# tomer196/GaUDI

Measured on AMD Instinct MI355X. Metric: guided molecules/sec (1000-step), higher is better.
Workload: dtype f32

## Files before the change

gaudi_amd/_lib.py:

```python
from __future__ import annotations

import ctypes as C
import os

import numpy as np

_PKG = os.path.dirname(os.path.abspath(__file__))
LIB_PATH = os.environ.get("GAUDI_LIB", os.path.join(_PKG, "libgaudi_hip.so"))


class GaudiError(RuntimeError):
    pass


class EdmConfig(C.Structure):
    _fields_ = [("in_node_nf", C.c_int32), ("hidden_nf", C.c_int32), ("n_layers", C.c_int32),
                ("inv_sublayers", C.c_int32), ("attention", C.c_int32), ("tanh", C.c_int32),
                ("coords_range", C.c_float), ("norm_constant", C.c_float), ("normalization_factor", C.c_float),
                ("diffusion_steps", C.c_int32), ("noise_power", C.c_float), ("noise_precision", C.c_float),
                ("norm_values", C.c_float * 3), ("sin_embedding", C.c_int32)]


class PredConfig(C.Structure):
    _fields_ = [("in_nf", C.c_int32), ("out_nf", C.c_int32), ("hidden_nf", C.c_int32), ("n_layers", C.c_int32),
# ... 4 lines not shown
    _fields_ = [("max_masked_leak", C.c_float), ("max_cog_rel", C.c_float), ("max_cog_abs", C.c_float),
                ("nan_count", C.c_int32), ("reprojected", C.c_int32)]


class RingTables(C.Structure):
    _fields_ = [("n_types", C.c_int32), ("orientation", C.c_int32), ("check_dihedrals", C.c_int32), ("tol", C.c_double),
                ("min_dist", C.c_double), ("dist_lo", (C.c_double * 16) * 16), ("dist_hi", (C.c_double * 16) * 16),
                ("a3_count", C.c_int32 * 16), ("a3_lo", (C.c_double * 4) * 16), ("a3_hi", (C.c_double * 4) * 16),
                ("a4_0", C.c_double), ("a4_180", C.c_double)]


class StabilityAux(C.Structure):
    _fields_ = [("n_rings", C.c_int32), ("n_edges", C.c_int32), ("n_triplets", C.c_int32), ("n_nan_angles", C.c_int32),
                ("a3_min", C.c_float), ("a3_max", C.c_float), ("a4_min", C.c_float), ("a4_max", C.c_float)]


class AtomTables(C.Structure):
    _fields_ = [("n_types", C.c_int32), ("ring_size", C.c_int32 * 16), ("ring_elem", (C.c_int32 * 6) * 16),
                ("templ", ((C.c_double * 2) * 6) * 16), ("no_orientation", C.c_int32 * 16), ("extra_angle", C.c_double * 16),
                ("n_template_h", C.c_int32 * 16), ("template_h_parent", (C.c_int32 * 2) * 16), ("h_elem", C.c_int32),
                ("c_elem", C.c_int32), ("h_bond", C.c_double)]


class PerceptionTables(C.Structure):
    _fields_ = [("n_elems", C.c_int32), ("cov_radius", C.c_double * 8), ("h_elem", C.c_int32), ("c_elem", C.c_int32),
                ("b_elem", C.c_int32), ("n_types", C.c_int32), ("ring_size", C.c_int32 * 16), ("ring_elem", (C.c_int32 * 6) * 16),
                ("no_orientation", C.c_int32 * 16), ("db_type", C.c_int32), ("dhdb_type", C.c_int32)]


class ValenceTables(C.Structure):
    _fields_ = [("n_elems", C.c_int32), ("n_options", (C.c_int32 * 5) * 8), ("option", (((C.c_int32 * 2) * 2) * 5) * 8),
                ("h_elem", C.c_int32), ("c_elem", C.c_int32)]


RINGS_MAX_ATOMS, RINGS_MAX_HEAVY, RINGS_MAX_RINGS = 384, 192, 32
RINGS_USE_H = 1
RINGS_OK, RINGS_NO_RINGS, RINGS_BAD_TYPE, RINGS_NOT_A_BASIS, RINGS_OVERFLOW = 0, 1, 2, 3, 4

ATOMS_MAX_ATOMS = 384
ATOMS_MAX_BONDS = 384
ATOMS_PLACE_H, ATOMS_FINGERPRINT = 1, 2

BONDS_MAX_ATOMS, BONDS_MAX_HEAVY, BONDS_MAX_BONDS, BONDS_MAX_CHARGED = 384, 192, 384, 4
(BONDS_OK, BONDS_NO_STRUCTURE, BONDS_CAPPED, BONDS_NOT_CONNECTED, BONDS_BAD_VALENCE, BONDS_BAD_INPUT, BONDS_OVERFLOW,
 BONDS_EMPTY, BONDS_GAVE_UP) = range(9)

FP_BINS = (256, 512, 1024)
CANON_MAX_ATOMS, CANON_MAX_HEAVY, CANON_MAX_BONDS, CANON_MAX_DEGREE, CANON_MAX_NODES, CANON_MAX_DEPTH = 384, 192, 384, 8, 4096, 16
CANON_OK, CANON_GAVE_UP, CANON_BAD_INPUT, CANON_OVERFLOW, CANON_EMPTY = range(5)
SUB_MAX_QUERY, SUB_MAX_PATTERNS, SUB_MAX_STEPS, SUB_H_EXACT, SUB_CLOSED = 32, 64, 8192, 1, 2
SUB_OK, SUB_GAVE_UP, SUB_BAD_INPUT, SUB_OVERFLOW, SUB_EMPTY, SUB_BAD_PATTERN = range(6)

FP = C.POINTER(C.c_float)
IP = C.POINTER(C.c_int32)
DP = C.POINTER(C.c_double)
U8P = C.POINTER(C.c_uint8)


class TargetSpec(C.Structure):
    _fields_ = [("K", C.c_int32), ("w", FP), ("q", FP), ("c", FP), ("side", IP), ("scale", FP),
                ("w_per_mol", C.c_int32), ("q_per_mol", C.c_int32), ("c_per_mol", C.c_int32), ("side_per_mol", C.c_int32),
                ("scale_per_mol", C.c_int32), ("t_lo", C.c_int32), ("t_hi", C.c_int32)]


TARGET_CB = C.CFUNCTYPE(None, C.c_void_p, C.c_int, C.c_int, FP, C.c_float, FP)
TARGET_CBZ = C.CFUNCTYPE(None, C.c_void_p, C.c_int, C.c_int, C.c_int, C.c_int, FP, FP, C.c_float, FP, FP)

EXPORTS = {
    "gaudi_create": (C.c_int, [C.c_int, C.POINTER(C.c_void_p)]),
    "gaudi_destroy": (None, [C.c_void_p]),
    "gaudi_last_error": (C.c_char_p, [C.c_void_p]),
    "gaudi_load_edm": (C.c_int, [C.c_void_p, C.POINTER(EdmConfig), C.c_int, C.POINTER(C.c_char_p), C.POINTER(FP),
                                 C.POINTER(C.c_int64)]),
    "gaudi_load_predictor": (C.c_int, [C.c_void_p, C.POINTER(PredConfig), C.c_int, C.POINTER(C.c_char_p),
                                       C.POINTER(FP), C.POINTER(C.c_int64)]),
    "gaudi_get_gamma": (C.c_int, [C.c_void_p, FP]),
    "gaudi_get_step_coefficients": (C.c_int, [C.c_void_p, FP]),
    "gaudi_phi": (C.c_int, [C.c_void_p, C.c_int, C.c_int, FP, FP, FP, FP, FP]),
    "gaudi_predictor_fwd": (C.c_int, [C.c_void_p, C.c_int, C.c_int, FP, FP, FP, FP, FP]),
    "gaudi_predictor_grad": (C.c_int, [C.c_void_p, C.c_int, C.c_int, FP, FP, FP, FP, FP, FP, FP]),
    "gaudi_step": (C.c_int, [C.c_void_p, C.c_int, C.c_int, C.c_int, FP, FP, FP, FP, FP, C.c_float, FP]),
    "gaudi_decode": (C.c_int, [C.c_void_p, C.c_int, C.c_int, FP, FP, FP, FP, FP, FP]),
    "gaudi_sample": (C.c_int, [C.c_void_p, C.c_int, C.c_int, FP, FP, C.c_uint64, C.c_int64, FP, C.c_float, FP,
                               C.c_float, FP, FP, FP, C.POINTER(Diag)]),
    "gaudi_sample_cb": (C.c_int, [C.c_void_p, C.c_int, C.c_int, FP, FP, C.c_uint64, C.c_int64, FP, C.c_float, TARGET_CB,
                                  C.c_void_p, C.c_float, FP, FP, FP, C.POINTER(Diag)]),
    "gaudi_sample_cbz": (C.c_int, [C.c_void_p, C.c_int, C.c_int, FP, FP, C.c_uint64, C.c_int64, FP, C.c_float, TARGET_CBZ,
                                   C.c_void_p, C.c_float, FP, FP, FP, C.POINTER(Diag)]),
    "gaudi_sample_chain": (C.c_int, [C.c_void_p, C.c_int, C.c_int, FP, FP, C.c_uint64, C.c_int64, FP, C.c_float, C.c_int, FP]),
    "gaudi_predict_noised": (C.c_int, [C.c_void_p, C.c_int, C.c_int, FP, FP, IP, FP, FP, C.c_uint64, C.c_int64, FP, FP, FP]),
    "gaudi_check_stability": (C.c_int, [C.c_void_p, C.POINTER(RingTables), C.c_int, C.c_int, FP, IP, IP,
                                        C.POINTER(C.c_uint8), FP, FP, C.POINTER(StabilityAux)]),
    "gaudi_stability_profile_get": (C.c_int, [C.c_void_p, C.POINTER(C.c_int32), C.POINTER(C.c_double)]),
    "gaudi_rings_to_atoms": (C.c_int, [C.c_void_p, C.POINTER(RingTables), C.POINTER(AtomTables), C.c_int, C.c_int, FP, IP, IP,
                                       C.c_int, C.c_int, C.c_int, IP, IP, DP, DP, IP, IP, IP, C.POINTER(C.c_uint64)]),
    "gaudi_atoms_profile_get": (C.c_int, [C.c_void_p, C.POINTER(C.c_int32), C.POINTER(C.c_double)]),
    "gaudi_atoms_to_rings": (C.c_int, [C.c_void_p, C.POINTER(PerceptionTables), C.c_int, C.c_int, DP, IP, IP, C.c_int, C.c_double,
                                       C.c_int, IP, IP, IP, IP, IP, DP, IP, DP, C.POINTER(C.c_uint8)]),
    "gaudi_rings_profile_get": (C.c_int, [C.c_void_p, C.POINTER(C.c_int32), C.POINTER(C.c_double)]),
    "gaudi_host_atoms_to_rings": (C.c_int, [C.POINTER(PerceptionTables), C.c_int, C.c_int, DP, IP, IP, C.c_int, C.c_double,
                                            C.c_int, IP, IP, IP, IP, IP, DP, IP, DP, C.POINTER(C.c_uint8)]),
    "gaudi_bond_orders": (C.c_int, [C.c_void_p, C.POINTER(ValenceTables), C.c_int, C.c_int, C.c_int, IP, IP, IP, IP,
                                    C.POINTER(C.c_uint8), C.POINTER(C.c_int8), IP, IP]),
    "gaudi_bonds_profile_get": (C.c_int, [C.c_void_p, C.POINTER(C.c_int32), C.POINTER(C.c_double)]),
    "gaudi_host_bond_orders": (C.c_int, [C.POINTER(ValenceTables), C.c_int, C.c_int, C.c_int, IP, IP, IP, IP,
                                         C.POINTER(C.c_uint8), C.POINTER(C.c_int8), IP, IP]),
    "gaudi_canonical_order": (C.c_int, [C.c_void_p, C.c_int, C.c_int, C.c_int, C.c_int, C.c_int, C.c_int, IP, IP, IP, IP, IP, IP,
                                        C.POINTER(C.c_uint8), IP, C.POINTER(C.c_uint16), IP, IP]),
    "gaudi_canon_profile_get": (C.c_int, [C.c_void_p, C.POINTER(C.c_int32), C.POINTER(C.c_double)]),
    "gaudi_host_canonical_order": (C.c_int, [C.c_int, C.c_int, C.c_int, C.c_int, C.c_int, C.c_int, IP, IP, IP, IP, IP, IP,
                                             C.POINTER(C.c_uint8), IP, C.POINTER(C.c_uint16), IP, IP]),
    "gaudi_circular_fingerprint": (C.c_int, [C.c_void_p, C.c_int, C.c_int, C.c_int, C.c_int, C.c_int, C.c_int, IP, IP, IP, IP, C.c_int,
                                             C.c_int, U8P, IP, IP]),
    "gaudi_host_circular_fingerprint": (C.c_int, [C.c_int, C.c_int, C.c_int, C.c_int, C.c_int, C.c_int, IP, IP, IP, IP, C.c_int,
                                                  C.c_int, U8P, IP, IP]),
    "gaudi_fp_library_set": (C.c_int, [C.c_void_p, C.c_int, C.c_int, U8P]),
    "gaudi_fp_nearest": (C.c_int, [C.c_void_p, C.c_int, C.c_int, U8P, C.c_int, U8P, C.c_int, IP, IP, IP]),
    "gaudi_fp_common": (C.c_int, [C.c_void_p, C.c_int, C.c_int, U8P, C.c_int, U8P, IP]),
    "gaudi_host_fp_nearest": (C.c_int, [C.c_int, C.c_int, U8P, C.c_int, U8P, C.c_int, IP, IP, IP]),
    "gaudi_fp_profile_get": (C.c_int, [C.c_void_p, C.POINTER(C.c_int32), C.POINTER(C.c_double)]),
    "gaudi_substructure_search": (C.c_int, [C.c_void_p] + [C.c_int] * 6 + [IP] * 4 + [C.c_int] * 3 + [IP] * 5 + [IP, IP, U8P, IP, IP]),
    "gaudi_host_substructure_search": (C.c_int, [C.c_int] * 6 + [IP] * 4 + [C.c_int] * 3 + [IP] * 5 + [IP, IP, U8P, IP, IP]),
    "gaudi_host_substructure_root_steps": (C.c_int, [C.c_int]),
    "gaudi_substructure_profile_get": (C.c_int, [C.c_void_p, C.POINTER(C.c_int32), C.POINTER(C.c_double)]),
    "gaudi_philox_normal": (C.c_int, [C.c_void_p, C.c_uint64, C.c_int64, C.c_int, C.c_int, C.c_int, C.c_int, FP]),
    "gaudi_host_schedule": (C.c_int, [C.c_int, C.c_float, C.c_float, FP, FP]),
    "gaudi_host_eigh3": (C.c_int, [C.c_int, DP, DP]),
    "gaudi_host_graph_meta": (C.c_int, [C.c_int, C.c_int, FP, FP, C.POINTER(C.c_int32), C.POINTER(C.c_int32),
                                        C.POINTER(C.c_int32), C.POINTER(C.c_uint32), C.POINTER(C.c_uint32), FP, C.c_int32,
                                        C.POINTER(C.c_int32)]),
    "gaudi_host_pack_matrix": (C.c_int, [C.c_int, C.c_int, C.c_int, C.c_int, C.c_int, FP, FP]),
    "gaudi_host_pack_matrix_split": (C.c_int, [C.c_int, C.c_int, C.c_int, C.c_int, C.c_int, C.c_int, C.c_float, FP, FP]),
    "gaudi_host_pack_matrix_f16": (C.c_int, [C.c_int, C.c_int, C.c_int, C.c_int, C.c_int, C.c_float, FP, FP]),
    "gaudi_host_weight_scale": (C.c_int, [C.c_int, C.POINTER(FP), IP, IP, IP, FP]),
    "gaudi_host_node_operand_offset": (C.c_int, [C.c_int, C.c_int, C.c_int, C.c_int, C.c_int, IP]),
    "gaudi_profile_reset": (C.c_int, [C.c_void_p, C.c_int]),
    "gaudi_profile_get": (C.c_int, [C.c_void_p, C.POINTER(C.c_int32), C.POINTER(C.c_double), C.POINTER(C.c_int64)]),
    "gaudi_set_steps_per_launch": (C.c_int, [C.c_void_p, C.c_int]),
    "gaudi_set_readout_nodes": (C.c_int, [C.c_void_p, C.c_int]),
    "gaudi_set_fix_noise": (C.c_int, [C.c_void_p, C.c_int, C.c_int64]),
    "gaudi_host_graph_meta8": (C.c_int, [C.c_int, C.c_int, FP, FP, C.POINTER(C.c_int32), C.POINTER(C.c_int32),
                                         C.POINTER(C.c_int32), C.POINTER(C.c_uint32), C.POINTER(C.c_uint32), FP,
                                         C.POINTER(C.c_uint16), C.POINTER(C.c_uint16), C.c_int32, C.POINTER(C.c_int32)]),
    "gaudi_kernel_variant": (C.c_int, [C.c_void_p, C.POINTER(C.c_int32), C.POINTER(C.c_int32)]),
    "gaudi_edge_math": (C.c_int, [C.c_void_p, C.POINTER(C.c_int32), C.POINTER(C.c_int32)]),
    "gaudi_node_buffers": (C.c_int, [C.c_void_p, C.POINTER(C.c_int32)]),
    "gaudi_last_workgroups": (C.c_int, [C.c_void_p, C.POINTER(C.c_int32), C.POINTER(C.c_int32)]),
    "gaudi_host_pack_plan_wide": (C.c_int, [C.c_int, C.c_int, C.c_int, C.c_int, FP, FP, C.POINTER(C.c_int32), C.POINTER(C.c_int32),
                                           C.POINTER(C.c_int32), C.POINTER(C.c_int32)]),
    "gaudi_set_plan_hint": (C.c_int, [C.c_void_p, C.c_int32, C.c_int32]),
    "gaudi_last_warning": (C.c_char_p, [C.c_void_p]),
    "gaudi_last_kernel_key": (C.c_int, [C.c_void_p, C.c_char_p, C.c_int]),
    "gaudi_kernel_key_log": (C.c_int, [C.c_void_p, C.c_char_p, C.c_int]),
    "gaudi_host_kernel_keys": (C.c_int, [C.c_char_p, C.c_int]),
    "gaudi_abi_version": (C.c_int, []),
    "gaudi_last_family_split": (C.c_int, [C.c_void_p, C.POINTER(C.c_int32)]),
    "gaudi_profile_clock": (C.c_int, [C.c_void_p, C.POINTER(C.c_double)]),
    "gaudi_last_keep_h": (C.c_int, [C.c_void_p, C.POINTER(C.c_int32)]),
    "gaudi_host_pack_plan": (C.c_int, [C.c_int, C.c_int, FP, FP, C.POINTER(C.c_int32), C.POINTER(C.c_int32), C.POINTER(C.c_int32),
                                      C.POINTER(C.c_int32)]),
    "gaudi_edm_nll": (C.c_int, [C.c_void_p, C.c_int, C.c_int, FP, FP, IP, FP, FP, C.c_uint64, C.c_int64, FP, FP, FP]),
    "gaudi_host_nll_terms": (C.c_int, [C.c_int, C.c_float, C.c_float, C.c_float, C.c_float, C.c_int, C.c_int, C.c_int, FP, FP, FP,
                                       IP, FP]),
    "gaudi_predictor_loss_grad": (C.c_int, [C.c_void_p, C.c_int, C.c_int, FP, FP, IP, FP, FP, FP, C.c_uint64, C.c_int64, FP, FP,
                                            FP, FP, IP]),
    "gaudi_predictor_grad_size": (C.c_int, [C.c_void_p, C.POINTER(C.c_int64)]),
    "gaudi_host_pred_train_layout": (C.c_int, [C.c_void_p, C.c_int, C.POINTER(C.c_char_p), C.POINTER(FP), C.POINTER(C.c_int64),
                                               IP, IP, FP]),
    "gaudi_edm_loss_grad": (C.c_int, [C.c_void_p, C.c_int, C.c_int, FP, FP, IP, FP, FP, C.c_uint64, C.c_int64, FP, C.c_int, FP,
                                      FP, FP, FP, IP]),
    "gaudi_edm_grad_size": (C.c_int, [C.c_void_p, C.POINTER(C.c_int64)]),
    "gaudi_edm_set_train_weights": (C.c_int, [C.c_void_p, C.c_int, C.POINTER(C.c_char_p), C.POINTER(FP), C.POINTER(C.c_int64)]),
    "gaudi_host_edm_train_layout": (C.c_int, [C.c_void_p, C.c_int, C.POINTER(C.c_char_p), C.POINTER(FP), C.POINTER(C.c_int64),
                                              IP, IP, FP]),
    "gaudi_host_train_floats_per_mol": (C.c_int, [C.c_int] * 8 + [C.POINTER(C.c_int64)]),
    "gaudi_host_edm_seed_coef": (C.c_int, [C.c_int, C.c_int, C.c_int, C.c_int, C.c_int, IP, FP, FP, FP]),
    "gaudi_sample_grid": (C.c_int, [C.c_void_p, C.c_int, C.c_int, FP, FP, C.c_uint64, C.c_int64, FP, C.c_float, FP, C.c_float,
                                    C.c_int, IP, FP, FP, FP, FP, FP, FP, C.POINTER(Diag)]),
    "gaudi_step_pair": (C.c_int, [C.c_void_p, C.c_int, C.c_int, C.c_int, C.c_int, FP, FP, FP, FP, FP, C.c_float, FP]),
    "gaudi_sample_cb_grid": (C.c_int, [C.c_void_p, C.c_int, C.c_int, FP, FP, C.c_uint64, C.c_int64, FP, C.c_float, TARGET_CB,
                                       TARGET_CBZ, C.c_void_p, C.c_float, C.c_int, IP, FP, FP, FP, FP, FP, FP, C.POINTER(Diag)]),
    "gaudi_host_grid_coefficients": (C.c_int, [C.c_int, C.c_float, C.c_float, C.c_int, IP, FP, IP]),
    "gaudi_sample_target": (C.c_int, [C.c_void_p, C.c_int, C.c_int, FP, FP, C.c_uint64, C.c_int64, FP, C.c_float,
                                      C.POINTER(TargetSpec), C.c_int, IP, FP, FP, FP, FP, FP, FP, FP, C.POINTER(Diag)]),
    "gaudi_step_target": (C.c_int, [C.c_void_p, C.c_int, C.c_int, C.c_int, C.c_int, FP, FP, FP, FP, C.POINTER(TargetSpec), FP, FP]),
    "gaudi_host_target_seed": (C.c_int, [C.POINTER(TargetSpec), C.c_int, C.c_int, FP, FP]),
}

ABI_VERSION = 7
_ROUND6_EXPORTS = ("gaudi_last_warning", "gaudi_abi_version", "gaudi_last_family_split", "gaudi_profile_clock", "gaudi_last_keep_h")
_NLL_EXPORTS = ("gaudi_edm_nll", "gaudi_predictor_loss_grad", "gaudi_predictor_grad_size", "gaudi_edm_loss_grad",
                "gaudi_edm_grad_size", "gaudi_edm_set_train_weights")
_GRID_EXPORTS = ("gaudi_sample_grid", "gaudi_step_pair", "gaudi_sample_cb_grid")
_TARGET_EXPORTS = ("gaudi_sample_target", "gaudi_step_target")
_ATOMS_EXPORTS = ("gaudi_rings_to_atoms", "gaudi_atoms_profile_get")
_RINGS_EXPORTS = ("gaudi_atoms_to_rings", "gaudi_rings_profile_get")
_BONDS_EXPORTS = ("gaudi_bond_orders", "gaudi_bonds_profile_get")
_CANON_EXPORTS = ("gaudi_canonical_order", "gaudi_canon_profile_get")
_FP_EXPORTS = ("gaudi_circular_fingerprint", "gaudi_fp_library_set", "gaudi_fp_nearest", "gaudi_fp_common",
               "gaudi_fp_profile_get")
_SUB_EXPORTS = ("gaudi_substructure_search", "gaudi_substructure_profile_get")
_KEY_EXPORTS = ("gaudi_last_kernel_key", "gaudi_kernel_key_log", "gaudi_host_kernel_keys")

_lib = None


def load_library() -> C.CDLL:
    global _lib
    if _lib is not None:
        return _lib
    if not os.path.exists(LIB_PATH):
        raise GaudiError(f"{LIB_PATH} not found: build it with `python -m gaudi_amd.build` "
                         "(there is no CPU fallback for the sampler)")
    lib = C.CDLL(LIB_PATH)
    lenient = "GAUDI_LIB" in os.environ
    abi = None
    if hasattr(lib, "gaudi_abi_version"):
        lib.gaudi_abi_version.restype, lib.gaudi_abi_version.argtypes = C.c_int, []
        abi = int(lib.gaudi_abi_version())
    if abi != ABI_VERSION and not lenient:
        raise GaudiError(f"{LIB_PATH} exports ABI version {abi}, this package expects {ABI_VERSION}: rebuild it "
                         "(`python -m gaudi_amd.build --force`)")
    for name, (res, args) in EXPORTS.items():
        if lenient and not hasattr(lib, name) and (name.startswith("gaudi_host_") or name in _ROUND6_EXPORTS + _NLL_EXPORTS + _GRID_EXPORTS + _TARGET_EXPORTS + _ATOMS_EXPORTS + _RINGS_EXPORTS + _BONDS_EXPORTS + _CANON_EXPORTS + _FP_EXPORTS + _SUB_EXPORTS + _KEY_EXPORTS):
            continue
        if lenient and abi != ABI_VERSION and name.startswith("gaudi_host_"):
            continue
        fn = getattr(lib, name)
        fn.restype = res
        fn.argtypes = args
    _lib = lib
    return lib


def key_lines(fn, *head) -> list:
    need = fn(*head, None, 0)
    if need < 0:
        raise GaudiError(f"{fn.__name__} failed ({need})")
    buf = C.create_string_buffer(need)
    fn(*head, buf, need)
    return buf.value.decode().splitlines()


def registered_kernel_keys() -> list:
    return key_lines(load_library().gaudi_host_kernel_keys)


def rings_outputs(B: int, max_rings: int) -> dict:
    M = int(max_rings)
    return dict(status=np.zeros(B, np.int32), n_rings=np.zeros(B, np.int32), ring_size=np.zeros((B, M), np.int32),
                ring_atoms=np.full((B, M, 6), -1, np.int32), ring_type=np.zeros((B, M), np.int32),
                centre=np.zeros((B, M, 3), np.float64), n_orient=np.zeros((B, M), np.int32),
                orient=np.zeros((B, M, 2, 3), np.float64), adj=np.zeros((B, M, M), np.uint8))


def rings_args(xyz, elem, n_atoms, flags, covalency_factor, max_rings, out):
    assert xyz.dtype == np.float64 and elem.dtype == np.int32 and n_atoms.dtype == np.int32
    assert xyz.flags["C_CONTIGUOUS"] and elem.flags["C_CONTIGUOUS"] and n_atoms.flags["C_CONTIGUOUS"]
    B, A = xyz.shape[0], xyz.shape[1]
    assert xyz.shape == (B, A, 3) and elem.shape == (B, A) and n_atoms.shape == (B,)
    ip = lambda a: a.ctypes.data_as(IP)
    dp = lambda a: a.ctypes.data_as(DP)
    return (B, A, dp(xyz), ip(elem), ip(n_atoms), int(flags), float(covalency_factor), int(max_rings), ip(out["status"]),
            ip(out["n_rings"]), ip(out["ring_size"]), ip(out["ring_atoms"]), ip(out["ring_type"]), dp(out["centre"]),
            ip(out["n_orient"]), dp(out["orient"]), out["adj"].ctypes.data_as(C.POINTER(C.c_uint8)))


def host_atoms_to_rings(tables, xyz, elem, n_atoms, flags=0, covalency_factor=1.3, max_rings=RINGS_MAX_RINGS) -> dict:
    lib = load_library()
    out = rings_outputs(xyz.shape[0], max_rings)
    rc = lib.gaudi_host_atoms_to_rings(C.byref(tables), *rings_args(xyz, elem, n_atoms, flags, covalency_factor, max_rings, out))
    if rc != 0:
        raise GaudiError(f"gaudi_host_atoms_to_rings failed ({rc})")
    return out


def bonds_outputs(B: int, A: int, M: int) -> dict:
    return dict(order=np.zeros((B, M), np.uint8), charge=np.zeros((B, A), np.int8), n_charged=np.zeros(B, np.int32),
                status=np.zeros(B, np.int32))


def bonds_args(elem, n_atoms, bonds, n_bonds, out):
    for a in (elem, n_atoms, bonds, n_bonds):
        assert a.dtype == np.int32 and a.flags["C_CONTIGUOUS"]
    B, A, M = elem.shape[0], elem.shape[1], bonds.shape[1]
    assert elem.shape == (B, A) and bonds.shape == (B, M, 2) and n_atoms.shape == (B,) and n_bonds.shape == (B,)
    ip = lambda a: a.ctypes.data_as(IP)
    return (B, A, M, ip(elem), ip(n_atoms), ip(bonds), ip(n_bonds), out["order"].ctypes.data_as(C.POINTER(C.c_uint8)),
            out["charge"].ctypes.data_as(C.POINTER(C.c_int8)), ip(out["n_charged"]), ip(out["status"]))


def host_bond_orders(tables, elem, n_atoms, bonds, n_bonds) -> dict:
    lib = load_library()
    out = bonds_outputs(elem.shape[0], elem.shape[1], bonds.shape[1])
    rc = lib.gaudi_host_bond_orders(C.byref(tables), *bonds_args(elem, n_atoms, bonds, n_bonds, out))
    if rc != 0:
        raise GaudiError(f"gaudi_host_bond_orders failed ({rc})")
    return out


def canon_outputs(B: int, A: int, M: int) -> dict:
    return dict(rank=np.zeros((B, A), np.int32), n_heavy=np.zeros(B, np.int32), label=np.zeros((B, A), np.uint8),
                n_hbonds=np.zeros(B, np.int32), cbonds=np.zeros((B, M, 2), np.uint16), nodes=np.zeros(B, np.int32),
                status=np.zeros(B, np.int32))


def canon_args(n_elems, h_elem, c_elem, elem, n_atoms, bonds, n_bonds, out):
    for a in (elem, n_atoms, bonds, n_bonds):
        assert a.dtype == np.int32 and a.flags["C_CONTIGUOUS"]
    B, A, M = elem.shape[0], elem.shape[1], bonds.shape[1]
    assert elem.shape == (B, A) and bonds.shape == (B, M, 2) and n_atoms.shape == (B,) and n_bonds.shape == (B,)
    ip = lambda a: a.ctypes.data_as(IP)
    return (int(n_elems), int(h_elem), int(c_elem), B, A, M, ip(elem), ip(n_atoms), ip(bonds), ip(n_bonds), ip(out["rank"]),
            ip(out["n_heavy"]), out["label"].ctypes.data_as(C.POINTER(C.c_uint8)), ip(out["n_hbonds"]),
            out["cbonds"].ctypes.data_as(C.POINTER(C.c_uint16)), ip(out["nodes"]), ip(out["status"]))


def host_canonical_order(n_elems, h_elem, c_elem, elem, n_atoms, bonds, n_bonds) -> dict:
    lib = load_library()
    out = canon_outputs(elem.shape[0], elem.shape[1], bonds.shape[1])
    rc = lib.gaudi_host_canonical_order(*canon_args(n_elems, h_elem, c_elem, elem, n_atoms, bonds, n_bonds, out))
    if rc != 0:
        raise GaudiError(f"gaudi_host_canonical_order failed ({rc})")
    return out


def fp_outputs(B: int, n_bins: int) -> dict:
    return dict(fp=np.zeros((B, n_bins), np.uint8), total=np.zeros(B, np.int32), status=np.zeros(B, np.int32))


def fp_args(n_elems, h_elem, c_elem, elem, n_atoms, bonds, n_bonds, radius, n_bins, out):
    for a in (elem, n_atoms, bonds, n_bonds):
        assert a.dtype == np.int32 and a.flags["C_CONTIGUOUS"]
    B, A, M = elem.shape[0], elem.shape[1], bonds.shape[1]
    assert elem.shape == (B, A) and bonds.shape == (B, M, 2) and n_atoms.shape == (B,) and n_bonds.shape == (B,)
    ip = lambda a: a.ctypes.data_as(IP)
    return (int(n_elems), int(h_elem), int(c_elem), B, A, M, ip(elem), ip(n_atoms), ip(bonds), ip(n_bonds), int(radius),
            int(n_bins), out["fp"].ctypes.data_as(U8P), ip(out["total"]), ip(out["status"]))


def host_circular_fingerprint(n_elems, h_elem, c_elem, elem, n_atoms, bonds, n_bonds, radius=2, n_bins=1024) -> dict:
    lib = load_library()
    out = fp_outputs(elem.shape[0], n_bins if n_bins in FP_BINS else 1)
    rc = lib.gaudi_host_circular_fingerprint(*fp_args(n_elems, h_elem, c_elem, elem, n_atoms, bonds, n_bonds, radius, n_bins, out))
    if rc != 0:
        raise GaudiError(f"gaudi_host_circular_fingerprint failed ({rc})")
    return out


def fp_rows(a) -> np.ndarray:
    a = np.ascontiguousarray(a, dtype=np.uint8)
    if a.ndim != 2:
        raise GaudiError(f"fingerprints must be [rows, n_bins], got shape {a.shape}")
    return a


def nearest_outputs(B: int, k: int) -> dict:
    k = max(int(k), 1)
    return dict(idx=np.zeros((B, k), np.int32), common=np.zeros((B, k), np.int32), union=np.zeros((B, k), np.int32))


def host_fp_nearest(q, lib_rows, k=1) -> dict:
    lib = load_library()
    q, lib_rows = fp_rows(q), fp_rows(lib_rows)
    out = nearest_outputs(q.shape[0], k)
    rc = lib.gaudi_host_fp_nearest(q.shape[1], q.shape[0], q.ctypes.data_as(U8P), lib_rows.shape[0], lib_rows.ctypes.data_as(U8P),
                                   int(k), *(out[n].ctypes.data_as(IP) for n in ("idx", "common", "union")))
    if rc != 0:
        raise GaudiError(f"gaudi_host_fp_nearest failed ({rc})")
    return out


def sub_outputs(B: int, P: int, A: int, QA: int) -> dict:
    return dict(count=np.zeros((B, P), np.int32), first=np.full((B, P, QA), -1, np.int32), covered=np.zeros((B, P, A), np.uint8),
                steps=np.zeros((B, P), np.int32), status=np.zeros((B, P), np.int32))


# ... 52 lines not shown
```

gaudi_amd/csrc/gaudi_hip.hip:

```cpp
#include <hip/hip_runtime.h>

#include <algorithm>
#include <climits>
#include <queue>
#include <cmath>
#include <cstdio>
#include <cstdlib>
#include <chrono>
#include <cstring>
#include <map>
#include <mutex>
#include <string>
#include <vector>

#include "../../include/gaudi_hip.h"
#include "kernel_table.h"

using namespace gaudi;

struct DevBuf {
  void* p = nullptr;
  size_t cap = 0;
  hipError_t reserve(size_t bytes) {
    if (bytes <= cap) return hipSuccess;
    if (p) (void)hipFree(p);
    p = nullptr;
    cap = 0;
    hipError_t e = hipMalloc(&p, bytes);
    if (e == hipSuccess) cap = bytes;
    return e;
  }
  void release() {
    if (p) (void)hipFree(p);
    p = nullptr;
    cap = 0;
  }
  template <class T>
  T* as() const { return (T*)p; }
};

struct PinBuf {
  void* p = nullptr;
  size_t cap = 0;
  hipError_t reserve(size_t bytes) {
    if (bytes <= cap) return hipSuccess;
    if (p) (void)hipHostFree(p);
    p = nullptr;
    cap = 0;
    hipError_t e = hipHostMalloc(&p, bytes, hipHostMallocDefault);
    if (e == hipSuccess) cap = bytes;
    return e;
  }
  void release() {
    if (p) (void)hipHostFree(p);
    p = nullptr;
    cap = 0;
  }
  template <class T>
  T* as() const { return (T*)p; }
};

enum NodeBuf : int {
  kResident = 0,
  kAllGlobal = 1,
  kPqLds = 2,
  kPredFifthGlobal = 3,
};
struct LaunchPlan {
  int waves = 4;
  int ring = 0;
  bool mr = false;
  NodeBuf nodes = kResident;
  bool two = false;
  bool fr = false;
  bool n1 = false;
  int ef = 2;
  int groups = 0;
  int nslots = 0;
  int hk = 0;
  int pubx = 0, pub_ch = 0;
};

struct VtCall {
  const gaudi_target_spec* spec = nullptr;
  int K = 0, Btot = 0, b0 = 0;
  float* trace = nullptr;
};

struct CallHints {
  int min_slots = 0, force_waves = 0;
  bool cut = false;
  int narrow = 0;
  const int32_t* molmap = nullptr;
  bool may_pack = false;
  const VtCall* vt = nullptr;
};

struct gaudi_handle {
  int device = 0;
  hipStream_t stream = nullptr;
  std::string err;
  std::string warn;
  bool has_edm = false, has_pred = false;
  gaudi_edm_config ecfg{};
  gaudi_pred_config pcfg{};
  int HPE = 0, HPP = 0;
  DevBuf edm_w, pred_w, coef_d, edm_w4, pred_w4;
  DevBuf edm_ws, pred_ws;
  size_t edm_w_bytes = 0, pred_w_bytes = 0, edm_ws_bytes = 0, pred_ws_bytes = 0;
  float edm_hinv = 0.f, pred_hinv = 0.f;
  std::vector<float> gamma, coef;
  DevBuf d_mask, d_order, d_edges, d_emask, d_npairs, d_seg, d_zin, d_zout, d_t, d_x, d_h, d_noise, d_nan, d_dpred,
      d_pred, d_tw, d_stash, d_chain, d_sx, d_stype, d_sn, d_sflags, d_sdist, d_sadj, d_saux, d_stab, d_as, d_ncols, d_soff,
      d_sidx, d_gnode, d_rowmap, d_compmol, d_ncomp, d_clock, d_gcoef, d_gidx, d_zt;
  DevBuf d_atoms[9];
  DevBuf d_rings[13];
  DevBuf d_bonds[9];
  DevBuf d_canon[11];
  DevBuf d_fp[16];
  int fp_lib_rows = 0, fp_lib_bins = 0;
  DevBuf d_sub[10];
  DevBuf d_vtpar, d_vttrace, d_vtdev;
  PinBuf p_pred, p_dpred;
  PinBuf p_z, p_dz;
  DevBuf d_dz;
  hipEvent_t cb_event = nullptr;
  int steps_per_launch = 25;
  int variant = 8;
  LaunchPlan plan;
  bool split = true;
  bool no_fr = false;
  bool no_n1 = false;
  bool no_side = false;
  std::string last_key;
  std::vector<std::string> key_log;
  bool wide_full = true;
  bool gn8_pq = true;
  bool gn8 = true;
  bool force_gn8 = false;
  bool pack = true;
  int pairs_cap = -1;
  int pairs = 1;
  int num_cus = 256;
  bool pred_rounds = true;
  bool force_mr = false;
  bool force_gn = false;
  bool fix_noise = false;
  long long fix_key = 0;
  int readout_n = 0;
  struct PredTrainState* pt = nullptr;
  struct EdmTrainState* et = nullptr;
  bool edm_stale = false;
  int plan_min_slots = 0, plan_force_waves = 0;
  bool keep_h = true;
  bool gn8_pack = true;
  bool family_split = false;
  int last_split_resident = 0;
  bool prof = false;
  struct EventLog {
    std::vector<std::pair<hipEvent_t, hipEvent_t>> pending, spare;
    double ms = 0.0;
    long long n = 0;
    static constexpr size_t kWindow = 32;
    hipError_t fold(size_t keep) {
      while (pending.size() > keep) {
        float t = 0.f;
        hipError_t e = hipEventSynchronize(pending.front().second);
        if (e == hipSuccess) e = hipEventElapsedTime(&t, pending.front().first, pending.front().second);
        if (e != hipSuccess) return e;
        ms += t;
        ++n;
        spare.push_back(pending.front());
        pending.erase(pending.begin());
      }
      return hipSuccess;
    }
    hipError_t begin(hipStream_t st, std::pair<hipEvent_t, hipEvent_t>& ev) {
      hipError_t e = fold(kWindow - 1);
      if (e != hipSuccess) return e;
      if (!spare.empty()) {
        ev = spare.back();
        spare.pop_back();
      } else {
        if ((e = hipEventCreate(&ev.first)) != hipSuccess) return e;
        if ((e = hipEventCreate(&ev.second)) != hipSuccess) return e;
      }
      return hipEventRecord(ev.first, st);
    }
    hipError_t end(hipStream_t st, const std::pair<hipEvent_t, hipEvent_t>& ev) {
      pending.push_back(ev);
      return hipEventRecord(ev.second, st);
    }
    void reset(bool destroy) {
      for (auto& p : pending) spare.push_back(p);
      pending.clear();
      if (destroy) {
        for (auto& p : spare) {
          (void)hipEventDestroy(p.first);
          (void)hipEventDestroy(p.second);
        }
        spare.clear();
      }
      ms = 0.0;
      n = 0;
    }
  } prof_log, stab_log, atoms_log, rings_log, bonds_log, canon_log, fp_log, sub_log;
  long long prof_steps = 0;
#ifdef GAUDI_STAMPS
  DevBuf d_stamps;
  unsigned long long stamp_acc[32] = {0};
#endif
};

#define HIPCHECK(h, call)                                                                         \
  do {                                                                                            \
    hipError_t e__ = (call);                                                                      \
    if (e__ != hipSuccess) {                                                                      \
      (h)->err = std::string(#call) + ": " + hipGetErrorString(e__);                              \
      return GAUDI_E_HIP;                                                                         \
    }                                                                                             \
  } while (0)

static int fail(gaudi_handle* h, int code, const std::string& msg) {
  if (h) h->err = msg;
  return code;
}

static void pt_release(gaudi_handle* h);
static void et_release(gaudi_handle* h);
static int et_upload(gaudi_handle* h, const gaudi_edm_config* cfg, int n, const char* const* names, const float* const* tensors,
                     const int64_t* numel);
static const char* et_check(const gaudi_edm_config* cfg, int n, const char* const* names, const int64_t* numel);
extern const char* const kEdmStale;
static int pt_load(gaudi_handle* h, const gaudi_pred_config* cfg, int n, const char* const* names, const float* const* tensors,
                   const int64_t* numel);

static std::vector<float> make_gamma(int T, double power, double precision) {
  const int steps = T + 1;
  if (power <= 0.0) {
    const int n = T + 2;
    const double s_ = 0.008, pi = 3.14159265358979323846;
    std::vector<double> ac(n);
    for (int i = 0; i < n; ++i) {
      const double x = (i == n - 1) ? (double)n : i * ((double)n / (double)(n - 1));
      const double c = std::cos(((x / n) + s_) / (1.0 + s_) * pi * 0.5);
      ac[i] = c * c;
    }
    const double a0 = ac[0];
    for (double& v : ac) v /= a0;
    std::vector<float> g(steps);
    double cum = 1.0;
    for (int i = 0; i < steps; ++i) {
      double beta = 1.0 - ac[i + 1] / ac[i];
      beta = std::min(std::max(beta, 0.0), 0.999);
      cum *= 1.0 - beta;
      g[i] = (float)(-(std::log(cum) - std::log(1.0 - cum)));
    }
    return g;
  }
  std::vector<double> a2(steps);
  const double step = (double)steps / (double)(steps - 1);
  for (int i = 0; i < steps; ++i) {
    double x = (i == steps - 1) ? (double)steps : i * step;
    double v = 1.0 - std::pow(x / steps, power);
    a2[i] = v * v;
  }
  std::vector<double> out(steps);
  double prev = 1.0, cum = 1.0;
  for (int i = 0; i < steps; ++i) {
    double r = a2[i] / prev;
    r = std::min(std::max(r, 0.001), 1.0);
    cum *= r;
    out[i] = cum;
    prev = a2[i];
  }
  std::vector<float> g(steps);
  const double pr = 1.0 - 2.0 * precision;
  for (int i = 0; i < steps; ++i) {
    double a = pr * out[i] + precision;
    g[i] = (float)(-(std::log(a) - std::log(1.0 - a)));
  }
  return g;
}

static inline float softplus_f(float x) { return x > 20.f ? x : log1pf(expf(x)); }
static inline float logsigmoid_f(float x) { return fminf(x, 0.f) - log1pf(expf(-fabsf(x))); }
// ... 401 lines not shown
  std::stable_sort(M.order.begin(), M.order.end(), [&](int a, int c) {
    return M.ntiles[a] != M.ntiles[c] ? M.ntiles[a] > M.ntiles[c] : total[a] > total[c];
  });
  return GAUDI_OK;
}

KernelTable* gaudi::g_kernel_tables;

static const KernelEntry* find_entry(const KernelKey& k) {
  for (const KernelTable* t = g_kernel_tables; t; t = t->next)
    for (int i = 0; i < t->n; ++i)
      if (t->entries[i].key == k) return &t->entries[i];
  return nullptr;
}
static kernel_fn find_kernel(const KernelKey& k) {
  const KernelEntry* e = find_entry(k);
  return e ? e->fn : nullptr;
}
static std::string key_name(const KernelKey& k) {
  char buf[160];
  snprintf(buf, sizeof buf, "waves=%d SP=%d MR=%d GN=%d FR=%d PG=%d N1=%d EF=%d HPE=%d HPP=%d VT=%d", k.waves, k.sp, (int)k.mr, k.gn,
           (int)k.fr, (int)k.pg, (int)k.n1, k.ef, k.hpe, k.hpp, (int)k.vt);
  return buf;
}
static std::string duplicate_kernel_key() {
  std::vector<KernelKey> seen;
  for (const KernelTable* t = g_kernel_tables; t; t = t->next)
    for (int i = 0; i < t->n; ++i) {
      if (std::find(seen.begin(), seen.end(), t->entries[i].key) != seen.end()) return key_name(t->entries[i].key);
      seen.push_back(t->entries[i].key);
    }
  return "";
}
static int gn_of(NodeBuf nodes) { return nodes == kAllGlobal ? 1 : nodes == kPqLds ? 2 : 0; }
static KernelKey key4(int hpe, int hpp, bool gn = false, int ef = 2) {
  KernelKey k{};
  k.waves = 4;
  k.gn = gn ? 1 : 0;
  k.ef = ef;
  k.hpe = hpe;
  k.hpp = hpp;
  return k;
}
static KernelKey key8(int hpe, int hpp, int ring, bool mr, NodeBuf nodes = kResident) {
  KernelKey k{};
  k.waves = 8;
  k.sp = ring;
  k.mr = mr;
  k.gn = gn_of(nodes);
  k.pg = nodes == kPredFifthGlobal;
  k.ef = 2;
  k.hpe = hpe;
  k.hpp = hpp;
  return k;
}
static bool have_kernel8(int hpe, int hpp, int ring, bool mr, NodeBuf nodes = kResident) {
  return find_kernel(key8(hpe, hpp, ring, mr, nodes)) != nullptr;
}
static NodeBuf launch_nodes(const LaunchPlan& p, int hpe, int hpp) {
  return p.nodes == kPredFifthGlobal && !(hpe && hpp) ? kResident : p.nodes;
}
static kernel_fn plan_kernel(const LaunchPlan& p, int hpe, int hpp, bool vt, KernelKey* key = nullptr) {
  KernelKey unused;
  KernelKey& k = key ? *key : unused;
  if (p.waves != 8) {
    k = key4(hpe, hpp, p.nodes == kAllGlobal, hpe ? p.ef : 2);
    k.vt = vt && hpp;
    return find_kernel(k);
  }
  const NodeBuf nodes = launch_nodes(p, hpe, hpp);
  const bool mr = p.mr && hpp;
  k = nodes == kResident ? key8(hpe, hpp, p.ring, mr) : key8(hpe, hpp, 1, true, nodes);
  k.vt = vt && hpp;
  if (p.fr && nodes == kResident && !mr) {
    k.fr = true;
    if (kernel_fn f = find_kernel(k)) return f;
    k.fr = false;
  }
  if (p.n1 && nodes == kResident && !mr) {
    k.n1 = true;
    if (kernel_fn f = find_kernel(k)) return f;
    k.n1 = false;
  }
  return find_kernel(k);
}

static int round_hidden(int H) {
  static const int sizes[] = {32, 48, 64, 128, 192, 208, 256};
  for (int s : sizes)
    if (s >= H) return s;
  return 0;
}

static int dense_ew4(int N) { return std::max(32, ((N + kWaves - 1) / kWaves * (N - 1) + 31) / 32 * 32); }

static size_t lds_bytes(int hpe, int hpp, int N, int D, int EW, bool gn = false, int ef = 2) {
  size_t net = 0;
  if (hpe)
    net = std::max(net, (size_t)((gn ? 0 : 4 * N * (hpe + 4)) + kWaves * 16 * (hpe + 4) + 8 * N + kWaves * EW * 9 + (6 + ef) * hpe +
                                 (ef > 2 ? kWaves * EW * ef : 0)));
  if (hpp) net = std::max(net, (size_t)((gn ? 0 : 5 * N * (hpp + 4)) + kWaves * 16 * (hpp + 4) + 12 * N + kWaves * EW * 10 + 32 + 10 * hpp));
  return sizeof(float) * (common_floats(N, D, EW) + net);
}
static size_t gnode_floats(int hpe, int hpp, int N) {
  return std::max((size_t)(hpe ? 4 * N * (hpe + 4) : 0), (size_t)(hpp ? 5 * N * (hpp + 4) : 0));
}

static size_t lds_floats8_base(int hpe, int hpp, int N, int D, int S, int split, NodeBuf nodes = kResident) {
  size_t net = 0;
  const int pbuf = nodes == kPredFifthGlobal ? 4 : 5;
  const int gn = gn_of(nodes);
  if (hpe) net = std::max(net, (size_t)((gn ? w8::gn_lds_buffers(gn) : 5) * N * (hpe + 4) + w8::edge_ring_floats(hpe, split) + 8 * N + 2 * align4(N) + 96 + S * 9 + 8 * hpe));
  if (hpp) net = std::max(net, (size_t)(w8::edge_ring_floats(hpp, split) + (gn ? w8::gn_lds_buffers(gn) : pbuf) * N * (hpp + 4) + 12 * N + 2 * align4(N) + 96 + S * 10 + 32 + 10 * hpp));
  return common_floats8(N, D, S) + net;
}
static size_t gnode_floats8(int hpe, int hpp, int N) {
  return std::max((size_t)(hpe ? 5 * N * (hpe + 4) : 0), (size_t)(hpp ? 5 * N * (hpp + 4) : 0));
}
static bool gn8_stage_fits(int hpe, int hpp, int N) {
  for (int hp : {hpe, hpp})
    if (hp && 2 * (size_t)w8::stage_stride(N * (hp + 4)) > w8::edge_ring_floats(hp, 1)) return false;
  return true;
}
static bool node_f16_fits(int hp, int N, int split, NodeBuf nodes) {
  const bool gn = gn_of(nodes) != 0;
  if (!hp || !split || !GAUDI_NODE_F16) return true;
  if (N > (gn ? 48 : 32)) return false;
  const int nct = N <= 16 ? 1 : N <= 32 ? 2 : 3;
  const int ring = w8::edge_ring_floats(hp, split);
  return w8::nh_split_floats(hp, nct) <= (w8::node_ring_idle(hp, split, gn) ? ring : ring / 2);
}
static bool plan_pub8(int hpe, int hpp, int N, int D, int S, int split, int& pubx, int& pub_ch, NodeBuf nodes = kResident) {
  pubx = 0;
  pub_ch = 0;
  const int gn = gn_of(nodes);
  if (!node_f16_fits(hpe, N, split, nodes) || !node_f16_fits(hpp, N, split, nodes)) return false;
  const long long cap = 160 * 1024 / 4 - 64;
  const long long base = (long long)lds_floats8_base(hpe, hpp, N, D, S, split, nodes);
  if (base > cap) return false;
  if (!hpp) return true;
  const int T = hpp / 16;
  const long long own = (gn ? 0LL : 2LL * N * (hpp + 4)) + (split ? w8::edge_ring_floats(hpp, split) : 0);
  pub_ch = w8::pub_chunk_tiles(S, own + (cap - base), T);
  if (pub_ch < 1) return false;
  const int nch = (T + pub_ch - 1) / pub_ch;
  pub_ch = (T + nch - 1) / nch;
  pubx = (int)std::max(0LL, (long long)S * (16 * pub_ch + 4) - own);
  return true;
}
static size_t lds_bytes8(int hpe, int hpp, int N, int D, int S, int pubx, int split, NodeBuf nodes = kResident) {
  return sizeof(float) * (lds_floats8_base(hpe, hpp, N, D, S, split, nodes) + (hpp ? pubx : 0));
}

static int launch(gaudi_handle* h, const KParams& P, int hpe, int hpp, long long steps) {
  const LaunchPlan& plan = h->plan;
  const bool v8 = plan.waves == 8;
  const bool se = hpe && plan.ef > 2;
  KernelKey key{};
  const kernel_fn fn = plan_kernel(plan, hpe, hpp, P.vt != nullptr, &key);
  if (!fn)
    return fail(h, GAUDI_E_INVALID,
                "no kernel instantiated for padded hidden sizes (" + std::to_string(hpe) + "," + std::to_string(hpp) + ")" +
                    (v8 ? " in the 8-wave family" : se ? " among the sin_embedding kernels" : ""));
  size_t lds = v8 ? lds_bytes8(hpe, hpp, P.N, 3 + P.F, P.EW, P.pubx, plan.ring, launch_nodes(plan, hpe, hpp))
                  : lds_bytes(hpe, hpp, P.N, 3 + P.F, P.EW, plan.nodes == kAllGlobal, se ? 24 : 2);
  if (v8 && P.hk_off) lds = sizeof(float) * ((size_t)P.hk_off + (size_t)plan.hk);
  if (lds > 160 * 1024)
    return fail(h, GAUDI_E_CAPACITY, "molecule needs " + std::to_string(lds) + " B of LDS (>160 KiB): N too large");
  {
    static std::mutex attr_mu;
    static std::map<std::pair<int, const void*>, int> granted_by_fn;
    std::lock_guard<std::mutex> lock(attr_mu);
    int& granted = granted_by_fn[{h->device, (const void*)fn}];
    if ((int)lds > granted) {
      HIPCHECK(h, hipFuncSetAttribute((const void*)fn, hipFuncAttributeMaxDynamicSharedMemorySize, (int)lds));
      granted = (int)lds;
    }
  }
  std::pair<hipEvent_t, hipEvent_t> ev{nullptr, nullptr};
  if (h->prof) HIPCHECK(h, h->prof_log.begin(h->stream, ev));
#ifdef GAUDI_STAMPS
  KParams PS = P;
  HIPCHECK(h, h->d_stamps.reserve(sizeof(unsigned long long) * 32));
  HIPCHECK(h, hipMemsetAsync(h->d_stamps.p, 0, sizeof(unsigned long long) * 32, h->stream));
  PS.stamps = h->d_stamps.as<unsigned long long>();
  hipLaunchKernelGGL(fn, dim3(P.B), dim3(v8 ? w8::kThreads : kThreads), lds, h->stream, PS);
  {
    unsigned long long tmp[32];
    HIPCHECK(h, hipMemcpyAsync(tmp, h->d_stamps.p, sizeof(tmp), hipMemcpyDeviceToHost, h->stream));
    HIPCHECK(h, hipStreamSynchronize(h->stream));
    for (int i = 0; i < 32; ++i) h->stamp_acc[i] += tmp[i];
    if (getenv("GAUDI_PRINT_STAMPS")) {
      static const char* nm[] = {"node_gemm", "edge_gemm", "edge_epilogue", "barrier", "misc", "bwd_node", "bwd_stash_reload",
                                 "bwd_colsum_tail", "pub_wait", "stash", "pub_write", "colsum_loop", "colsum_barrier", "b_dcp",
                                 "b_gemm_de", "b_dv", "b_gemm_dt1", "b_du", "stage_vectors", "geo", "edm_embed_head", "noise_update",
                                 "bwd_reload_loads", "bwd_vec_commit", "pred_readout", "bwd_prologue", "x2", "x3"};
      unsigned long long tot = 0;
      for (int i = 0; i < ST_N; ++i) tot += h->stamp_acc[i];
      fprintf(stderr, "[stamps] cumulative shares (block 0, wave 0):");
      for (int i = 0; i < ST_N; ++i) fprintf(stderr, " %s=%.1f%%", nm[i], 100.0 * h->stamp_acc[i] / (tot ? tot : 1));
      fprintf(stderr, " total=%llu ticks\n", tot);
      if (tmp[31])
        fprintf(stderr, "[stamps] shader clock during this launch: %.0f MHz (%llu cycles / %llu ticks of 100 MHz)\n",
                100.0 * (double)tmp[30] / (double)tmp[31], tmp[30], tmp[31]);
    }
  }
#else
  if (h->prof) {
    KParams PC = P;
    HIPCHECK(h, h->d_clock.reserve(sizeof(unsigned long long) * 4));
    PC.clock_out = h->d_clock.as<unsigned long long>();
    hipLaunchKernelGGL(fn, dim3(P.B), dim3(v8 ? w8::kThreads : kThreads), lds, h->stream, PC);
  } else {
    hipLaunchKernelGGL(fn, dim3(P.B), dim3(v8 ? w8::kThreads : kThreads), lds, h->stream, P);
  }
#endif
  HIPCHECK(h, hipGetLastError());
  h->last_key = key_name(key);
  if (std::find(h->key_log.begin(), h->key_log.end(), h->last_key) == h->key_log.end()) h->key_log.push_back(h->last_key);
  if (const KernelEntry* e = find_entry(key); e && (e->side & 1) && P.side_off != 0) h->last_key += " SD=" + std::to_string(e->side);
  if (getenv("GAUDI_DEBUG_PLAN")) fprintf(stderr, "[launch] %s\n", h->last_key.c_str());
  if (h->prof) {
    HIPCHECK(h, h->prof_log.end(h->stream, ev));
    h->prof_steps += steps;
  }
  return GAUDI_OK;
}

struct Pack {
  int G = 0;
  int NG = 0;
  std::vector<float> umask, uemask;
  std::vector<uint8_t> align;
  std::vector<int32_t> rowmap;
  std::vector<int32_t> compmol;
  std::vector<int32_t> ncomp;
};
static std::vector<std::vector<int>> used_nodes(int B, int N, const float* node_mask, const float* edge_mask) {
  std::vector<std::vector<int>> used(B);
  for (int b = 0; b < B; ++b) {
    std::vector<char> keep(N, 0);
    for (int i = 0; i < N; ++i) {
      const bool li = node_mask[(size_t)b * N + i] != 0.f;
      if (li) keep[i] = 1;
      for (int j = 0; j < N; ++j) {
        const bool lj = node_mask[(size_t)b * N + j] != 0.f;
        if (edge_mask[((size_t)b * N + i) * N + j] != 0.f && (li || lj)) keep[i] = keep[j] = 1;
      }
    }
    for (int i = 0; i < N; ++i)
      if (keep[i]) used[b].push_back(i);
  }
  return used;
}
static void pack_groups(int B, int N, const float* node_mask, const float* edge_mask, const Meta8& M, Pack& pk, int NG = 0,
                        int TG = w8::kWaves, bool narrow = false, int maxcomp = kMaxComp, const int32_t* molmap = nullptr,
                        int max_multi = INT_MAX) {
  if (NG < N && !narrow) NG = N;
  const std::vector<std::vector<int>> used = used_nodes(B, N, node_mask, edge_mask);
  struct Group {
    std::vector<int> mols;
    int nodes = 0, tiles = 0;
  };
  std::vector<Group> groups;
  int multi = 0;
  for (int b : M.order) {
    const int nn = (int)used[b].size(), nt = M.ntiles[b];
    Group* fit = nullptr;
    for (Group& g : groups)
      if ((int)g.mols.size() < maxcomp && g.nodes + nn <= NG && g.tiles + nt <= TG && (g.mols.size() > 1 || multi < max_multi)) {
        fit = &g;
        if (g.mols.size() == 1) ++multi;
        break;
      }
    if (!fit) {
      groups.emplace_back();
      fit = &groups.back();
    }
    fit->mols.push_back(b);
    fit->nodes += nn;
    fit->tiles += nt;
  }
  const int G = (int)groups.size();
  pk.G = G;
  pk.NG = NG;
  pk.umask.assign((size_t)G * NG, 0.f);
  pk.uemask.assign((size_t)G * NG * NG, 0.f);
  pk.align.assign((size_t)G * NG, 0);
  pk.rowmap.assign((size_t)G * NG, -1);
  pk.compmol.assign((size_t)G * kMaxComp, 0);
  pk.ncomp.assign(G, 0);
  std::vector<int> slot_of(N);
  for (int g = 0; g < G; ++g) {
    int base = 0;
    for (size_t k = 0; k < groups[g].mols.size(); ++k) {
      const int b = groups[g].mols[k];
      pk.compmol[(size_t)g * kMaxComp + k] = molmap ? molmap[b] : b;
      std::fill(slot_of.begin(), slot_of.end(), -1);
      for (size_t r = 0; r < used[b].size(); ++r) slot_of[used[b][r]] = base + (int)r;
      if (!used[b].empty()) pk.align[(size_t)g * NG + base] = 1;
      for (int i : used[b]) {
        const int si = slot_of[i];
        pk.umask[(size_t)g * NG + si] = node_mask[(size_t)b * N + i];
        pk.rowmap[(size_t)g * NG + si] = (b * N + i) | ((int32_t)k << 28);
        for (int j : used[b])
          pk.uemask[((size_t)g * NG + si) * NG + slot_of[j]] = edge_mask[((size_t)b * N + i) * N + j];
      }
      base += (int)used[b].size();
    }
    pk.ncomp[g] = (int)groups[g].mols.size();
  }
}

static int stage_graph8(gaudi_handle* h, int B, int N, const float* node_mask, const float* edge_mask, KParams& P, int hpe,
                        int hpp, const CallHints& hints, LaunchPlan& plan) {
  if (std::max(h->plan_force_waves, hints.force_waves) == 4) return 1;
  Meta8 M;
  std::string err;
  int rc = build_meta8(B, N, node_mask, edge_mask, M, err, std::max(h->plan_min_slots, hints.min_slots));
  if (rc == GAUDI_E_CAPACITY) return 1;
  if (rc) return fail(h, rc, err);
  const bool mr = hpp && (M.S > 16 * w8::kWaves || h->force_mr);
  if (mr && !h->pred_rounds) return 1;
  if (!have_kernel8(hpe, hpp, 0, mr) && !have_kernel8(hpe, hpp, 1, mr) && !have_kernel8(hpe, hpp, 2, mr)) return 1;
  const int Dz = 3 + (hpe ? h->ecfg.in_node_nf : h->pcfg.in_nf);
  const bool node_f16_ok = !GAUDI_NODE_F16 || ((!hpe || h->edm_hinv > 0.f) && (!hpp || h->pred_hinv > 0.f));
  struct RingPlan {
    int mode = -1, pubx = 0, pub_ch = 0;
  };
  auto plan_for = [&](int NS, int S, bool mrk) -> RingPlan {
    RingPlan r;
    if (h->split && (!hpe || h->edm_ws_bytes) && (!hpp || h->pred_ws_bytes) && node_f16_ok)
      for (int mode = 1; mode <= 2; ++mode)
        if (have_kernel8(hpe, hpp, mode, mrk) && plan_pub8(hpe, hpp, NS, Dz, S, mode, r.pubx, r.pub_ch)) return RingPlan{mode, r.pubx, r.pub_ch};
    return have_kernel8(hpe, hpp, 0, mrk) && plan_pub8(hpe, hpp, NS, Dz, S, 0, r.pubx, r.pub_ch) ? RingPlan{0, r.pubx, r.pub_ch} : RingPlan{};
  };
  RingPlan acc = plan_for(N, M.S, mr);
  int mode_u = acc.mode;
  Pack pk;
  const int B0 = B;
  const float* nm_used = node_mask;
  int n_slots = N;
  bool mr_run = mr;
  bool narrow_taken = false, use_pack = false, pg_run = false;
  if (hints.narrow > 0 && hints.narrow < N && hints.may_pack && (int64_t)B * N < (1 << 28)) {
    pack_groups(B, N, node_mask, edge_mask, M, pk, hints.narrow, w8::kWaves, true, kMaxComp, hints.molmap);
    Meta8 M2;
    rc = build_meta8(pk.G, hints.narrow, pk.umask.data(), pk.uemask.data(), M2, err, 0, pk.align.data());
    if (rc != GAUDI_OK) return fail(h, rc, "per-molecule kernel family: " + err);
    const bool mr2 = hpp && M2.S > 16 * w8::kWaves;
    const RingPlan p2 = plan_for(hints.narrow, M2.S, mr2);
    if (p2.mode < 1 || mr2) return fail(h, GAUDI_E_CAPACITY, "per-molecule kernel family: the resident plan of the small bucket does not fit");
    M = std::move(M2);
    B = pk.G;
    nm_used = pk.umask.data();
    n_slots = hints.narrow;
    acc = p2;
    mode_u = p2.mode;
    mr_run = mr2;
    narrow_taken = use_pack = true;
  }
  NodeBuf gn8 = kResident;
  RingPlan gplan{1, 0, 0};
  if (!narrow_taken && (mode_u < 0 || h->force_gn8) && h->gn8 && h->split && (!hpe || h->edm_ws_bytes) && (!hpp || h->pred_ws_bytes) && node_f16_ok &&
      (GAUDI_NODE_F16 || gn8_stage_fits(hpe, hpp, N))) {
    if (h->gn8_pq && GAUDI_NODE_F16 && have_kernel8(hpe, hpp, 1, true, kPqLds) && plan_pub8(hpe, hpp, N, Dz, M.S, 1, gplan.pubx, gplan.pub_ch, kPqLds)) gn8 = kPqLds;
    else if (have_kernel8(hpe, hpp, 1, true, kAllGlobal) && plan_pub8(hpe, hpp, N, Dz, M.S, 1, gplan.pubx, gplan.pub_ch, kAllGlobal)) gn8 = kAllGlobal;
  }
  if (gn8) {
    acc = gplan;
    mode_u = 1;
// ... 34 lines not shown
        auto run = [&](int n, double cost) {
          for (int k = 0; k < n; ++k) {
            const double t = free_at.top() + cost;
            free_at.pop();
            free_at.push(t);
            end = std::max(end, t);
          }
        };
        run(p, kPair);
        run(B - 2 * p, kAlone);
        return end;
      };
      double best = solo * 0.995;
      int best_p = -1;
      for (int p = cus; p <= B / 2 + cus - 1; p += cus) {
        const int pp = std::min(p, B / 2);
        const double m = makespan(pp);
        if (m < best) { best = m; best_p = pp; }
      }
      if (h->pairs_cap >= 0) best_p = std::min(h->pairs_cap, B / 2);
      if (best_p >= 0) {
        pack_groups(B, N, node_mask, edge_mask, M, pk, N, w8::kWaves);
        want_wide = (long long)pk.G * 10 >= (long long)B * 9;
        max_multi = best_p;
      }
    }
    if (want_wide && h->pairs_cap >= 0) max_multi = h->pairs_cap;
    if (want_wide)
      for (int ng = std::min(2 * N, 32); ng > N; --ng) {
        const long long cap = 160 * 1024 / 4 - 64;
        if ((long long)lds_floats8_base(hpe, hpp, ng, Dz, 16 * (w8::kWaves + 1), h->split ? 2 : 0) > cap) continue;
        cands.push_back({ng, 2 * w8::kWaves});
      }
    cands.push_back({N, w8::kWaves});
    for (const Cand& cd : cands) {
      const bool wide = cd.NG > N;
      pack_groups(B, N, node_mask, edge_mask, M, pk, cd.NG, cd.TG, false, kMaxComp, nullptr, wide ? max_multi : INT_MAX);
      if (pk.G >= B && !(wide && h->pairs_cap == 0)) continue;
      Meta8 M2;
      rc = build_meta8(pk.G, cd.NG, pk.umask.data(), pk.uemask.data(), M2, err, wide ? 0 : M.S, pk.align.data());
      if (rc != GAUDI_OK) continue;
      const bool mr2 = hpp && M2.S > 16 * w8::kWaves;
      if (!wide && M2.S > std::max(M.S, 16 * w8::kWaves)) continue;
      if (mr2 && !mr && !h->pred_rounds) continue;
      RingPlan p2 = plan_for(cd.NG, M2.S, mr2);
      if (p2.mode < 0 || (p2.mode != 0) != (mode_u != 0)) continue;
      RingPlan full{1, 0, 0};
      if (wide && p2.mode == 2 && mr2 && h->wide_full && hpe && hpp && have_kernel8(hpe, hpp, 1, true, kPredFifthGlobal) &&
          plan_pub8(hpe, hpp, cd.NG, Dz, M2.S, 1, full.pubx, full.pub_ch, kPredFifthGlobal)) {
        p2 = full;
        pg_run = true;
      }
      M = std::move(M2);
      B = pk.G;
      nm_used = pk.umask.data();
      n_slots = cd.NG;
      acc = p2;
      mr_run = mr2;
      use_pack = true;
      break;
    }
  }
  const bool packed = use_pack;
  const NodeBuf nodes = pg_run ? kPredFifthGlobal : gn8;
  P.pubx = acc.pubx;
  P.pub_ch = acc.pub_ch;
  auto one_step_tail = [](int H, int HP) { return !HP || !w8::nh_odd(HP) || has_ktail(H, HP); };
  const bool n1_run = !h->no_n1 && nodes == kResident && acc.mode == 1 && n_slots <= 16 &&
                      one_step_tail(h->ecfg.hidden_nf, hpe) && one_step_tail(h->pcfg.hidden_nf, hpp);
  if (getenv("GAUDI_DEBUG_PLAN"))
    fprintf(stderr, "[plan] molecules=%d workgroups=%d N=%d node slots=%d S=%d split=%d mr=%d nodes=%d n1=%d pub_ch=%d pubx=%d lds=%zu\n", B0, B,
            N, n_slots, M.S, acc.mode, (int)mr_run, (int)nodes, (int)n1_run, acc.pub_ch, acc.pubx,
            lds_bytes8(hpe, hpp, n_slots, Dz, M.S, acc.pubx, acc.mode, nodes));
  auto up = [&](DevBuf& d, const void* src, size_t bytes) -> hipError_t {
    hipError_t e = d.reserve(bytes);
    if (e != hipSuccess) return e;
    return hipMemcpyAsync(d.p, src, bytes, hipMemcpyHostToDevice, h->stream);
  };
  HIPCHECK(h, up(h->d_ncols, M.ncols.data(), sizeof(int) * B));
  HIPCHECK(h, up(h->d_mask, nm_used, sizeof(float) * B * n_slots));
  if (packed) {
    HIPCHECK(h, up(h->d_rowmap, pk.rowmap.data(), sizeof(int32_t) * pk.rowmap.size()));
    HIPCHECK(h, up(h->d_compmol, pk.compmol.data(), sizeof(int32_t) * pk.compmol.size()));
    HIPCHECK(h, up(h->d_ncomp, pk.ncomp.data(), sizeof(int32_t) * pk.ncomp.size()));
  }
  HIPCHECK(h, up(h->d_order, M.order.data(), sizeof(int) * B));
  HIPCHECK(h, up(h->d_edges, M.edges.data(), sizeof(uint32_t) * M.edges.size()));
  HIPCHECK(h, up(h->d_emask, M.emask.data(), sizeof(float) * M.emask.size()));
  HIPCHECK(h, up(h->d_npairs, M.ntiles.data(), sizeof(int) * B));
  HIPCHECK(h, up(h->d_seg, M.seg.data(), sizeof(uint32_t) * M.seg.size()));
  HIPCHECK(h, up(h->d_soff, M.soff.data(), sizeof(uint16_t) * M.soff.size()));
  HIPCHECK(h, up(h->d_sidx, M.sidx.data(), sizeof(uint16_t) * M.sidx.size()));
  HIPCHECK(h, hipStreamSynchronize(h->stream));
  P.B = B;
  P.N = n_slots;
  P.NR = N;
  P.EW = M.S;
  P.node_mask = h->d_mask.as<float>();
  P.order = h->d_order.as<int>();
  P.edges = h->d_edges.as<uint32_t>();
  P.emask = h->d_emask.as<float>();
  P.npairs = h->d_npairs.as<int>();
  P.seginfo = h->d_seg.as<uint32_t>();
  P.ncols = h->d_ncols.as<int>();
  P.soff = h->d_soff.as<uint16_t>();
  P.sidx = h->d_sidx.as<uint16_t>();
  P.rowmap = packed ? h->d_rowmap.as<int32_t>() : nullptr;
  P.compmol = packed ? h->d_compmol.as<int32_t>() : nullptr;
  P.ncomp = packed ? h->d_ncomp.as<int32_t>() : nullptr;
  P.hk_off = 0;
  P.side_off = 0;
  int hk = 0;
  bool side_run = false;
  if (h->keep_h && GAUDI_NODE_F16 && acc.mode >= 1 && nodes == kResident) {
    const size_t floats = lds_bytes8(hpe, hpp, n_slots, Dz, M.S, acc.pubx, acc.mode) / sizeof(float);
    const size_t at = (floats + 3) & ~(size_t)3;
    const size_t need = (size_t)w8::nh_keep_floats(std::max(hpe, hpp), n_slots);
    KernelKey kn = key8(hpe, hpp, 1, false);
    kn.n1 = true;
    const KernelEntry* const en = find_entry(kn);
    const bool side_want = !h->no_side && n1_run && hpe && hpp && !mr_run && en != nullptr && (en->side & 1) &&
                           *std::max_element(M.ntiles.begin(), M.ntiles.begin() + B) <= w8::kWaves - 1;
    const size_t side = (size_t)n_slots * (hpp + 4);
    if (side_want && (at + side + need) * sizeof(float) + 1024 <= 160 * 1024) {
      P.side_off = (int)at;
      P.hk_off = (int)(at + side);
      hk = (int)need;
      side_run = true;
    } else if ((at + need) * sizeof(float) + 1024 <= 160 * 1024) {
      P.hk_off = (int)at;
      hk = (int)need;
    }
  }
  if (getenv("GAUDI_DEBUG_PLAN")) fprintf(stderr, "[plan] side=%d side_off=%d hk_off=%d hk=%d\n", (int)side_run, P.side_off, P.hk_off, hk);
  if (pg_run) {
    const size_t stride = ((size_t)n_slots * (hpp + 4) + 63) / 64 * 64;
    HIPCHECK(h, h->d_gnode.reserve(sizeof(float) * (stride * (size_t)B + 256)));
    P.gnode = h->d_gnode.as<float>();
    P.gnode_stride = (long long)stride;
  }
  if (gn8) {
    const size_t stride = (gnode_floats8(hpe, hpp, N) + 63) / 64 * 64;
    HIPCHECK(h, h->d_gnode.reserve(sizeof(float) * (stride * (size_t)B + 256)));
    P.gnode = h->d_gnode.as<float>();
    P.gnode_stride = (long long)stride;
  }
  plan.waves = 8;
  plan.ring = acc.mode;
  plan.mr = mr_run;
  plan.nodes = nodes;
  plan.fr = !h->no_fr && gn8 == kResident && acc.mode == 1 && n_slots > 16;
  plan.n1 = n1_run;
  plan.groups = B;
  plan.nslots = n_slots;
  plan.hk = hk;
  plan.pubx = acc.pubx;
  plan.pub_ch = acc.pub_ch;
  return GAUDI_OK;
}

static int stage_graph(gaudi_handle* h, int B, int N, const float* node_mask, const float* edge_mask, KParams& P, int hpe,
                       int hpp, const CallHints& hints) {
  if (B <= 0 || N <= 0) return fail(h, GAUDI_E_INVALID, "B and N must be positive");
  if ((int64_t)B * N >= (1 << 28)) return fail(h, GAUDI_E_CAPACITY, "B * N must stay below 2^28 per call: cut the request into several calls");
  LaunchPlan plan;
  const bool se = hpe && h->ecfg.sin_embedding;
  if (h->variant == 8 && !h->force_gn && !se) {
    const int rc8 = stage_graph8(h, B, N, node_mask, edge_mask, P, hpe, hpp, hints, plan);
    if (rc8 == GAUDI_OK) h->plan = plan;
    if (rc8 <= 0) return rc8;
    P.pubx = P.pub_ch = 0;
  }
  plan.groups = B;
  plan.nslots = N;
  if (hpp && 4 * N * 3 > 4 * 16 * (hpp + 4))
    return fail(h, GAUDI_E_CAPACITY, "N too large for the 4-wave predictor kernels at this hidden size");
  Meta M;
  std::string err;
  int rc = build_meta(B, N, node_mask, edge_mask, M, err);
  if (rc) return fail(h, rc, err);
  HIPCHECK(h, h->d_mask.reserve(sizeof(float) * B * N));
  HIPCHECK(h, h->d_order.reserve(sizeof(int) * B));
  HIPCHECK(h, h->d_edges.reserve(sizeof(uint32_t) * M.edges.size()));
  HIPCHECK(h, h->d_emask.reserve(sizeof(float) * M.emask.size()));
  HIPCHECK(h, h->d_npairs.reserve(sizeof(int) * M.npairs.size()));
  HIPCHECK(h, h->d_seg.reserve(sizeof(uint32_t) * M.seg.size()));
  HIPCHECK(h, h->d_ncols.reserve(sizeof(int) * B));
  HIPCHECK(h, hipMemcpyAsync(h->d_ncols.p, M.ncols.data(), sizeof(int) * B, hipMemcpyHostToDevice, h->stream));
  HIPCHECK(h, hipMemcpyAsync(h->d_mask.p, node_mask, sizeof(float) * B * N, hipMemcpyHostToDevice, h->stream));
  HIPCHECK(h, hipMemcpyAsync(h->d_order.p, M.order.data(), sizeof(int) * B, hipMemcpyHostToDevice, h->stream));
  HIPCHECK(h, hipMemcpyAsync(h->d_edges.p, M.edges.data(), sizeof(uint32_t) * M.edges.size(), hipMemcpyHostToDevice, h->stream));
  HIPCHECK(h, hipMemcpyAsync(h->d_emask.p, M.emask.data(), sizeof(float) * M.emask.size(), hipMemcpyHostToDevice, h->stream));
  HIPCHECK(h, hipMemcpyAsync(h->d_npairs.p, M.npairs.data(), sizeof(int) * M.npairs.size(), hipMemcpyHostToDevice, h->stream));
  HIPCHECK(h, hipMemcpyAsync(h->d_seg.p, M.seg.data(), sizeof(uint32_t) * M.seg.size(), hipMemcpyHostToDevice, h->stream));
  HIPCHECK(h, hipStreamSynchronize(h->stream));
  P.B = B;
  P.N = N;
  P.NR = N;
  P.EW = M.EW;
  P.node_mask = h->d_mask.as<float>();
  P.order = h->d_order.as<int>();
  P.edges = h->d_edges.as<uint32_t>();
  P.emask = h->d_emask.as<float>();
  P.npairs = h->d_npairs.as<int>();
  P.seginfo = h->d_seg.as<uint32_t>();
  P.ncols = h->d_ncols.as<int>();
  const int Dz = 3 + (hpe ? h->ecfg.in_node_nf : h->pcfg.in_nf);
  const bool part_of_batch = h->plan_min_slots || h->plan_force_waves || hints.min_slots || hints.force_waves || hints.cut;
  const int ef = plan.ef = se ? 24 : 2;
  const bool have_g = (!hpe || find_kernel(key4(hpe, 0, true, ef))) && (!hpp || find_kernel(key4(0, hpp, true)));
  if (h->force_gn || lds_bytes(hpe, hpp, N, Dz, part_of_batch ? std::max(M.EW, dense_ew4(N)) : M.EW, false, ef) > 160 * 1024) {
    if (have_g && lds_bytes(hpe, hpp, N, Dz, M.EW, true, ef) <= 160 * 1024) {
      plan.nodes = kAllGlobal;
      const size_t stride = (gnode_floats(hpe, hpp, N) + 63) / 64 * 64;
      HIPCHECK(h, h->d_gnode.reserve(sizeof(float) * stride * (size_t)B));
      P.gnode = h->d_gnode.as<float>();
      P.gnode_stride = (long long)stride;
    }
  }
  plan.two = plan.nodes == kAllGlobal || (se && hpp && !find_kernel(key4(hpe, hpp, false, ef)));
  h->plan = plan;
  return GAUDI_OK;
}

static void fill_edm(gaudi_handle* h, KParams& P) {
  const gaudi_edm_config& c = h->ecfg;
  P.F = c.in_node_nf;
  P.T = c.diffusion_steps;
  P.edm.w = (h->variant == 8 && h->plan.waves == 4) ? h->edm_w4.as<float>() : h->edm_w.as<float>();
  P.edm.w_bytes = (unsigned)h->edm_w_bytes;
  P.edm.F = c.in_node_nf;
  P.edm.L = c.n_layers;
  P.edm.S = c.inv_sublayers;
  P.edm.attention = c.attention;
  P.edm.use_tanh = c.tanh;
  P.edm.coords_range = c.coords_range;
  P.edm.norm_constant = c.norm_constant;
  P.edm.normf = c.normalization_factor > 0.f ? c.normalization_factor : (float)P.NR;
  P.edm.ktail = h->plan.waves == 8 && has_ktail(c.hidden_nf, h->HPE);
  P.edm.ws = h->edm_ws.as<float>();
  P.edm.ws_bytes = (unsigned)h->edm_ws_bytes;
  P.edm.hinv = h->edm_hinv;
  P.coef = h->coef_d.as<float>();
  const float g0 = h->gamma[0];
  P.alpha0 = sqrtf(sigmoid_host(-g0));
  P.sigma0 = sqrtf(sigmoid_host(g0));
  P.sigma_x = expf(0.5f * g0);
  P.nv0 = c.norm_values[0];
  P.nv1 = c.norm_values[1];
}

extern "C" {

int gaudi_create(int device, gaudi_handle** out) {
  if (!out) return GAUDI_E_INVALID;
  *out = nullptr;
  static const std::string dup = duplicate_kernel_key();
  if (!dup.empty()) {
    fprintf(stderr, "libgaudi_hip: two translation units register the kernel %s\n", dup.c_str());
    return GAUDI_E_INVALID;
  }
  int n = 0;
  if (hipGetDeviceCount(&n) != hipSuccess || device < 0 || device >= n) return GAUDI_E_HIP;
  gaudi_handle* h = new gaudi_handle();
  h->device = device;
  if (const char* v = getenv("GAUDI_WAVES")) h->variant = atoi(v) == 4 ? 4 : 8;
  if (const char* v = getenv("GAUDI_EDGE_MATH")) h->split = std::string(v) != "fp32";
  if (const char* v = getenv("GAUDI_FORCE_GN")) h->force_gn = atoi(v) != 0;
  if (const char* v = getenv("GAUDI_GN8")) h->gn8 = atoi(v) != 0;
  if (const char* v = getenv("GAUDI_FORCE_GN8")) h->force_gn8 = atoi(v) != 0;
  if (const char* v = getenv("GAUDI_FORCE_MR")) h->force_mr = atoi(v) != 0;
  if (const char* v = getenv("GAUDI_PACK")) h->pack = atoi(v) != 0;
  if (const char* v = getenv("GAUDI_GN8_PACK")) h->gn8_pack = atoi(v) != 0;
  if (const char* v = getenv("GAUDI_GN8_PQ")) h->gn8_pq = atoi(v) != 0;
  if (const char* v = getenv("GAUDI_WIDE_FULL")) h->wide_full = atoi(v) != 0;
  if (const char* v = getenv("GAUDI_KEEP_H")) h->keep_h = atoi(v) != 0;
  if (const char* v = getenv("GAUDI_FAMILY_SPLIT")) h->family_split = atoi(v) != 0;
  if (const char* v = getenv("GAUDI_PAIRS")) h->pairs = atoi(v);
  if (const char* v = getenv("GAUDI_PAIRS_CAP")) h->pairs_cap = atoi(v);
  {
    int cus = 0;
    if (hipDeviceGetAttribute(&cus, hipDeviceAttributeMultiprocessorCount, device) == hipSuccess && cus > 0) h->num_cus = cus;
  }
  if (const char* v = getenv("GAUDI_PRED_ROUNDS")) h->pred_rounds = atoi(v) != 0;
  h->no_fr = getenv("GAUDI_NO_FR") != nullptr;
  h->no_n1 = getenv("GAUDI_NO_N1") != nullptr;
  h->no_side = getenv("GAUDI_NO_SIDE") != nullptr;
  h->plan.waves = h->variant;
  if (hipSetDevice(device) != hipSuccess || hipStreamCreateWithFlags(&h->stream, hipStreamNonBlocking) != hipSuccess) {
    delete h;
    return GAUDI_E_HIP;
  }
  *out = h;
  return GAUDI_OK;
}

void gaudi_destroy(gaudi_handle* h) {
  if (!h) return;
  (void)hipSetDevice(h->device);
  if (h->stream) (void)hipStreamSynchronize(h->stream);
  h->prof_log.reset(true);
  h->stab_log.reset(true);
  h->atoms_log.reset(true);
  h->rings_log.reset(true);
  h->bonds_log.reset(true);
  h->canon_log.reset(true);
  h->fp_log.reset(true);
  h->sub_log.reset(true);
  DevBuf* bufs[] = {&h->edm_w, &h->pred_w, &h->coef_d, &h->edm_w4, &h->pred_w4, &h->edm_ws, &h->pred_ws, &h->d_mask, &h->d_order, &h->d_edges, &h->d_emask, &h->d_npairs,
                    &h->d_seg, &h->d_zin, &h->d_zout, &h->d_t, &h->d_x, &h->d_h, &h->d_noise, &h->d_nan, &h->d_dpred,
                    &h->d_pred, &h->d_tw, &h->d_stash, &h->d_chain, &h->d_sx, &h->d_stype, &h->d_sn,
                    &h->d_sflags, &h->d_sdist, &h->d_sadj, &h->d_saux, &h->d_stab, &h->d_as, &h->d_ncols, &h->d_soff, &h->d_sidx,
                    &h->d_gnode, &h->d_rowmap, &h->d_compmol, &h->d_ncomp, &h->d_gcoef, &h->d_gidx, &h->d_zt, &h->d_vtpar, &h->d_vttrace, &h->d_vtdev};
  for (DevBuf* b : bufs) b->release();
  for (DevBuf& b : h->d_atoms) b.release();
  for (DevBuf& b : h->d_rings) b.release();
  for (DevBuf& b : h->d_bonds) b.release();
  for (DevBuf& b : h->d_canon) b.release();
  for (DevBuf& b : h->d_fp) b.release();
  for (DevBuf& b : h->d_sub) b.release();
  pt_release(h);
  et_release(h);
  h->p_pred.release();
  h->p_dpred.release();
  h->p_z.release();
  h->p_dz.release();
  h->d_dz.release();
  if (h->cb_event) (void)hipEventDestroy(h->cb_event);
  if (h->stream) (void)hipStreamDestroy(h->stream);
  delete h;
}

const char* gaudi_last_error(const gaudi_handle* h) { return h ? h->err.c_str() : "null handle"; }
const char* gaudi_last_warning(const gaudi_handle* h) { return h ? h->warn.c_str() : ""; }
int gaudi_last_kernel_key(const gaudi_handle* h, char* buf, int n) {
  if (!h || !buf || n <= 0) return GAUDI_E_INVALID;
  snprintf(buf, (size_t)n, "%s", h->last_key.c_str());
  return GAUDI_OK;
}
static int copy_lines(const std::vector<std::string>& names, char* buf, int n) {
  std::string all;
  for (const std::string& s : names) all += s + "\n";
  if (buf && n > 0) snprintf(buf, (size_t)n, "%s", all.c_str());
  return (int)all.size() + 1;
}
int gaudi_host_kernel_keys(char* buf, int n) {
  if (n < 0) return GAUDI_E_INVALID;
  std::vector<std::string> names;
  for (const KernelTable* t = g_kernel_tables; t; t = t->next)
    for (int i = 0; i < t->n; ++i) names.push_back(key_name(t->entries[i].key));
  std::sort(names.begin(), names.end());
  return copy_lines(names, buf, n);
}
int gaudi_kernel_key_log(const gaudi_handle* h, char* buf, int n) {
  if (!h || n < 0) return GAUDI_E_INVALID;
  return copy_lines(h->key_log, buf, n);
}
int gaudi_abi_version(void) { return GAUDI_ABI_VERSION; }
int gaudi_profile_clock(gaudi_handle* h, double* shader_mhz) {
  if (!h || !shader_mhz) return GAUDI_E_INVALID;
  *shader_mhz = 0.0;
  if (!h->d_clock.p) return GAUDI_OK;
  HIPCHECK(h, hipSetDevice(h->device));
  unsigned long long c[4] = {0, 0, 0, 0};
  HIPCHECK(h, hipStreamSynchronize(h->stream));
  HIPCHECK(h, hipMemcpy(c, h->d_clock.p, sizeof(c), hipMemcpyDeviceToHost));
  if (c[3] > c[1] && c[2] > c[0]) *shader_mhz = 100.0 * (double)(c[2] - c[0]) / (double)(c[3] - c[1]);
  return GAUDI_OK;
}
int gaudi_last_keep_h(const gaudi_handle* h, int32_t* lds_floats) {
  if (!h || !lds_floats) return GAUDI_E_INVALID;
  *lds_floats = h->plan.hk;
  return GAUDI_OK;
}
int gaudi_last_family_split(const gaudi_handle* h, int32_t* resident_molecules) {
  if (!h || !resident_molecules) return GAUDI_E_INVALID;
  *resident_molecules = h->last_split_resident;
  return GAUDI_OK;
}

int gaudi_load_edm(gaudi_handle* h, const gaudi_edm_config* cfg, int n, const char* const* names,
                   const float* const* tensors, const int64_t* numel) {
  if (!h || !cfg) return GAUDI_E_INVALID;
  HIPCHECK(h, hipSetDevice(h->device));
  const int H = cfg->hidden_nf, F = cfg->in_node_nf, F1 = F + 1, L = cfg->n_layers, S = cfg->inv_sublayers;
  if (H <= 0 || H > 256) return fail(h, GAUDI_E_INVALID, "hidden_nf must be in 1..256");
  if (F < 1 || F > 15) return fail(h, GAUDI_E_INVALID, "in_node_nf must be in 1..15");
  if (L < 1 || S < 1 || cfg->diffusion_steps < 1) return fail(h, GAUDI_E_INVALID, "bad n_layers/inv_sublayers/diffusion_steps");
  if (!(cfg->normalization_factor >= 0.f)) return fail(h, GAUDI_E_INVALID, "normalization_factor must be > 0 (or 0: 'mean' aggregation)");
  const int HP = round_hidden(H);
  if (!HP) return fail(h, GAUDI_E_INVALID, "no kernel instantiated for this hidden size");
  Tensors T;
  for (int i = 0; i < n; ++i) T.m[names[i]] = {tensors[i], numel[i]};
  const int EF = cfg->sin_embedding ? 24 : 2;
  EdmLayout lay{HP, F1, L, S, EF};
  const std::string p = "dynamics.egnn.";
  const int PK = HP * HP;
  float hscale = 0.f;
  {
    NodeScale ns;
    for (int l = 0; l < L; ++l) {
      for (int s = 0; s <= S; ++s) {
        const std::string q = p + "e_block_" + std::to_string(l) + (s < S ? ".gcl_" + std::to_string(s) + "." : ".gcl_equiv.");
        ns.see(T.peek(q + (s < S ? "edge_mlp.0.weight" : "coord_mlp.0.weight"), (int64_t)H * (2 * H + EF)), H, 2 * H + EF, 0, 2 * H);
        ns.see(T.peek(q + (s < S ? "edge_mlp.2.weight" : "coord_mlp.2.weight"), (int64_t)H * H), H, H, 0, H, true);
        if (s < S) {
          ns.see(T.peek(q + "node_mlp.0.weight", (int64_t)H * 2 * H), H, 2 * H, 0, 2 * H);
          ns.see(T.peek(q + "node_mlp.2.weight", (int64_t)H * H), H, H, 0, H);
        }
      }
    }
    hscale = ns.scale();
    if (!(hscale > 0.f) && h->variant == 8 && h->split && EF == 2)
      h->warn = std::string("EDM weights: the fp16-pair images cannot carry this weight set (") + ns.why() +
                "): its calls run the fp32-instruction kernels (about 0.55 x the speed, same results at fp32 accuracy)";
  }
  auto pack = [&](bool lane_linear, std::vector<float>& w, std::vector<float>* ws) {
  w.assign((size_t)lay.total(), 0.f);
  if (ws) ws->assign(2 * (size_t)lay.total(), 0.f);
  PackMode pe;
  pe.lane_linear = lane_linear;
  pe.ktail = lane_linear && has_ktail(H, HP);
  pe.wbase = w.data();
  pe.ws = ws;
  pe.hscale = ws ? hscale : 0.f;
  pe.hktail = has_ktail(H, HP);
  const PackMode pn = pe.with_ktail(false);
  {
    const float* ew = T.get(p + "embedding.weight", (int64_t)H * F1);
    const float* eb = T.get(p + "embedding.bias", H);
    const float* ow = T.get(p + "embedding_out.weight", (int64_t)F1 * H);
    const float* ob = T.get(p + "embedding_out.bias", F1);
    if (ew && eb && ow && ob) {
      for (int f = 0; f < H; ++f)
        for (int k = 0; k < F1; ++k) w[lay.emb_w() + f * F1 + k] = ew[f * F1 + k];
      pack_vec(&w[lay.emb_b()], eb, H);
      for (int o = 0; o < F1; ++o)
        for (int k = 0; k < H; ++k) w[lay.out_w() + o * HP + k] = ow[o * H + k];
      pack_vec(&w[lay.out_b()], ob, F1);
    }
  }
  const int ld1 = 2 * H + EF;
  for (int l = 0; l < L; ++l) {
    for (int s = 0; s < S; ++s) {
      const std::string q = p + "e_block_" + std::to_string(l) + ".gcl_" + std::to_string(s) + ".";
      float* G = &w[lay.gcl(l, s)];
      float* V = G + 6 * PK;
      const float* W1 = T.get(q + "edge_mlp.0.weight", (int64_t)H * ld1);
      const float* b1 = T.get(q + "edge_mlp.0.bias", H);
      const float* W2 = T.get(q + "edge_mlp.2.weight", (int64_t)H * H);
      const float* b2 = T.get(q + "edge_mlp.2.bias", H);
      const float* Wn1 = T.get(q + "node_mlp.0.weight", (int64_t)H * 2 * H);
      const float* bn1 = T.get(q + "node_mlp.0.bias", H);
      const float* Wn2 = T.get(q + "node_mlp.2.weight", (int64_t)H * H);
      const float* bn2 = T.get(q + "node_mlp.2.bias", H);
      const float *wa = nullptr, *ba = nullptr;
      if (cfg->attention) {
        wa = T.get(q + "att_mlp.0.weight", H);
        ba = T.get(q + "att_mlp.0.bias", 1);
      }
      if (!(W1 && b1 && W2 && b2 && Wn1 && bn1 && Wn2 && bn2) || (cfg->attention && !(wa && ba))) continue;
      pack_node_matrix(pn, G, W1, H, ld1, 0, HP);
      pack_node_matrix(pn, G + PK, W1, H, ld1, H, HP);
      pack_edge_matrix(pe, G + 2 * PK, W2, H, H, 0, HP);
      pack_node_matrix(pn, G + 3 * PK, Wn1, H, 2 * H, 0, HP);
      pack_node_matrix(pn, G + 4 * PK, Wn1, H, 2 * H, H, HP);
      pack_node_matrix(pn, G + 5 * PK, Wn2, H, H, 0, HP);
      for (int k = 0; k < EF; ++k) pack_col(V + k * HP, W1, H, ld1, 2 * H + k);
      pack_vec(V + EF * HP, b1, H);
      pack_vec(V + (EF + 1) * HP, b2, H);
      if (wa) pack_vec(V + (EF + 2) * HP, wa, H);
      pack_vec(V + (EF + 3) * HP, bn1, H);
      pack_vec(V + (EF + 4) * HP, bn2, H);
      if (ba) V[(EF + 5) * HP] = ba[0];
      V[(EF + 5) * HP + 1] = col_absmax(W1, H, ld1, 2 * H);
      V[(EF + 5) * HP + 2] = col_absmax(W1, H, ld1, 2 * H + 1);
    }
    const std::string q = p + "e_block_" + std::to_string(l) + ".gcl_equiv.";
    float* E = &w[lay.equ(l)];
    float* V = E + 3 * PK;
    const float* W1 = T.get(q + "coord_mlp.0.weight", (int64_t)H * ld1);
    const float* b1 = T.get(q + "coord_mlp.0.bias", H);
    const float* W2 = T.get(q + "coord_mlp.2.weight", (int64_t)H * H);
    const float* b2 = T.get(q + "coord_mlp.2.bias", H);
    const float* w3 = T.get(q + "coord_mlp.4.weight", H);
    if (!(W1 && b1 && W2 && b2 && w3)) continue;
    pack_node_matrix(pn, E, W1, H, ld1, 0, HP);
// ... 358 lines not shown
```

gaudi_amd/csrc/w8_edm.h:

```cpp
#pragma once
#include "edm_device.h"
#include "w8_common.h"
#include "w8_split.h"
#include "w8_nodes_f16.h"

namespace gaudi {
namespace w8 {

__host__ __device__ constexpr int gn_lds_buffers(int gn) { return gn == 2 ? 2 : 0; }
template <int HP, int SP = 0, int GN = 0>
struct NetSmem {
  static constexpr bool kGlobalNodes = GN != 0;
  float *h, *p, *q;
  float *agg, *agg1;
  float* ring;
  float *x, *x0;
  uint32_t *pmax, *qmax;
  float* hsc;
  f4* geo;
  float* d0;
  float* trans;
  float* vec;
  float* hk = nullptr;
  __host__ __device__ static int floats(int N, int S) {
    return (GN ? gn_lds_buffers(GN) : 5) * N * (HP + 4) + EdgeRing<HP, SP>::kFloats + 8 * N + 2 * align4(N) + 96 + S * 9 + 8 * HP;
  }
  __device__ void carve(float* base, int N, int S, float* gnode = nullptr) {
    constexpr int LD = HP + 4;
    ring = base; base += EdgeRing<HP, SP>::kFloats;
    if (GN) gnode = assume_global(gnode);
    float*& nb = GN ? gnode : base;
    h = nb; nb += N * LD;
    if (GN == 2) {
      p = base; base += N * LD;
      q = base; base += N * LD;
    } else {
      p = nb; nb += N * LD;
      q = nb; nb += N * LD;
    }
    agg = nb; nb += N * LD;
    agg1 = nb; nb += N * LD;
    x = base; base += 4 * N;
    x0 = base; base += 4 * N;
    pmax = (uint32_t*)base; base += align4(N);
    qmax = (uint32_t*)base; base += align4(N);
    hsc = base; base += 96;
    geo = (f4*)base; base += S * 4;
    d0 = base; base += S;
    trans = base; base += S * 4;
    vec = base;
  }
};

template <class SM>
__device__ __forceinline__ void compute_geo(const SM& sm, const MolGraph& mg, float norm_constant, int tid, bool write_d0) {
  for (int slot = tid; slot < mg.ntiles * 16; slot += kThreads) {
    const uint32_t e = mg.edge[slot];
    const int i = ew_i(e), j = ew_j(e);
    const float dx = sm.x[4 * i + 0] - sm.x[4 * j + 0];
    const float dy = sm.x[4 * i + 1] - sm.x[4 * j + 1];
    const float dz = sm.x[4 * i + 2] - sm.x[4 * j + 2];
    const float r = dx * dx + dy * dy + dz * dz;
    if (write_d0) {
      sm.d0[slot] = r;
    } else {
      const float inv = 1.0f / (sqrtf(r + 1e-8f) + norm_constant);
      sm.geo[slot] = (f4){r, dx * inv, dy * inv, dz * inv};
    }
  }
}

template <class SM>
__device__ __forceinline__ void coord_update(const SM& sm, const MolGraph& mg, float normf, int tid) {
  for (int idx = tid; idx < mg.N * 3; idx += kThreads) {
    const int n = idx / 3, d = idx % 3;
    const uint32_t sg = mg.seg[n];
    const int st = sg >> 16, len = sg & 0xffff;
    float s = 0.f;
    for (int k = 0; k < len; ++k) s += sm.trans[(st + k) * 4 + d];
    sm.x[4 * n + d] = (sm.x[4 * n + d] + s / normf) * mg.mask[n];
  }
}

struct TileCols {
  bool active;
  int slot;
  int i, j;
  bool run_end;
  int part;
  float mk;
  RunMask rm;
};
__device__ __forceinline__ TileCols load_tile(const MolGraph& mg, int round, int wave, int c) {
  TileCols tc;
  const int tile = round * kWaves + wave;
  tc.active = __builtin_amdgcn_readfirstlane(tile < mg.ntiles ? 1 : 0) != 0;
  tc.slot = (tc.active ? tile : 0) * 16 + c;
  const uint32_t e = mg.edge[tc.slot];
  tc.i = ew_i(e);
  tc.j = ew_j(e);
  tc.run_end = ew_run_end(e);
  tc.part = ew_part(e);
  tc.mk = mg.em[tc.slot];
  tc.rm.set(c, ew_run_start(e));
  return tc;
}

template <int HP>
__device__ __forceinline__ void scatter_runs(f4 (&e)[HP / 16], const TileCols& tc, float* agg0, float* agg1, int g) {
  constexpr int T = HP / 16, LD = HP + 4;
  float* dst = (tc.part ? agg1 : agg0) + tc.i * LD + 4 * g;
#pragma unroll
  for (int t = 0; t < T; ++t) {
    const f4 s = seg_scan(e[t], tc.rm);
    if (tc.run_end) *(f4*)(dst + 16 * t) = s;
  }
}

template <int HP, int SP = 0, int GN = 0, int FL = 0>
__device__ __forceinline__ void edm_forward(const EdmDev& W, const MolGraph& mg, const NetSmem<HP, SP, GN>& sm, const float* sZ,
                                            float* sEps, float* sMean , float t_val, int tid STAMP_DECL) {
  constexpr int LD = HP + 4;
  constexpr int T = HP / 16;
  constexpr int PK = HP * HP;
  const int wave = __builtin_amdgcn_readfirstlane(tid >> 6), lane = tid & 63, c = lane & 15, g = lane >> 4;
  const int N = mg.N, D = mg.D, F = W.F, F1 = F + 1;
  EdmLayout lay{HP, F1, W.L, W.S};
  const float* __restrict__ w = W.w;
  const WBuf wb = make_wbuf(W.w, W.w_bytes);
  const WBuf wbe = SP ? make_wbuf(W.ws, W.ws_bytes) : wb;
  const bool tw = W.ktail != 0;

  for (int idx = tid; idx < N * 3; idx += kThreads) {
    const int n = idx / 3, d = idx % 3;
    const float v = sZ[n * D + d] * mg.mask[n];
    sm.x[4 * n + d] = v;
    sm.x0[4 * n + d] = v;
  }
  {
    const float* ew = w + lay.emb_w();
    const float* eb = w + lay.emb_b();
    for (int idx = tid; idx < N * HP; idx += kThreads) {
      const int n = idx / HP, f = idx % HP;
      float acc = 0.f;
      const float m = mg.mask[n];
      for (int k = 0; k < F; ++k) acc += gload(ew + f * F1 + k) * (sZ[n * D + 3 + k] * m);
      acc += gload(ew + f * F1 + F) * t_val;
      sm.h[n * LD + f] = acc + gload(eb + f);
    }
  }
  __syncthreads();
  compute_geo(sm, mg, 0.f, tid, true);
  typename EdgeRing<HP, SP>::type ring;
  er_init<HP>(ring, sm.ring, W.ktail != 0, W.ws, W.hinv);
  static_assert(SP == 0 || NodeMath<SP>::kF16, "the split edge GEMMs take their column scales from the fp16 node GEMMs' row maxima");
  constexpr bool NH = NodeMath<SP>::kF16;
  constexpr bool RI = node_ring_idle(HP, SP, GN);
  constexpr bool STG = GN && !NH;
  float* const xs0 = sm.ring;
  float* const xs1 = sm.ring + stage_stride(N * LD);
  if constexpr (!RI) er_start<HP>(ring, wbe, lay.gcl(0, 0) + 2 * PK, wave, lane);
  typename NodePFSel<HP, NH>::type pf;
  node_prefetch_x<HP, NH, kAheadOne, FL>(pf, wb, wbe, lay.gcl(0, 0), mg.NC, wave, lane, tw);
  auto hctx = [&]() {
    if constexpr (NH) {
      if constexpr (RI) return node_ctx_h<HP>(sm.ring, EdgeRing<HP, SP>::kFloats, mg.NC, W.hinv, tw, sm.hsc);
      else return node_ctx_h<HP>(ring.slot(ring.par ^ 1), EdgeRing<HP, SP>::kFloats / 2, mg.NC, W.hinv, tw, sm.hsc);
    } else {
      return NodeCtxH{1.f, nullptr, nullptr, tw, nullptr};
    }
  };
  const bool keep = NH && sm.hk != nullptr;
  bool h_kept = false;
  constexpr int NV = (7 * HP + 16 + kThreads - 1) / kThreads;
  VecPF<NV> vpf;
  vec_prefetch<NV, kThreads>(vpf, wb, lay.gcl(0, 0) + 6 * PK, 7 * HP + 16, tid);
  STAMP(ST_EDM_IO);

  for (int l = 0; l < W.L; ++l) {
    compute_geo(sm, mg, W.norm_constant, tid, false);
    STAMP(ST_GEO);
    for (int s = 0; s < W.S; ++s) {
      const int G = lay.gcl(l, s);
      const int Wnext_edge = s + 1 < W.S ? lay.gcl(l, s + 1) + 2 * PK : lay.equ(l) + 2 * PK;
      if constexpr (STG) stage_rows(xs0, sm.h, N * LD, wave, lane);
      for (int idx = tid; idx < N * (LD / 4); idx += kThreads) {
        *(f4*)(sm.agg + 4 * idx) = splat(0.f);
        *(f4*)(sm.agg1 + 4 * idx) = splat(0.f);
      }
      if (tid < N) {
        sm.pmax[tid] = 0u;
        sm.qmax[tid] = 0u;
      }
      vec_commit<NV, kThreads>(vpf, sm.vec, 7 * HP + 16, tid);
      if constexpr (STG) stage_wait();
      else __syncthreads();
      STAMP(ST_STAGE);
      const float *cr = sm.vec, *cd = sm.vec + HP, *b1 = sm.vec + 2 * HP, *b2 = sm.vec + 3 * HP, *wa = sm.vec + 4 * HP,
                  *bn1 = sm.vec + 5 * HP, *bn2 = sm.vec + 6 * HP;
      const float ba = sm.vec[7 * HP];
      const float crmax = sm.vec[7 * HP + 1], cdmax = sm.vec[7 * HP + 2];
      {
        const NodeCtxH cx = keep ? node_ctx_keep<HP>(hctx(), sm.hk, mg.NC) : hctx();
        node_gemm_x<HP, EPI_NONE, false, GN, NH, kAheadOne, kAheadAll, FL>(wb, wbe, G, sm.h, xs0, !h_kept, -1, nullptr, nullptr, b1, sm.p, nullptr, nullptr, mg.NC,
                                                      wave, lane, tw, cx, pf, G + PK, nullptr, sm.pmax);
        h_kept = keep;
        node_gemm_x<HP, EPI_NONE, false, GN, NH, kAheadAll, kAheadOne, FL>(wb, wbe, G + PK, sm.h, xs0, false, -1, nullptr, nullptr, nullptr, sm.q, nullptr,
                                                      nullptr, mg.NC, wave, lane, tw, cx, pf,
                                                      G + 3 * PK, nullptr, sm.qmax);
      }
      STAMP(ST_NODE);
      __syncthreads();
      STAMP(ST_BARRIER);
      if constexpr (RI) er_start<HP>(ring, wbe, G + 2 * PK, wave, lane);
      for (int rd = 0; rd < mg.rounds; ++rd) {
        const TileCols tc = load_tile(mg, rd, wave, c);
        const f4 gg = sm.geo[tc.slot];
        f4 acc[T];
        const float d0v = sm.d0[tc.slot];
        const float ub = __builtin_bit_cast(float, sm.pmax[tc.i]) + __builtin_bit_cast(float, sm.qmax[tc.j]) + crmax * gg[0] + cdmax * fabsf(d0v);
        er_gemm_pq<HP>(acc, ring, wbe, G + 2 * PK, rd + 1 < mg.rounds ? G + 2 * PK : (RI ? -1 : Wnext_edge), b2, cr, cd,
                         sm.p + tc.i * LD + 4 * g, sm.q + tc.j * LD + 4 * g, gg[0], d0v, ub, tc.active, wave, lane STAMP_ARGS);
        STAMP(ST_EDGE);
        if (tc.active) {
          float sdot = 0.f;
#pragma unroll
          for (int t = 0; t < T; ++t) {
            const f4 m = silu4v(acc[t]);
            acc[t] = m;
            const f4 wv = *(const f4*)(wa + 16 * t + 4 * g);
            sdot += m[0] * wv[0] + m[1] * wv[1] + m[2] * wv[2] + m[3] * wv[3];
          }
          float a = 1.f;
          if (W.attention) a = sigmoid_f(reduce_groups(sdot) + ba);
          const float sc = a * tc.mk;
#pragma unroll
          for (int t = 0; t < T; ++t) acc[t] = acc[t] * sc;
          scatter_runs<HP>(acc, tc, sm.agg, sm.agg1, g);
        }
        STAMP(ST_EDGE_EPI);
      }
      __syncthreads();
      STAMP(ST_BARRIER);
      constexpr bool SUM = NH && GN == 0;
      if constexpr (!SUM) {
        if constexpr (STG) stage_rows(xs0, sm.h, N * LD, wave, lane);
        for (int idx = tid; idx < N * (HP / 4); idx += kThreads) {
          const int n = idx / (HP / 4), f = 4 * (idx % (HP / 4));
          if constexpr (STG)
            *(f4*)(xs1 + n * LD + f) = (*(const f4*)(sm.agg + n * LD + f) + *(const f4*)(sm.agg1 + n * LD + f)) / W.normf;
          else
            *(f4*)(sm.agg + n * LD + f) = (*(const f4*)(sm.agg + n * LD + f) + *(const f4*)(sm.agg1 + n * LD + f)) / W.normf;
        }
        if constexpr (STG) stage_wait();
        else __syncthreads();
      }
      STAMP(ST_MISC);
      node_gemm_x<HP, EPI_SILU, true, GN, NH, kAheadOne, kAheadOne, FL, SUM ? 2 : 0>(
          wb, wbe, G + 3 * PK, sm.h, xs0, !h_kept, G + 4 * PK, sm.agg, xs1, bn1, sm.p, nullptr, nullptr, mg.NC, wave, lane, tw,
          keep ? node_ctx_keep<HP>(hctx(), sm.hk, mg.NC) : hctx(), pf, G + 5 * PK, nullptr, nullptr, sm.agg1, W.normf);
      STAMP(ST_NODE);
      __syncthreads();
      STAMP(ST_BARRIER);
      vec_prefetch<NV, kThreads>(vpf, wb, s + 1 < W.S ? lay.gcl(l, s + 1) + 6 * PK : lay.equ(l) + 3 * PK,
                                 s + 1 < W.S ? 7 * HP + 16 : 5 * HP + 16, tid);
      if constexpr (STG) {
        stage_rows(xs0, sm.p, N * LD, wave, lane);
        stage_wait();
      }
      node_gemm_x<HP, EPI_RESIDUAL_MASK, false, GN, NH, kAheadOne, kAheadOne, FL>(wb, wbe, G + 5 * PK, sm.p, xs0, true, -1, nullptr, nullptr, bn2, sm.h, sm.h, mg.mask,
                                                       mg.NC, wave, lane, tw, hctx(), pf,
                                                       s + 1 < W.S ? lay.gcl(l, s + 1) : lay.equ(l));
      h_kept = false;
      STAMP(ST_NODE);
      __syncthreads();
      STAMP(ST_BARRIER);
    }
    {
      const int E = lay.equ(l);
      const int Wnext_edge = l + 1 < W.L ? lay.gcl(l + 1, 0) + 2 * PK : -1;
      vec_commit<NV, kThreads>(vpf, sm.vec, 5 * HP + 16, tid);
      if (tid < N) {
        sm.pmax[tid] = 0u;
        sm.qmax[tid] = 0u;
      }
      if constexpr (STG) {
        stage_rows(xs0, sm.h, N * LD, wave, lane);
        stage_wait();
      } else {
        __syncthreads();
      }
      STAMP(ST_STAGE);
      const float *cr = sm.vec, *cd = sm.vec + HP, *b1 = sm.vec + 2 * HP, *b2 = sm.vec + 3 * HP, *w3 = sm.vec + 4 * HP;
      const float crmax = sm.vec[5 * HP], cdmax = sm.vec[5 * HP + 1];
      {
        const NodeCtxH cx = keep ? node_ctx_keep<HP>(hctx(), sm.hk, mg.NC) : hctx();
        node_gemm_x<HP, EPI_NONE, false, GN, NH, kAheadOne, kAheadAll, FL>(wb, wbe, E, sm.h, xs0, !h_kept, -1, nullptr, nullptr, b1, sm.p, nullptr, nullptr, mg.NC,
                                                      wave, lane, tw, cx, pf, E + PK, nullptr, sm.pmax);
        h_kept = keep;
        node_gemm_x<HP, EPI_NONE, false, GN, NH, kAheadAll, kAheadOne, FL>(wb, wbe, E + PK, sm.h, xs0, false, -1, nullptr, nullptr, nullptr, sm.q, nullptr,
                                                      nullptr, mg.NC, wave, lane, tw, cx, pf, l + 1 < W.L ? lay.gcl(l + 1, 0) : -1, nullptr,
                                                      sm.qmax);
      }
      STAMP(ST_NODE);
      __syncthreads();
      STAMP(ST_BARRIER);
      if constexpr (RI) er_start<HP>(ring, wbe, E + 2 * PK, wave, lane);
// ... 88 lines not shown
```

gaudi_amd/csrc/w8_pred.h:

```cpp
#pragma once
#include "pred_device.h"
#include "w8_edm.h"

namespace gaudi {
namespace w8 {

template <int HP, int SP = 0, int GN = 0, bool PG = false>
struct PredSmem {
  static_assert(!(PG && GN != 0), "PG is a variant of the resident kernels");
  static_assert(!GN || SP != 0, "global node buffers: split edge GEMMs only (the fp32 form's publish buffer starts in b0 / b1)");
  static constexpr bool kGlobalNodes = GN != 0;
  float *b2, *b3, *b4;
  float *b0, *b1;
  float* ring;
  float* pub;
  float *x, *x0, *dx;
  uint32_t *pmax, *qmax;
  float* hsc;
  f4* geo;
  float *d0, *trans, *dd0;
  float* pred;
  float* vec;
  float* hk = nullptr;
  float* side = nullptr;
  __host__ __device__ static int floats(int N, int S, int pubx) {
    return EdgeRing<HP, SP>::kFloats + (GN ? gn_lds_buffers(GN) : PG ? 4 : 5) * N * (HP + 4) + pubx + 12 * N + 2 * align4(N) + 96 + S * 10 + 32 + 10 * HP;
  }
  __device__ __forceinline__ float* publish() const { return GN ? ring : b0; }
  __device__ void carve(float* base, int N, int S, int pubx, float* gnode = nullptr) {
    constexpr int LD = HP + 4;
    if (SP == 0) { ring = base; base += EdgeRing<HP, SP>::kFloats; }
    if (GN || PG) gnode = assume_global(gnode);
    float*& nb = GN ? gnode : base;
    if (GN == 2) { b2 = base; base += N * LD; } else { b2 = nb; nb += N * LD; }
    b3 = nb; nb += N * LD;
    if (PG) { b4 = gnode; gnode += N * LD; } else { b4 = nb; nb += N * LD; }
    b0 = nb; nb += N * LD;
    if (GN == 2) { b1 = base; base += N * LD; } else { b1 = nb; nb += N * LD; }
    if (SP != 0) { ring = base; base += EdgeRing<HP, SP>::kFloats; }
    pub = base; base += pubx;
    x = base; base += 4 * N;
    x0 = base; base += 4 * N;
    dx = base; base += 4 * N;
    pmax = (uint32_t*)base; base += align4(N);
    qmax = (uint32_t*)base; base += align4(N);
    hsc = base; base += 96;
    geo = (f4*)base; base += S * 4;
    d0 = base; base += S;
    trans = base; base += S * 4;
    dd0 = base; base += S;
    pred = base; base += 32;
    vec = base;
  }
};

__host__ __device__ inline long long pred_stash_floats8(int N, int HP, int L, int S) {
  return pred_stash_node_floats(N, HP, L) + (long long)L * S * HP * 2 + 2LL * L * S + (S > 16 * kWaves ? (long long)S * HP : 0);
}
__device__ __forceinline__ size_t edge_stash_off8(int l, int tile, int arr, int S, int HP) {
  return (((size_t)l * (S / 16) + tile) * 2 + arr) * (size_t)(16 * HP);
}

__host__ __device__ inline int pub_chunk_tiles(int S, long long avail_floats, int T) {
  int ch = (int)((avail_floats / (S > 0 ? S : 1) - 4) / 16);
  return ch > T ? T : ch;
}

template <int HP, int SP = 0, bool MR = false, int GN = 0, int FL = 0, int SD = 0, class SM = PredSmem<HP, SP, GN>>
__device__ __forceinline__ void pred_forward(const PredDev& W, const MolGraph& mg, const SM& sm, const float* sZ,
                                             float t_val, float* stash, float readout_div, int tid STAMP_DECL) {
  constexpr int LD = HP + 4;
  constexpr int T = HP / 16;
  const int wave = __builtin_amdgcn_readfirstlane(tid >> 6), lane = tid & 63, c = lane & 15, g = lane >> 4;
  const int N = mg.N, D = mg.D, F = W.F, F1 = F + 1, K = W.K, S = mg.S;
  PredLayout lay{HP, F1, K, W.L};
  const float* __restrict__ w = W.w;
  const WBuf wb = make_wbuf(W.w, W.w_bytes);
  const WBuf wbe = SP ? make_wbuf(W.ws, W.ws_bytes) : wb;
  const bool tw = W.ktail != 0;
  float *h = sm.b0, *p = sm.b1, *q = sm.b2, *agg = sm.b3, *agg1 = sm.b4;
  float* estash = stash + pred_stash_node_floats(N, HP, W.L);
  float* astash = estash + (size_t)W.L * S * HP * 2;
  float* pstash = astash + (size_t)W.L * S;

  for (int idx = tid; idx < N * 3; idx += kThreads) {
    const int n = idx / 3, d = idx % 3;
    const float v = sZ[n * D + d] * mg.mask[n];
    sm.x[4 * n + d] = v;
    sm.x0[4 * n + d] = v;
  }
  {
    const float* ew = w + lay.emb_w();
    const float* eb = w + lay.emb_b();
    for (int idx = tid; idx < N * HP; idx += kThreads) {
      const int n = idx / HP, f = idx % HP;
      float acc = 0.f;
      const float m = mg.mask[n];
      for (int k = 0; k < F; ++k) acc += gload(ew + f * F1 + k) * (sZ[n * D + 3 + k] * m);
      acc += gload(ew + f * F1 + F) * t_val;
      h[n * LD + f] = acc + gload(eb + f);
    }
  }
  __syncthreads();
  compute_geo(sm, mg, 0.f, tid, true);
  typename EdgeRing<HP, SP>::type ring;
  er_init<HP>(ring, sm.ring, W.ktail != 0, W.ws, W.hinv);
  constexpr bool NH = NodeMath<SP>::kF16;
  constexpr bool RI = node_ring_idle(HP, SP, GN);
  constexpr bool STG = GN && !NH;
  float* const xs0 = sm.ring;
  float* const xs1 = sm.ring + stage_stride(N * LD);
  if constexpr (!RI) er_start<HP>(ring, wbe, lay.layer(0) + 2 * HP * HP, wave, lane);
  typename NodePFSel<HP, NH>::type pf;
  node_prefetch_x<HP, NH, kAheadOne, FL>(pf, wb, wbe, lay.layer(0), mg.NC, wave, lane, tw);
  auto hctx = [&]() {
    if constexpr (NH) {
      if constexpr (RI) return node_ctx_h<HP>(sm.ring, EdgeRing<HP, SP>::kFloats, mg.NC, W.hinv, tw, sm.hsc);
      else return node_ctx_h<HP>(ring.slot(ring.par ^ 1), EdgeRing<HP, SP>::kFloats / 2, mg.NC, W.hinv, tw, sm.hsc);
    } else {
      return NodeCtxH{1.f, nullptr, nullptr, tw, nullptr};
    }
  };
  const bool keep = NH && sm.hk != nullptr;
  constexpr bool kSideA = (SD & 1) != 0;
  static_assert(!kSideA || (NH && !MR && GN == 0 && !RI && node_one_tile(FL)), "the side job is a form of the resident N1 kernel");
  constexpr int NV = (PredLayerW::vec_count(HP) + kThreads - 1) / kThreads;
  VecPF<NV> vpf;
  vec_prefetch<NV, kThreads>(vpf, wb, PredLayerW::vec_off(lay.layer(0), HP), PredLayerW::vec_count(HP), tid);

  for (int l = 0; l < W.L; ++l) {
    const bool last = l == W.L - 1;
    const PredLayerW Lw(w, lay.layer(l), HP, sm.vec);
    const bool side_l = kSideA && sm.side != nullptr && !last && (tw || !SplitGeo<HP, SP == 0 ? 1 : SP>::kTailOK);
    vec_commit<NV, kThreads>(vpf, sm.vec, PredLayerW::vec_count(HP), tid);
    if constexpr (STG) stage_rows(xs0, h, N * LD, wave, lane);
    for (int idx = tid; idx < N * LD; idx += kThreads) {
      agg[idx] = 0.f;
      agg1[idx] = 0.f;
    }
    if (tid < N) {
      sm.pmax[tid] = 0u;
      sm.qmax[tid] = 0u;
    }
    float* st = stash + (size_t)l * (3 * N * HP + 4 * N);
    for (int idx = tid; idx < N; idx += kThreads) gstore4((f4*)(st + 3 * N * HP) + idx, *(const f4*)(sm.x + 4 * idx));
    compute_geo(sm, mg, 1.0f, tid, false);
    if constexpr (STG) stage_wait();
    else __syncthreads();
    STAMP(ST_STAGE);
    {
      const NodeCtxH cx = keep ? node_ctx_keep<HP>(hctx(), sm.hk, mg.NC) : hctx();
      node_gemm_x<HP, EPI_NONE, false, GN, NH, kAheadOne, kAheadAll, FL>(wb, wbe, Lw.A, h, xs0, true, -1, nullptr, nullptr, Lw.b1, p, nullptr, nullptr, mg.NC, wave,
                                                    lane, tw, cx, pf, Lw.Bm, nullptr, sm.pmax);
      node_gemm_x<HP, EPI_NONE, false, GN, NH, kAheadAll, kAheadOne, FL>(wb, wbe, Lw.Bm, h, xs0, false, -1, nullptr, nullptr, nullptr, q, nullptr, nullptr, mg.NC,
                                                    wave, lane, tw, cx, pf, side_l ? Lw.Wn1a : Lw.Wn1h, nullptr, sm.qmax);
    }
    STAMP(ST_NODE);
    __syncthreads();
    STAMP(ST_BARRIER);
    if constexpr (RI) er_start<HP>(ring, wbe, Lw.W2, wave, lane);
    for (int idx = tid; idx < N * (HP / 4); idx += kThreads) {
      const int n = idx / (HP / 4), f = 4 * (idx % (HP / 4));
      nstash_store((f4*)st + idx, *(const f4*)(p + n * LD + f));
      nstash_store((f4*)(st + N * HP) + idx, *(const f4*)(q + n * LD + f));
    }
    STAMP(ST_STASH);
    int rd = 0;
    if (side_l && wave == kWaves - 1) {
      if constexpr (kSideA) {
        constexpr int n = side_trip_count<HP, SP>();
        SideJobH<HP> job;
        const SideArgsH sa{wbe, Lw.Wn1h, Lw.bn1, SplitBufH{sm.hk + kScaleFloatsH, 1, sm.hk}, W.hinv, sm.side, mg.NC};
        side_issue<HP, 0>(job, sa, lane);
        side_trips<HP, SP, 0>(ring, wbe, split_off(Lw.W2), split_off(Lw.Wc1), lane, job, sa);
        side_trips<HP, SP, n>(ring, wbe, split_off(Lw.Wc1), split_off(lay.layer(l + 1) + 2 * HP * HP), lane, job, sa);
        side_rest<HP, 2 * n>(job, sa, lane);
      }
    } else
    {
    pred_fwd_round:
      const bool more = MR && rd + 1 < mg.rounds;
      const TileCols tc = load_tile(mg, MR ? rd : 0, wave, c);
      const f4 gg = sm.geo[tc.slot];
      f4 acc[T];
      const float d0f = sm.d0[tc.slot];
      const float ub = __builtin_bit_cast(float, sm.pmax[tc.i]) + __builtin_bit_cast(float, sm.qmax[tc.j]) + sm.vec[9 * HP + 1] * gg[0] +
                       sm.vec[9 * HP + 2] * fabsf(d0f);
      er_gemm_pq<HP>(acc, ring, wbe, Lw.W2, last ? (more ? Lw.W2 : -1) : Lw.Wc1, Lw.b2, Lw.cr, Lw.cd, p + tc.i * LD + 4 * g,
                       q + tc.j * LD + 4 * g, gg[0], d0f, ub, tc.active, wave, lane STAMP_ARGS);
      STAMP(ST_EDGE);
      const int tile = tc.slot >> 4;
      if (tc.active) {
        {
          f4* sv = (f4*)(estash + edge_stash_off8(l, tile, 0, S, HP)) + lane;
#pragma unroll
          for (int t = 0; t < T; ++t) stash_store(sv + t * 64, acc[t]);
        }
        float sdot = 0.f;
#pragma unroll
        for (int t = 0; t < T; ++t) {
          const f4 m = silu4v(acc[t]);
          acc[t] = m;
          sdot += dot4(m, *(const f4*)(Lw.wa + 16 * t + 4 * g));
        }
        float a = 1.f;
        if (W.attention) a = sigmoid_f(reduce_groups(sdot) + Lw.ba);
        if (g == 0) gstore(astash + (size_t)l * S + tc.slot, a);
        const float sc = a * tc.mk;
#pragma unroll
        for (int t = 0; t < T; ++t) acc[t] = acc[t] * sc;
        scatter_runs<HP>(acc, tc, agg, agg1, g);
      }
      STAMP(ST_EDGE_EPI);
      if (!last) {
        f4 cp[T];
        er_gemm_regs<HP>(cp, acc, ring, wbe, Lw.Wc1, more ? Lw.W2 : (RI ? -1 : lay.layer(l + 1) + 2 * HP * HP), Lw.bc1, nullptr,
                         tc.active, wave, lane);
        STAMP(ST_EDGE);
        if (tc.active) {
          f4* sc = (f4*)(estash + edge_stash_off8(l, tile, 1, S, HP)) + lane;
          float sdot = 0.f;
#pragma unroll
          for (int t = 0; t < T; ++t) {
            const f4 sg = sigmoid4v(cp[t]);
            const f4 ds = sg * (splat(1.0f) + cp[t] * (splat(1.0f) - sg)), sl = cp[t] * sg;
            stash_store(sc + t * 64, ds);
            sdot += dot4(sl, *(const f4*)(Lw.wc2 + 16 * t + 4 * g));
          }
          const float phi = reduce_groups(sdot);
          if (g == 0) gstore(pstash + (size_t)l * S + tc.slot, phi);
          const float tau = (W.use_tanh ? tanhf(phi) * W.coords_range_layer : phi) * tc.mk;
          if (g == 0) *(f4*)(sm.trans + 4 * tc.slot) = (f4){gg[1] * tau, gg[2] * tau, gg[3] * tau, 0.f};
        }
        STAMP(ST_EDGE_EPI);
      }
      if constexpr (MR) {
        if (++rd < mg.rounds) goto pred_fwd_round;
      }
    }
    __syncthreads();
    STAMP(ST_BARRIER);
    constexpr bool SUM = NH && GN == 0;
    if constexpr (!SUM) {
      if constexpr (STG) stage_rows(xs0, h, N * LD, wave, lane);
      for (int idx = tid; idx < N * (HP / 4); idx += kThreads) {
        const int n = idx / (HP / 4), f = 4 * (idx % (HP / 4));
        if constexpr (STG)
          *(f4*)(xs1 + n * LD + f) = *(const f4*)(agg + n * LD + f) + *(const f4*)(agg1 + n * LD + f);
        else
          *(f4*)(agg + n * LD + f) = *(const f4*)(agg + n * LD + f) + *(const f4*)(agg1 + n * LD + f);
      }
      if constexpr (STG) stage_wait();
      else __syncthreads();
    }
    STAMP(ST_MISC);
    if constexpr (kSideA) {
      if (side_l)
        node_gemm_h<HP, EPI_SILU, false, 1, kAheadOne, kAheadOne, FL, nh_odd(HP) ? kTailOne : kTailRuntime, node_slots<HP>(FL)>(
            wbe, Lw.Wn1a, RowsSum<false>{agg, agg1, 1.f}, true, -1, (const float*)nullptr, nullptr, p, nullptr, nullptr, mg.NC, wave, lane,
            hctx(), pf, Lw.Wn2, st + 2 * N * HP , nullptr, nullptr, YInitRows{sm.side});
    }
    if (!side_l)
    node_gemm_x<HP, EPI_SILU, true, GN, NH, kAheadOne, kAheadOne, FL, SUM ? 1 : 0>(
        wb, wbe, Lw.Wn1h, h, xs0, !keep, Lw.Wn1a, agg, xs1, Lw.bn1, p, nullptr, nullptr, mg.NC, wave, lane, tw,
        keep ? node_ctx_keep<HP>(hctx(), sm.hk, mg.NC) : hctx(), pf, Lw.Wn2, st + 2 * N * HP , nullptr, agg1);
    STAMP(ST_NODE);
    __syncthreads();
    STAMP(ST_BARRIER);
    vec_prefetch<NV, kThreads>(vpf, wb, PredLayerW::vec_off(lay.layer(l + 1 < W.L ? l + 1 : l), HP), PredLayerW::vec_count(HP), tid);
    if constexpr (STG) {
      stage_rows(xs0, p, N * LD, wave, lane);
      stage_wait();
    }
    node_gemm_x<HP, EPI_RESIDUAL_MASK, false, GN, NH, kAheadOne, kAheadOne, FL>(wb, wbe, Lw.Wn2, p, xs0, true, -1, nullptr, nullptr, Lw.bn2, h, h, mg.mask, mg.NC, wave,
                                                     lane, tw, hctx(), pf, l + 1 < W.L ? lay.layer(l + 1) : -1);
    if (!last) coord_update(sm, mg, 1.0f, tid);
    STAMP(ST_NODE);
    __syncthreads();
    STAMP(ST_BARRIER);
  }
  {
    const float* ow = w + lay.out_w();
    const float* ob = w + lay.out_b();
    const float* msk = mg.mask;
    small_dots<kThreads>(
        N * K, HP, tid, [=](int qq, int f) { return gload(ow + (qq % K) * HP + f); },
        [=](int qq, int f) { return h[(qq / K) * LD + f]; },
        [=](int qq, float acc) { p[qq] = (acc + gload(ob + qq % K)) * msk[qq / K]; });
    __syncthreads();
    if (tid < K) {
      float s = 0.f;
      for (int n = 0; n < N; ++n) s += p[n * K + tid];
      sm.pred[tid] = s / readout_div;
    }
    __syncthreads();
  }
  STAMP(ST_X0);
}

template <int HP, int SP = 0, bool MR = false, int GN = 0, int FL = 0, class SM = PredSmem<HP, SP, GN>>
__device__ __forceinline__ void pred_backward(const PredDev& W, const MolGraph& mg, const SM& sm, const float* stash,
                                              float* sGrad, float readout_div, int pub_ch, int tid STAMP_DECL, const float* sZin = nullptr) {
  constexpr int LD = HP + 4;
  constexpr int T = HP / 16;
  const int wave = __builtin_amdgcn_readfirstlane(tid >> 6), lane = tid & 63, c = lane & 15, g = lane >> 4;
  const int N = mg.N, D = mg.D, F = W.F, F1 = F + 1, K = W.K, S = mg.S;
  PredLayout lay{HP, F1, K, W.L};
  const float* __restrict__ w = W.w;
  const WBuf wb = make_wbuf(W.w, W.w_bytes);
  const WBuf wbe = SP ? make_wbuf(W.ws, W.ws_bytes) : wb;
  const bool tw = W.ktail != 0;
  float *B0 = sm.b0, *B1 = sm.b1, *B2 = sm.b2, *dh = sm.b3, *B4 = sm.b4;
  const int tid_ = tid;
  float* pub = sm.publish();
  const int PLD = 16 * pub_ch + 4;
  const float* estash = stash + pred_stash_node_floats(N, HP, W.L);
  const float* astash = estash + (size_t)W.L * S * HP * 2;
  const float* pstash = astash + (size_t)W.L * S;
  const float* dpred = sm.pred + 16;
  const int nslots = mg.ntiles * 16;
  f4* dus = (f4*)const_cast<float*>(pstash + (size_t)W.L * S);

  if (sZin != nullptr) {
    for (int idx = tid; idx < N * 3; idx += kThreads) {
      const int n = idx / 3, d = idx % 3;
      const float v = sZin[n * D + d] * mg.mask[n];
      sm.x[4 * n + d] = v;
      sm.x0[4 * n + d] = v;
    }
    __syncthreads();
    compute_geo(sm, mg, 0.f, tid, true);
    __syncthreads();
  }
  {
    const float* ow = w + lay.out_w();
    for (int idx = tid; idx < N * HP; idx += kThreads) {
      const int n = idx / HP, f = idx % HP;
      float acc = 0.f;
      for (int k = 0; k < K; ++k) acc += (dpred[k] / readout_div) * gload(ow + k * HP + f);
      dh[n * LD + f] = acc * mg.mask[n];
    }
    for (int idx = tid; idx < N * 4; idx += kThreads) sm.dx[idx] = 0.f;
    for (int idx = tid; idx < S; idx += kThreads) sm.dd0[idx] = 0.f;
  }
  __syncthreads();

  typename EdgeRing<HP, SP>::type ring;
  er_init<HP>(ring, sm.ring, W.ktail != 0, W.ws, W.hinv);
  constexpr bool NH = NodeMath<SP>::kF16;
  constexpr bool RI = node_ring_idle(HP, SP, GN);
  constexpr bool STG = GN && !NH;
  float* const xs0 = sm.ring;
  float* const xs1 = sm.ring + stage_stride(N * LD);
  if constexpr (!RI) {
    const int L0 = lay.layer(W.L - 1);
    er_start<HP>(ring, wbe, L0 + 9 * HP * HP , wave, lane);
  }
  typename NodePFSel<HP, NH>::type pf;
  node_prefetch_x<HP, NH, kAheadOne, FL>(pf, wb, wbe, lay.layer(W.L - 1) + 13 * HP * HP , mg.NC, wave, lane, tw);
  auto hctx = [&]() {
    if constexpr (NH) {
      if constexpr (RI) return node_ctx_h<HP>(sm.ring, EdgeRing<HP, SP>::kFloats, mg.NC, W.hinv, tw, sm.hsc);
      else return node_ctx_h<HP>(ring.slot(ring.par ^ 1), EdgeRing<HP, SP>::kFloats / 2, mg.NC, W.hinv, tw, sm.hsc);
    } else {
      return NodeCtxH{1.f, nullptr, nullptr, tw, nullptr};
    }
  };
  constexpr int NV = (PredLayerW::vec_count(HP) + kThreads - 1) / kThreads;
  VecPF<NV> vpf;
  vec_prefetch<NV, kThreads>(vpf, wb, PredLayerW::vec_off(lay.layer(W.L - 1), HP), PredLayerW::vec_count(HP), tid);
  STAMP(ST_X1);
  for (int l = W.L - 1; l >= 0; --l) {
    const bool last = l == W.L - 1;
    const PredLayerW Lw(w, lay.layer(l), HP, sm.vec);
    const float* st = stash + (size_t)l * (3 * N * HP + 4 * N);
    {
      const int tid = fresh(tid_);
      const int n4 = N * (HP / 4);
#ifdef GAUDI_DIAG_HOT_STASH
      const f4* sp = (const f4*)W.w;
      const f4* sq = (const f4*)(W.w + N * HP);
      const f4* sn = (const f4*)(W.w + 2 * N * HP);
#else
      const f4* sp = (const f4*)st;
      const f4* sq = (const f4*)(st + N * HP);
      const f4* sn = (const f4*)(st + 2 * N * HP);
#endif
      const int i0 = tid < n4 ? tid : n4 - 1, i1 = tid + kThreads < n4 ? tid + kThreads : n4 - 1;
      const f4 xv = gload4((const f4*)(st + 3 * N * HP) + (tid < N ? tid : N - 1));
      const f4 p0 = nstash_load(sp + i0), q0 = nstash_load(sq + i0), v0 = nstash_load(sn + i0);
      const f4 p1 = nstash_load(sp + i1), q1 = nstash_load(sq + i1), v1 = nstash_load(sn + i1);
      vec_commit<NV, kThreads>(vpf, sm.vec, PredLayerW::vec_count(HP), tid);
      STAMP(ST_GUIDE);
      auto put = [&](int idx, f4 pv, f4 qv, f4 nv) {
        const int n = idx / (HP / 4), f = 4 * (idx % (HP / 4));
        *(f4*)(B2 + n * LD + f) = pv;
        *(f4*)(B1 + n * LD + f) = qv;
        *(f4*)(B4 + n * LD + f) = nv;
        *(f4*)(dh + n * LD + f) = *(const f4*)(dh + n * LD + f) * mg.mask[n];
      };
      if (tid < N) {
        *(f4*)(sm.x + 4 * tid) = xv;
        *(f4*)(sm.dx + 4 * tid) = *(const f4*)(sm.dx + 4 * tid) * mg.mask[tid];
      }
      if (tid < n4) put(tid, p0, q0, v0);
      if (tid + kThreads < n4) put(tid + kThreads, p1, q1, v1);
      for (int idx = tid + 2 * kThreads; idx < n4; idx += kThreads) put(idx, nstash_load(sp + idx), nstash_load(sq + idx), nstash_load(sn + idx));
      for (int idx = tid + kThreads; idx < N; idx += kThreads) {
        *(f4*)(sm.x + 4 * idx) = gload4((const f4*)(st + 3 * N * HP) + idx);
        *(f4*)(sm.dx + 4 * idx) = *(const f4*)(sm.dx + 4 * idx) * mg.mask[idx];
      }
    }
    STAMP(ST_PRED_IO);
    __syncthreads();
    if constexpr (STG) stage_rows(xs0, dh, N * LD, wave, lane);
    compute_geo(sm, mg, 1.0f, tid, false);
    if constexpr (STG) stage_wait();
    STAMP(ST_BWD_EDGE);
    node_gemm_x<HP, EPI_MUL_DSILU, false, GN, NH, kAheadOne, kAheadOne, FL>(wb, wbe, Lw.Wn2t, dh, xs0, true, -1, nullptr, nullptr, nullptr, STG ? xs1 : B4, B4, nullptr,
                                                 mg.NC, wave, lane, tw, hctx(), pf, Lw.Wn1ht);
    __syncthreads();
    {
      const NodeCtxH cx = hctx();
      node_gemm_x<HP, EPI_ACCUM, false, GN, NH, kAheadOne, kAheadAll, FL>(wb, wbe, Lw.Wn1ht, B4, xs1, true, -1, nullptr, nullptr, nullptr, dh, dh, nullptr, mg.NC,
                                                     wave, lane, tw, cx, pf, Lw.Wn1at);
      node_gemm_x<HP, EPI_NONE, false, GN, NH, kAheadAll, 0, FL>(wb, wbe, Lw.Wn1at, B4, xs1, false, -1, nullptr, nullptr, nullptr, B0, nullptr, nullptr,
                                                    mg.NC, wave, lane, tw, cx, pf);
    }
    __syncthreads();
    STAMP(ST_BWD_NODE);
    if constexpr (RI) er_start<HP>(ring, wbe, last ? Lw.W2t : Lw.Wc1t, wave, lane);
    {
      constexpr bool mr = MR;
      int rd = 0;
    pred_bwd_round:
      const bool more = MR && rd + 1 < mg.rounds;
      const TileCols tc = load_tile(mg, MR ? rd : 0, wave, c);
      const int tile = tc.slot >> 4;
      const f4 gg = sm.geo[tc.slot];
      const float d0v = sm.d0[tc.slot];
      f4 du[T];
      float a = 0.f, tau = 0.f, dtx = 0.f, dty = 0.f, dtz = 0.f;
      {
        f4 de[T];
        if (tc.active) {
          a = gload(astash + (size_t)l * S + tc.slot);
          dtx = sm.dx[4 * tc.i + 0];
          dty = sm.dx[4 * tc.i + 1];
          dtz = sm.dx[4 * tc.i + 2];
        }
        if (!last) {
          f4 cp[T];
          if (tc.active) {
#ifdef GAUDI_DIAG_HOT_STASH
            const f4* sc = (const f4*)(W.w + (size_t)tile * (T * 256)) + lane;
#else
            const f4* sc = (const f4*)(estash + edge_stash_off8(l, tile, 1, S, HP)) + lane;
#endif
#pragma unroll
            for (int t = 0; t < T; ++t) cp[t] = stash_load(sc + t * 64);
            const float phi = gload(pstash + (size_t)l * S + tc.slot);
            const float th = tanhf(phi);
            tau = W.use_tanh ? th * W.coords_range_layer : phi;
            const float dtau = (dtx * gg[1] + dty * gg[2] + dtz * gg[3]) * tc.mk;
            const float dphi = W.use_tanh ? dtau * W.coords_range_layer * (1.0f - th * th) : dtau;
#pragma unroll
            for (int t = 0; t < T; ++t)
              cp[t] = *(const f4*)(Lw.wc2 + 16 * t + 4 * g) * dphi * cp[t];
          } else {
#pragma unroll
            for (int t = 0; t < T; ++t) cp[t] = splat(0.f);
          }
          STAMP(ST_B_DCP);
          er_gemm_regs<HP>(de, cp, ring, wbe, Lw.Wc1t, Lw.W2t, nullptr, B0 + tc.i * LD ,
                             tc.active, wave, lane);
          STAMP(ST_B_DE);
        } else {
#pragma unroll
          for (int t = 0; t < T; ++t) de[t] = *(const f4*)(B0 + tc.i * LD + 16 * t + 4 * g);
        }
        if (tc.active) {
          f4 ve[T];
#ifdef GAUDI_DIAG_HOT_STASH
          const f4* sv = (const f4*)(W.w + (size_t)(8 + tile) * (T * 256)) + lane;
#else
          const f4* sv = (const f4*)(estash + edge_stash_off8(l, tile, 0, S, HP)) + lane;
#endif
#pragma unroll
          for (int t = 0; t < T; ++t) ve[t] = stash_load(sv + t * 64);
          float dadot = 0.f;
#pragma unroll
          for (int t = 0; t < T; ++t) dadot += dot4(de[t], silu4v(ve[t]));
          const float da = reduce_groups(dadot) * tc.mk;
          const float ds = W.attention ? da * a * (1.0f - a) : 0.f;
          const float am = a * tc.mk;
#pragma unroll
          for (int t = 0; t < T; ++t)
            de[t] = (de[t] * am + *(const f4*)(Lw.wa + 16 * t + 4 * g) * ds) * dsilu4v(ve[t]);
        }
        STAMP(ST_B_DV);
        er_gemm_regs<HP>(du, de, ring, wbe, Lw.W2t,
// ... 233 lines not shown
```

gaudi_amd/csrc/w8_split.h:

```cpp
#pragma once
#include "w8_common.h"
#ifndef GAUDI_EDGE_PRIO
#define GAUDI_EDGE_PRIO 0
#endif


namespace gaudi {
namespace w8 {

typedef _Float16 h8 __attribute__((ext_vector_type(8)));
typedef _Float16 h2 __attribute__((ext_vector_type(2)));
typedef __attribute__((ext_vector_type(2))) float f2;
typedef __attribute__((ext_vector_type(4))) uint32_t u4;
typedef __attribute__((ext_vector_type(2))) uint32_t u2;
constexpr int kPieces = 2;

template <int N, class F>
__device__ __forceinline__ void static_for(F f) {
  if constexpr (N > 0) {
    static_for<N - 1>(f);
    f(std::integral_constant<int, N - 1>{});
  }
}

struct B3 {
  u4 h, l;
};

__device__ __forceinline__ uint32_t pk_f16(float a, float b) {
  return __builtin_bit_cast(uint32_t, __builtin_convertvector((f2){a, b}, h2));
}
__device__ __forceinline__ f2 unpk_f16(uint32_t p) { return __builtin_convertvector(__builtin_bit_cast(h2, p), f2); }
__device__ __forceinline__ uint32_t umax(uint32_t a, uint32_t b) { return a > b ? a : b; }
__device__ __forceinline__ uint32_t absbits(float v) { return __builtin_bit_cast(uint32_t, v) & 0x7fffffffu; }
struct Pow2Scale {
  float s, inv;
};
__device__ __forceinline__ Pow2Scale scale_for(uint32_t maxbits) {
  int k = 141 - (int)(maxbits >> 23);
  k = k > 126 ? 126 : k;
  return Pow2Scale{__builtin_bit_cast(float, (uint32_t)(k + 127) << 23), __builtin_bit_cast(float, (uint32_t)(127 - k) << 23)};
}
struct P3 {
  uint32_t h, l;
};
__device__ __forceinline__ P3 split2(float a, float b) {
  P3 r;
  r.h = pk_f16(a, b);
  const f2 f = unpk_f16(r.h);
  r.l = pk_f16(a - f[0], b - f[1]);
  return r;
}
__device__ __forceinline__ B3 split8(const f4 lo, const f4 hi, float s) {
  const f4 ls = lo * s, hs = hi * s;
  auto sp = [s](float a, float b, float as, float bs) {
    P3 r;
    r.h = pk_f16(as, bs);
    const f2 f = unpk_f16(r.h);
    r.l = pk_f16(__builtin_fmaf(a, s, -f[0]), __builtin_fmaf(b, s, -f[1]));
    return r;
  };
  const P3 p0 = sp(lo[0], lo[1], ls[0], ls[1]), p1 = sp(lo[2], lo[3], ls[2], ls[3]), p2 = sp(hi[0], hi[1], hs[0], hs[1]),
           p3 = sp(hi[2], hi[3], hs[2], hs[3]);
  B3 r;
  r.h = (u4){p0.h, p1.h, p2.h, p3.h};
  r.l = (u4){p0.l, p1.l, p2.l, p3.l};
  return r;
}
__device__ __forceinline__ f4 mfma_bf(const u4 a, const u4 b, const f4 c) {
  return __builtin_amdgcn_mfma_f32_16x16x32_f16(__builtin_bit_cast(h8, a), __builtin_bit_cast(h8, b), c, 0, 0, 0);
}
__device__ __forceinline__ uint32_t column_max(uint32_t v) {
  v = umax(v, (uint32_t)__shfl_xor((int)v, 16));
  v = umax(v, (uint32_t)__shfl_xor((int)v, 32));
  return v;
}

template <int HP, int MODE>
struct SplitGeo {
  static_assert(MODE == 1 || MODE == 2, "split mode");
  static constexpr int T = HP / 16;
  static constexpr int NC = (T + 1) / 2;
  static constexpr int CH = (MODE == 2 || NC == 1) && T > 1 ? (T + 1) / 2 : T;
  static constexpr int NH = (T + CH - 1) / CH;
  static constexpr int kTrips = NC * NH;
  static constexpr int kUnit = 256;
  static constexpr int kSlotFloats = CH * kPieces * kUnit;
  static constexpr int kMatFloats = NC * T * kPieces * kUnit;
  static constexpr int UT = (CH * kPieces + kWaves - 1) / kWaves;
  static constexpr bool kTailOK = (T & 1) && T >= 3;
  static constexpr int kTripsTail = (NC - 1) * NH + 1;
  static_assert(!kTailOK || T <= CH * kPieces, "the fp32 tail tiles must fit one ring slot");
  __host__ __device__ static constexpr int tiles_of(int h) { return (h + 1) * CH <= T ? CH : T - h * CH; }
};

template <int HP, int MODE>
struct RingS {
  using G = SplitGeo<HP, MODE>;
  float* base;
  int par;
  bool ktail;
  const float* gbase;
  float winv;
  __device__ __forceinline__ float* slot(int p) const { return base + p * G::kSlotFloats; }
};

template <int HP, int MODE>
__device__ __forceinline__ bool trip_group(const RingS<HP, MODE>& r, int W, int nextW, int tr, int& off, int& units) {
  using G = SplitGeo<HP, MODE>;
  const bool tail = G::kTailOK && r.ktail;
  const int n = tail ? G::kTripsTail : G::kTrips;
  const bool nxt = tr >= n;
  const int t2 = nxt ? tr - n : tr;
  const int base = nxt ? nextW : W;
  if (tail && t2 == n - 1) {
    units = G::T;
    off = base + (G::NC - 1) * G::T * kPieces * G::kUnit;
  } else {
    const int m = t2 / G::NH, h = t2 % G::NH;
    units = G::tiles_of(h) * kPieces;
    off = base + (m * G::T + h * G::CH) * kPieces * G::kUnit;
  }
  off = __builtin_amdgcn_readfirstlane(off);
  units = __builtin_amdgcn_readfirstlane(units);
  asm volatile("" : "+s"(units));
  return !(nxt && nextW < 0);
}
template <int U, int UT, int kBytes>
__device__ __forceinline__ void dma_units(const WBuf& wb, int soff_bytes, int lane, float* l, int count) {
  if constexpr (U < UT) {
    if (U < count)
      __builtin_amdgcn_raw_ptr_buffer_load_lds(wb.r, (__attribute__((address_space(3))) void*)l, 16, lane * 16, soff_bytes, U * kBytes, 0);
    dma_units<U + 1, UT, kBytes>(wb, soff_bytes, lane, l, count);
  }
}
template <int HP, int MODE>
__device__ __forceinline__ bool rings_dma(const RingS<HP, MODE>& r, const WBuf& wb, float* slot, int W, int nextW, int tr, int wave, int lane) {
  using G = SplitGeo<HP, MODE>;
  int off, units;
  if (!trip_group(r, W, nextW, tr, off, units)) return false;
  static_assert(G::UT * G::kUnit * 4 <= 4096, "a wave's units must lie within the immediate offset of its first");
  const int first = (unsigned)(wave * units) / kWaves, count = (unsigned)((wave + 1) * units) / kWaves - first;
  dma_units<0, G::UT, G::kUnit * 4>(wb, (off + first * G::kUnit) * 4, lane, slot + first * G::kUnit, count);
  return true;
}
template <int HP, int MODE>
__device__ __forceinline__ void rings_start(RingS<HP, MODE>& r, const WBuf& wb, int W, int wave, int lane) {
  rings_dma(r, wb, r.slot(r.par), W, -1, 0, wave, lane);
}
template <int HP, int MODE>
__device__ __forceinline__ void rings_stage(RingS<HP, MODE>& r, const WBuf& wb, int W, int nextW, int tr, int wave, int lane) {
  rings_dma(r, wb, r.slot(r.par ^ 1), W, nextW, tr + 1, wave, lane);
}

template <int HP, int MODE>
__host__ __device__ constexpr int side_trip_count() {
  return SplitGeo<HP, MODE>::kTailOK ? SplitGeo<HP, MODE>::kTripsTail : SplitGeo<HP, MODE>::kTrips;
}
template <int HP, int MODE, int TR>
struct RingsStageSide {
__device__ __forceinline__ static void run(const RingS<HP, MODE>& r, const WBuf& wb, int W, int nextW, int lane) {
  using G = SplitGeo<HP, MODE>;
  constexpr int n = side_trip_count<HP, MODE>();
  constexpr bool nxt = TR + 1 >= n;
  constexpr int t2 = nxt ? TR + 1 - n : TR + 1;
  constexpr bool tt = G::kTailOK && t2 == n - 1;
  constexpr int units = tt ? G::T : G::tiles_of(t2 % G::NH) * kPieces;
  constexpr int rel = tt ? (G::NC - 1) * G::T * kPieces * G::kUnit : ((t2 / G::NH) * G::T + (t2 % G::NH) * G::CH) * kPieces * G::kUnit;
  constexpr int first = (unsigned)((kWaves - 1) * units) / kWaves, count = units - first;
  static_assert(count <= G::UT, "the side wave's share of a group");
  const int vo = lane * 16;
  const int off = __builtin_amdgcn_readfirstlane(((nxt ? nextW : W) + rel + first * G::kUnit) * 4);
  float* const l = r.slot(r.par ^ 1) + first * G::kUnit;
  static_for<count>([&](auto u_tag) {
    constexpr int U = decltype(u_tag)::value;
    __builtin_amdgcn_raw_ptr_buffer_load_lds(wb.r, (__attribute__((address_space(3))) void*)l, 16, vo, off, U * G::kUnit * 4, 0);
  });
}
};
template <int PENDING>
__device__ __forceinline__ void side_barrier() {
  asm volatile("s_waitcnt vmcnt(%0) lgkmcnt(0)" ::"n"(PENDING) : "memory");
  __builtin_amdgcn_s_barrier();
  asm volatile("" ::: "memory");
}

__device__ __forceinline__ void trip_barrier() {
  asm volatile("s_waitcnt vmcnt(0)" ::: "memory");
  __syncthreads();
}
template <int HP, int MODE>
__device__ __forceinline__ void trip_open(RingS<HP, MODE>& r, int lane) {
  (void)r;
  (void)lane;
  trip_barrier();
}
template <int HP, int MODE>
__device__ __forceinline__ void trip_close(RingS<HP, MODE>& r, int lane) {
  (void)lane;
  r.par ^= 1;
}

template <int HP, int MODE, int NT, bool ACT, class MID>
__device__ __forceinline__ void rings_mfma_act(f4* acc, const float* slot_lane, const B3& b, MID mid) {
  constexpr int U = SplitGeo<HP, MODE>::kUnit;
  if constexpr (!ACT) {
    mid();
    return;
  }
  constexpr int kAhead = NT > 2 ? 2 : 1, kSets = kAhead + 1;
  f4 a[kSets][kPieces];
#pragma unroll
  for (int q = 0; q < kAhead; ++q)
#pragma unroll
    for (int p = 0; p < kPieces; ++p) a[q][p] = *(const f4*)(slot_lane + (q * kPieces + p) * U);
  static_for<NT>([&](auto t_tag) {
    constexpr int t = decltype(t_tag)::value;
    constexpr int cur = t % kSets;
    if (t == NT / 2) {
      mid();
      __builtin_amdgcn_sched_barrier(0);
    }
    if (t == (NT - 2 > NT / 2 ? NT - 2 : NT - 1)) __builtin_amdgcn_sched_barrier(0);
    if (t + kAhead < NT) {
#pragma unroll
      for (int p = 0; p < kPieces; ++p) a[(t + kAhead) % kSets][p] = *(const f4*)(slot_lane + ((t + kAhead) * kPieces + p) * U);
    }
    __builtin_amdgcn_sched_barrier(0);
    {
      const u4 ah = __builtin_bit_cast(u4, a[cur][0]), al = __builtin_bit_cast(u4, a[cur][1]);
      f4 c = acc[t];
      c = mfma_bf(al, b.h, c);
      c = mfma_bf(ah, b.l, c);
      c = mfma_bf(ah, b.h, c);
      acc[t] = c;
    }
    __builtin_amdgcn_sched_barrier(0);
  });
}
template <int HP, int MODE, int NT, class MID>
__device__ __forceinline__ void rings_mfma(f4* acc, const float* slot_lane, const B3& b, bool active, MID mid) {
  if (active) rings_mfma_act<HP, MODE, NT, true>(acc, slot_lane, b, mid);
  else rings_mfma_act<HP, MODE, NT, false>(acc, slot_lane, b, mid);
}

template <int HP, int MODE, class MID>
__device__ __forceinline__ void rings_mfma_tail(f4 (&acc)[HP / 16], const float* slot_lane, float b, bool active, MID mid) {
  constexpr int T = HP / 16;
  float a[T];
#pragma unroll
  for (int t = 0; t < T; ++t) a[t] = slot_lane[t * SplitGeo<HP, MODE>::kUnit];
  __builtin_amdgcn_sched_barrier(0);
#pragma unroll
  for (int t = 0; t < T; ++t) {
    if (t == T / 2) {
      mid();
      __builtin_amdgcn_sched_barrier(0);
    }
    if (active) acc[t] = mfma1(a[t], b, acc[t]);
  }
  __builtin_amdgcn_sched_barrier(0);
}

template <int HP, int MODE>
__device__ __forceinline__ void edge_gemm_pq_s(f4 (&acc)[HP / 16], RingS<HP, MODE>& ring, const WBuf& wb, int W, int nextW,
                                               const float* sB2, const float* sCr, const float* sCd, const float* pp,
                                               const float* qq, float r, float d0, float ubound, bool active, int wave, int lane) {
  using G = SplitGeo<HP, MODE>;
  constexpr int T = G::T;
  const int g = lane >> 4;
#pragma unroll
  for (int t = 0; t < T; ++t) acc[t] = splat(0.f);
  const Pow2Scale sc = scale_for(absbits(ubound));
  const float se = sc.s;
  auto gen = [&](int m) {
    const f4 lo = silu4v(edge_u(pp, qq, sCr, sCd, g, 2 * m, r, d0));
    const f4 hi = 2 * m + 1 < T ? silu4v(edge_u(pp, qq, sCr, sCd, g, 2 * m + 1 < T ? 2 * m + 1 : 0, r, d0)) : splat(0.f);
    return split8(lo, hi, se);
  };
  B3 bin = gen(0), nb = bin;
  static_assert(G::NH <= 3, "at most three trips per K chunk");
  const bool tail = G::kTailOK && ring.ktail;
#if GAUDI_EDGE_PRIO & 1
  if (wave >= kWaves / 2) __builtin_amdgcn_s_setprio(1);
#endif
  auto chunk = [&](int m, const B3& bin, B3& nb) {
    const int mn = m + 1 < G::NC ? m + 1 : m;
    auto trip = [&](auto h_tag) {
      constexpr int h = decltype(h_tag)::value;
      constexpr int NT = G::tiles_of(h);
      const int tr = m * G::NH + h;
      trip_open(ring, lane);
      rings_mfma<HP, MODE, NT>(acc + h * G::CH, ring.slot(ring.par) + lane * 4, bin, active, [&] {
        rings_stage(ring, wb, W, nextW, tr, wave, lane);
        if (h == G::NH - 1) nb = gen(mn);
      });
      trip_close(ring, lane);
    };
    trip(std::integral_constant<int, 0>{});
    if constexpr (G::NH > 1) trip(std::integral_constant<int, 1>{});
    if constexpr (G::NH > 2) trip(std::integral_constant<int, 2>{});
  };
  const int full = tail ? G::NC - 1 : G::NC;
  int m = 0;
#pragma unroll 1
  for (; m + 1 < full; m += 2) {
    chunk(m, bin, nb);
    chunk(m + 1, nb, bin);
  }
  if (m < full) chunk(m, bin, nb);
  if constexpr (G::kTailOK) {
    if (tail) {
      trip_open(ring, lane);
      const float bt = silu_f(edge_u_tail(pp, qq, sCr, sCd, g, T, r, d0)[0]) * se;
      rings_mfma_tail<HP, MODE>(acc, ring.slot(ring.par) + lane * 4, bt, active,
                          [&] { rings_stage(ring, wb, W, nextW, G::kTripsTail - 1, wave, lane); });
      trip_close(ring, lane);
    }
  }
#if GAUDI_EDGE_PRIO & 1
  __builtin_amdgcn_s_setprio(0);
#endif
  const float dsc = sc.inv * ring.winv;
#pragma unroll
  for (int t = 0; t < T; ++t) acc[t] = acc[t] * dsc + *(const f4*)(sB2 + 16 * t + 4 * g);
}

template <int HP, int MODE>
__device__ __forceinline__ void edge_gemm_regs_s(f4 (&out)[HP / 16], const f4 (&in)[HP / 16], RingS<HP, MODE>& ring, const WBuf& wb,
                                                 int W, int nextW, const float* sBias, const float* rowinit, bool active,
                                                 int wave, int lane) {
  using G = SplitGeo<HP, MODE>;
  constexpr int T = G::T;
  const int g = lane >> 4;
  uint32_t mx = 0;
#pragma unroll
  for (int t = 0; t < T; ++t) {
    out[t] = splat(0.f);
    mx = umax(mx, umax(umax(absbits(in[t][0]), absbits(in[t][1])), umax(absbits(in[t][2]), absbits(in[t][3]))));
  }
  const Pow2Scale sc = scale_for(column_max(mx));
  const float se = sc.s;
  static_assert(G::NH <= 3, "at most three trips per K chunk");
  const int c = lane & 15;
#if GAUDI_EDGE_PRIO & 2
  if (wave >= kWaves / 2) __builtin_amdgcn_s_setprio(1);
#endif
  auto chunk = [&](auto m_tag) {
    constexpr int m = decltype(m_tag)::value;
    const B3 bin = split8(in[2 * m], 2 * m + 1 < T ? in[2 * m + 1 < T ? 2 * m + 1 : 0] : splat(0.f), se);
    auto trip = [&](auto h_tag) {
      constexpr int h = decltype(h_tag)::value;
      constexpr int tr = m * G::NH + h;
      trip_open(ring, lane);
      rings_mfma<HP, MODE, G::tiles_of(h)>(out + h * G::CH, ring.slot(ring.par) + lane * 4, bin, active,
                                           [&] { rings_stage(ring, wb, W, nextW, tr, wave, lane); });
      trip_close(ring, lane);
    };
    trip(std::integral_constant<int, 0>{});
    if constexpr (G::NH > 1) trip(std::integral_constant<int, 1>{});
    if constexpr (G::NH > 2) trip(std::integral_constant<int, 2>{});
  };
  auto finish = [&] {
#if GAUDI_EDGE_PRIO & 2
    __builtin_amdgcn_s_setprio(0);
#endif
    const float dsc = sc.inv * ring.winv;
#pragma unroll
    for (int t = 0; t < T; ++t) {
      f4 b = sBias != nullptr ? *(const f4*)(sBias + 16 * t + 4 * g) : splat(0.f);
      if (rowinit != nullptr) b = b + *(const f4*)(rowinit + 16 * t + 4 * g);
      out[t] = out[t] * dsc + b;
    }
  };
  static_for<G::NC - 1>([&](auto m_tag) { chunk(m_tag); });
  if constexpr (G::kTailOK) {
    if (ring.ktail) {
      trip_open(ring, lane);
      rings_mfma_tail<HP, MODE>(out, ring.slot(ring.par) + lane * 4, tail_to_b(in[T - 1], c, g)[0] * se, active,
                          [&] { rings_stage(ring, wb, W, nextW, G::kTripsTail - 1, wave, lane); });
      trip_close(ring, lane);
      finish();
      return;
    }
  }
  chunk(std::integral_constant<int, G::NC - 1>{});
  finish();
}

template <int HP, int SP>
struct EdgeRing {
  using type = RingS<HP, SP>;
  static constexpr int kFloats = 2 * SplitGeo<HP, SP>::kSlotFloats;
};
template <int HP>
struct EdgeRing<HP, 0> {
  using type = Ring<HP>;
  static constexpr int kFloats = 2 * (HP / 16) * 256;
};
__host__ __device__ constexpr int edge_ring_floats(int HP, int mode) {
  const int T = HP / 16;
  const int CH = (mode == 2 || (T + 1) / 2 == 1) && T > 1 ? (T + 1) / 2 : T;
  return mode ? 2 * CH * kPieces * 256 : 2 * T * 256;
}
static_assert(edge_ring_floats(32, 1) == EdgeRing<32, 1>::kFloats && edge_ring_floats(208, 1) == EdgeRing<208, 1>::kFloats &&
                  edge_ring_floats(48, 2) == EdgeRing<48, 2>::kFloats && edge_ring_floats(208, 2) == EdgeRing<208, 2>::kFloats,
              "host LDS planning and SplitGeo disagree");
__device__ __forceinline__ int split_off(int W) { return W < 0 ? -1 : 2 * W; }

template <int HP>
__device__ __forceinline__ void er_init(Ring<HP>& r, float* base, bool ktail, const float*, float) {
  r.base = base;
  r.par = 0;
  r.ktail = ktail;
}
template <int HP, int MODE>
__device__ __forceinline__ void er_init(RingS<HP, MODE>& r, float* base, bool ktail, const float* ws, float winv) {
  r.base = base;
  r.par = 0;
  r.ktail = ktail;
  r.gbase = ws;
  r.winv = winv;
}
template <int HP>
__device__ __forceinline__ void er_start(Ring<HP>& r, const WBuf& wb, int W, int wave, int lane) {
  ring_start<HP>(r, wb, W, wave, lane);
}
template <int HP, int MODE>
__device__ __forceinline__ void er_start(RingS<HP, MODE>& r, const WBuf& wb, int W, int wave, int lane) {
  rings_start(r, wb, split_off(W), wave, lane);
}
template <int HP>
__device__ __forceinline__ void er_gemm_pq(f4 (&acc)[HP / 16], Ring<HP>& ring, const WBuf& wb, int W, int nextW, const float* sB2,
                                           const float* sCr, const float* sCd, const float* pp, const float* qq, float r, float d0,
                                           float, bool active, int wave, int lane STAMP_DECL) {
  edge_gemm_pq<HP>(acc, ring, wb, W, nextW, sB2, sCr, sCd, pp, qq, r, d0, active, wave, lane STAMP_ARGS);
}
template <int HP, int MODE>
__device__ __forceinline__ void er_gemm_pq(f4 (&acc)[HP / 16], RingS<HP, MODE>& ring, const WBuf& wb, int W, int nextW, const float* sB2,
                                           const float* sCr, const float* sCd, const float* pp, const float* qq, float r, float d0,
                                           float ubound, bool active, int wave, int lane STAMP_DECL) {
  edge_gemm_pq_s(acc, ring, wb, split_off(W), split_off(nextW), sB2, sCr, sCd, pp, qq, r, d0, ubound, active, wave, lane);
}
template <int HP>
__device__ __forceinline__ void er_gemm_regs(f4 (&out)[HP / 16], const f4 (&in)[HP / 16], Ring<HP>& ring, const WBuf& wb, int W,
                                             int nextW, const float* sBias, const float* rowinit, bool active, int wave, int lane) {
  edge_gemm_regs<HP>(out, in, ring, wb, W, nextW, sBias, rowinit, active, wave, lane);
}
template <int HP, int MODE>
__device__ __forceinline__ void er_gemm_regs(f4 (&out)[HP / 16], const f4 (&in)[HP / 16], RingS<HP, MODE>& ring, const WBuf& wb, int W,
                                             int nextW, const float* sBias, const float* rowinit, bool active, int wave, int lane) {
  edge_gemm_regs_s(out, in, ring, wb, split_off(W), split_off(nextW), sBias, rowinit, active, wave, lane);
}

}
}
```

gaudi_amd/engine.py:

```python
from __future__ import annotations

import ctypes as C

import numpy as np

from . import _lib
from ._lib import TARGET_CB, TARGET_CBZ, Diag, EdmConfig, GaudiError, PredConfig, f32, fptr


def _strip(sd: dict) -> dict:
    out = {}
    for k, v in sd.items():
        if hasattr(v, "detach"):
            v = v.detach().cpu().numpy()
        out[k[7:] if k.startswith("module.") else k] = f32(v)
    return out


def _noise_power(schedule: str) -> float:
    if schedule == "cosine":
        return 0.0
    parts = str(schedule).split("_")
    try:
        power = float(parts[1]) if len(parts) == 2 and parts[0] == "polynomial" else 0.0
    except ValueError:
        power = 0.0
    if not power > 0:
        raise GaudiError(f"unsupported diffusion_noise_schedule {schedule!r}: 'polynomial_<p>' and 'cosine' are implemented "
                         "(the 'learned' schedule is training-only in the reference)")
    return power


def target_spec(spec, B: int, K: int):
    if not isinstance(spec, dict):
        if callable(getattr(spec, "spec", None)):
            spec = spec.spec()
        else:
            raise GaudiError("a target spec is a dict with any of w, q, c, side, scale, window (or a ValueTarget), "
                             f"got {type(spec).__name__}")
    unknown = set(spec) - {"w", "q", "c", "side", "scale", "window"}
    if unknown:
        raise GaudiError(f"unknown target spec entries {sorted(unknown)}")
    cs = _lib.TargetSpec()
    keep = []

    def arr(name, dtype):
        a = spec.get(name)
        if a is None:
            return None, 0
        a = np.ascontiguousarray(np.asarray(a), dtype=dtype)
        if a.shape == (K,):
            per = 0
        elif a.shape == (B, K):
            per = 1
        else:
            raise GaudiError(f"target spec '{name}' must be [K] = {(K,)} or [B,K] = {(B, K)}, got {a.shape}")
        keep.append(a)
        return a, per

    cs.K = K
    for name in ("w", "q", "c"):
        a, per = arr(name, np.float32)
        setattr(cs, name, None if a is None else a.ctypes.data_as(_lib.FP))
        setattr(cs, name + "_per_mol", per)
    sd = spec.get("side")
    if sd is not None and not np.all(np.asarray(sd) == np.round(np.asarray(sd, np.float64))):
        raise GaudiError("target spec 'side' must hold -1 (lower bound), 0 (value) or +1 (upper bound)")
    a, per = arr("side", np.int32)
    cs.side = None if a is None else a.ctypes.data_as(_lib.IP)
    cs.side_per_mol = per
    sc = spec.get("scale")
    if sc is not None:
        per = np.ndim(sc) > 0
        sc = np.asarray(sc, np.float32)
        if sc.shape != ((B,) if per else ()):
            raise GaudiError(f"target spec 'scale' must be a number or [B] = {(B,)}, got {sc.shape}")
        sc = np.ascontiguousarray(sc.reshape(-1))
        keep.append(sc)
        cs.scale = sc.ctypes.data_as(_lib.FP)
        cs.scale_per_mol = 1 if per else 0
    win = spec.get("window")
    if win is not None:
        cs.t_lo, cs.t_hi = int(win[0]), int(win[1])
        if cs.t_lo == 0 and cs.t_hi == 0:
            raise GaudiError("the guidance window must lie inside 1..T")
    return cs, keep


def host_target_seed(spec, pred) -> np.ndarray:
    p = f32(pred)
    if p.ndim != 2:
        raise GaudiError(f"pred must be [B,K], got {p.shape}")
    B, K = p.shape
    cs, keep = target_spec(spec, B, K)
    out = np.empty_like(p)
    rc = _lib.load_library().gaudi_host_target_seed(C.byref(cs), B, K, fptr(p), fptr(out))
    del keep
    if rc != 0:
        raise GaudiError(f"gaudi_host_target_seed failed ({rc}): side must be -1 / 0 / +1 and every parameter finite")
    return out


class Engine:
    def __init__(self, device: int = 0):
        self.lib = _lib.load_library()
        self.h = C.c_void_p()
        rc = self.lib.gaudi_create(int(device), C.byref(self.h))
        if rc != 0:
            raise GaudiError(f"gaudi_create(device={device}) failed with code {rc} (no usable HIP device?)")
        self.device = device
        self.edm_args = None
        self.pred_args = None
        self.fix_noise = False
        self.F = None
        self.K = None

    _default = None

    @classmethod
    def default(cls, device: int = 0) -> "Engine":
        if cls._default is None or not cls._default.h:
            cls._default = cls(device)
        return cls._default

    def close(self):
        if getattr(self, "h", None) is not None and self.h:
            self.lib.gaudi_destroy(self.h)
            self.h = C.c_void_p()

    def __del__(self):
        try:
            self.close()
        except Exception:
            pass

    def _warning(self):
        fn = getattr(self.lib, "gaudi_last_warning", None)
        if fn is None or fn.restype is not C.c_char_p:
            return ""
        msg = fn(self.h)
        return msg.decode() if msg else ""

    def _note_fallback(self):
        w = self._warning()
        if w and w != getattr(self, "_fallback_reason", None):
            import warnings
            warnings.warn("gaudi_amd: " + w, RuntimeWarning, stacklevel=3)
        if w:
            self._fallback_reason = w

    def profile_clock_mhz(self) -> float:
        fn = getattr(self.lib, "gaudi_profile_clock", None)
        if fn is None or not fn.argtypes:
            return 0.0
        v = C.c_double(0.0)
        self._check(fn(self.h, C.byref(v)), "gaudi_profile_clock")
        return float(v.value)

    def last_kernel_key(self) -> str:
        fn = getattr(self.lib, "gaudi_last_kernel_key", None)
        if fn is None or not fn.argtypes:
            return ""
        buf = C.create_string_buffer(256)
        self._check(fn(self.h, buf, len(buf)), "gaudi_last_kernel_key")
        return buf.value.decode()

    def kernel_keys_launched(self) -> list:
        fn = getattr(self.lib, "gaudi_kernel_key_log", None)
        if fn is None or not fn.argtypes:
            return []
        return _lib.key_lines(fn, self.h)

    def keep_h(self) -> int:
        fn = getattr(self.lib, "gaudi_last_keep_h", None)
        if fn is None or not fn.argtypes:
            return 0
        n = C.c_int32(0)
        self._check(fn(self.h, C.byref(n)), "gaudi_last_keep_h")
        return int(n.value)

    def family_split(self) -> int:
        fn = getattr(self.lib, "gaudi_last_family_split", None)
        if fn is None or not fn.argtypes:
            return 0
        n = C.c_int32(0)
        self._check(fn(self.h, C.byref(n)), "gaudi_last_family_split")
        return int(n.value)

    def _check(self, rc: int, what: str):
        if rc != 0:
            msg = self.lib.gaudi_last_error(self.h)
            raise GaudiError(f"{what} failed ({rc}): {msg.decode() if msg else ''}")

    def _tensor_args(self, sd: dict):
        names = list(sd.keys())
        arrs = [sd[k] for k in names]
        n = len(names)
        c_names = (C.c_char_p * n)(*[k.encode() for k in names])
        c_ptrs = (_lib.FP * n)(*[fptr(a) for a in arrs])
        c_numel = (C.c_int64 * n)(*[a.size for a in arrs])
        return n, c_names, c_ptrs, c_numel, arrs

    def load_edm(self, args: dict, state_dict: dict):
        agg = args.get("aggregation_method", "sum")
        if agg not in ("sum", "mean"):
            raise GaudiError(f"unknown aggregation_method {agg!r}")
        sd = _strip(state_dict)
        emb = sd.get("dynamics.egnn.embedding.weight")
        if emb is None:
            raise GaudiError("state dict has no dynamics.egnn.embedding.weight (mode='gnn_dynamics' is unsupported)")
        F = emb.shape[1] - 1
        from .checkpoint import normalize_factors
        nv = normalize_factors(args)
        cfg = EdmConfig(F, int(args["nf"]), int(args["n_layers"]), int(args.get("inv_sublayers", 1)),
                        int(bool(args["attention"])), int(bool(args["tanh"])), float(args["coords_range"]),
                        float(args["norm_constant"]), float(args.get("normalization_factor", 1)) if agg == "sum" else 0.0,
                        int(args["diffusion_steps"]), _noise_power(args["diffusion_noise_schedule"]),
                        float(args["diffusion_noise_precision"]), (C.c_float * 3)(*[float(v) for v in nv]),
                        int(bool(args.get("sin_embedding", False))))
        n, c_names, c_ptrs, c_numel, keep = self._tensor_args(sd)
        self._check(self.lib.gaudi_load_edm(self.h, C.byref(cfg), n, c_names, c_ptrs, c_numel), "gaudi_load_edm")
        self._note_fallback()
        self.edm_args, self.F, self.T = dict(args), F, int(args["diffusion_steps"])
        self.edm_names = list(sd.keys())
        self.edm_shapes = [sd[k].shape for k in self.edm_names]
        self._edm_train_sd = None
        sigma_0 = float(np.sqrt(1.0 / (1.0 + np.exp(-np.float64(self.gamma()[0])))))
        max_norm = max(float(nv[1]), float(nv[2]))
        if sigma_0 * 8 > 1.0 / max_norm:
            raise GaudiError(f"Value for normalization value {max_norm} probably too large with sigma_0 {sigma_0:.5f} and "
                             f"1 / norm_value = {1.0 / max_norm} (en_diffusion.py:336-349: the reference raises the same)")

    def load_predictor(self, args: dict, state_dict: dict):
        sd = _strip(state_dict)
        emb = sd["egnn.embedding.weight"]
        F = emb.shape[1] - 1
        K = sd["egnn.embedding_out.weight"].shape[0]
        cfg = PredConfig(F, K, int(args["nf"]), int(args["n_layers"]), int(bool(args["attention"])),
                         int(bool(args["tanh"])), float(args["coords_range"]))
        n, c_names, c_ptrs, c_numel, keep = self._tensor_args(sd)
        self._check(self.lib.gaudi_load_predictor(self.h, C.byref(cfg), n, c_names, c_ptrs, c_numel),
                    "gaudi_load_predictor")
        reason = getattr(self, "_fallback_reason", None)
        if reason and reason.startswith("predictor weights") and self._warning() != reason:
            self._fallback_reason = None
        self._note_fallback()
        self.pred_args, self.K = dict(args), K
        self.pred_names = list(sd.keys())
        self.pred_shapes = [sd[k].shape for k in self.pred_names]

    edm_sync = None

    def _sync_edm(self, sampler: bool = True):
        if self.edm_sync is not None:
            self.edm_sync()
        if sampler and getattr(self, "_edm_train_sd", None) is not None:
            sd, self._edm_train_sd = self._edm_train_sd, None
            self.load_edm(self.edm_args, sd)

    pred_sync = None

    def _sync_pred(self):
        if self.pred_sync is not None:
            self.pred_sync()

    def gamma(self) -> np.ndarray:
        g = np.empty(self.T + 1, np.float32)
        self._check(self.lib.gaudi_get_gamma(self.h, fptr(g)), "gaudi_get_gamma")
        return g

    def step_coefficients(self) -> np.ndarray:
        c = np.empty((self.T, 4), np.float32)
        self._check(self.lib.gaudi_get_step_coefficients(self.h, fptr(c)), "gaudi_get_step_coefficients")
        return c

    @staticmethod
    def _masks(node_mask, edge_mask, B, N):
        nm = f32(node_mask).reshape(B, N)
        em = f32(edge_mask).reshape(B, N, N)
        return nm, em

    def phi(self, z, t, node_mask, edge_mask) -> np.ndarray:
        self._sync_edm()
        z = f32(z)
        B, N, D = z.shape
        nm, em = self._masks(node_mask, edge_mask, B, N)
        t = f32(np.broadcast_to(np.asarray(t, np.float32).reshape(-1), (B,)))
        out = np.empty_like(z)
        self._check(self.lib.gaudi_phi(self.h, B, N, fptr(z), fptr(t), fptr(nm), fptr(em), fptr(out)), "gaudi_phi")
        return out

    def predictor_fwd(self, z, t, node_mask, edge_mask) -> np.ndarray:
        self._sync_pred()
        z = f32(z)
        B, N, D = z.shape
        nm, em = self._masks(node_mask, edge_mask, B, N)
        t = f32(np.broadcast_to(np.asarray(t, np.float32).reshape(-1), (B,)))
        out = np.empty((B, self.K), np.float32)
        self._check(self.lib.gaudi_predictor_fwd(self.h, B, N, fptr(z), fptr(t), fptr(nm), fptr(em), fptr(out)),
                    "gaudi_predictor_fwd")
        return out

    def predictor_grad(self, z, t, node_mask, edge_mask, dpred):
        self._sync_pred()
        z = f32(z)
        B, N, D = z.shape
        nm, em = self._masks(node_mask, edge_mask, B, N)
        t = f32(np.broadcast_to(np.asarray(t, np.float32).reshape(-1), (B,)))
        dp = f32(np.broadcast_to(np.asarray(dpred, np.float32), (B, self.K)))
        pred = np.empty((B, self.K), np.float32)
        grad = np.empty_like(z)
        self._check(self.lib.gaudi_predictor_grad(self.h, B, N, fptr(z), fptr(t), fptr(nm), fptr(em), fptr(dp),
                                                  fptr(pred), fptr(grad)), "gaudi_predictor_grad")
        return pred, grad

    def step(self, s_idx, z_t, node_mask, edge_mask, eps_raw, target_w=None, scale=1.0, t_idx=None) -> np.ndarray:
        self._sync_edm()
        self._sync_pred()
# ... 538 lines not shown
```

include/gaudi_hip.h:

```cpp
#ifndef GAUDI_HIP_H
#define GAUDI_HIP_H

#include <stdint.h>

#ifdef __cplusplus
extern "C" {
#endif

#define GAUDI_OK 0
#define GAUDI_E_INVALID (-1)
#define GAUDI_E_HIP (-2)
#define GAUDI_E_STATE (-3)
#define GAUDI_E_MISSING (-4)
#define GAUDI_E_CAPACITY (-5)

typedef struct gaudi_handle gaudi_handle;

typedef struct {
  int32_t in_node_nf;
  int32_t hidden_nf;
  int32_t n_layers;
  int32_t inv_sublayers;
  int32_t attention;
  int32_t tanh;
  float coords_range;
  float norm_constant;
  float normalization_factor;
  int32_t diffusion_steps;
  float noise_power;
  float noise_precision;
  float norm_values[3];
  int32_t sin_embedding;
} gaudi_edm_config;

typedef struct {
  int32_t in_nf;
  int32_t out_nf;
  int32_t hidden_nf;
  int32_t n_layers;
  int32_t attention;
  int32_t tanh;
  float coords_range;
} gaudi_pred_config;

typedef struct {
  float max_masked_leak;
  float max_cog_rel;
  float max_cog_abs;
  int32_t nan_count;
  int32_t reprojected;
} gaudi_diag;

int gaudi_create(int device, gaudi_handle** out);
void gaudi_destroy(gaudi_handle* h);
const char* gaudi_last_error(const gaudi_handle* h);
const char* gaudi_last_warning(const gaudi_handle* h);
int gaudi_last_kernel_key(const gaudi_handle* h, char* buf, int n);
int gaudi_kernel_key_log(const gaudi_handle* h, char* buf, int n);
int gaudi_host_kernel_keys(char* buf, int n);
#define GAUDI_ABI_VERSION 7
int gaudi_abi_version(void);

int gaudi_load_edm(gaudi_handle* h, const gaudi_edm_config* cfg, int n, const char* const* names,
                   const float* const* tensors, const int64_t* numel);
int gaudi_load_predictor(gaudi_handle* h, const gaudi_pred_config* cfg, int n, const char* const* names,
                         const float* const* tensors, const int64_t* numel);

int gaudi_get_gamma(gaudi_handle* h, float* gamma_out );
int gaudi_get_step_coefficients(gaudi_handle* h, float* coef_out );

int gaudi_phi(gaudi_handle* h, int B, int N, const float* z, const float* t ,
              const float* node_mask, const float* edge_mask, float* eps_out);

int gaudi_predictor_fwd(gaudi_handle* h, int B, int N, const float* z, const float* t ,
                        const float* node_mask, const float* edge_mask, float* pred_out );
int gaudi_predictor_grad(gaudi_handle* h, int B, int N, const float* z, const float* t, const float* node_mask,
                         const float* edge_mask, const float* dpred , float* pred_out ,
                         float* grad_out );

int gaudi_predict_noised(gaudi_handle* h, int B, int N, const float* x, const float* onehot, const int32_t* t_int,
                         const float* node_mask, const float* edge_mask, uint64_t seed, int64_t sample_offset,
                         const float* noise, float* zt_out , float* pred_out );

int gaudi_predictor_loss_grad(gaudi_handle* h, int B, int N, const float* x, const float* onehot, const int32_t* t_int,
                              const float* node_mask, const float* edge_mask, const float* y , uint64_t seed,
                              int64_t sample_offset, const float* noise , float* loss_out ,
                              float* pred_out , float* grad_out, int32_t* has_grad_out);
int gaudi_predictor_grad_size(gaudi_handle* h, int64_t* n_floats);

int gaudi_edm_loss_grad(gaudi_handle* h, int B, int N, const float* x, const float* onehot, const int32_t* t_int,
                        const float* node_mask, const float* edge_mask, uint64_t seed, int64_t sample_offset,
                        const float* noise , int loss_type, const float* weight ,
                        float* loss_out , float* net_out , float* grad_out ,
                        int32_t* has_grad_out);
int gaudi_edm_grad_size(gaudi_handle* h, int64_t* n_floats);
int gaudi_edm_set_train_weights(gaudi_handle* h, int n, const char* const* names, const float* const* tensors,
                                const int64_t* numel);

int gaudi_edm_nll(gaudi_handle* h, int B, int N, const float* x, const float* onehot, const int32_t* t_int, const float* node_mask,
                  const float* edge_mask, uint64_t seed, int64_t sample_offset, const float* noise ,
                  float* nll_out , float* terms_out );

int gaudi_step(gaudi_handle* h, int B, int N, int s_idx, const float* z_t, const float* node_mask,
               const float* edge_mask, const float* eps_raw, const float* target_w ,
               float scale, float* zs_out);

int gaudi_decode(gaudi_handle* h, int B, int N, const float* z0, const float* node_mask, const float* edge_mask,
                 const float* eps_raw, float* x_out , float* onehot_out );

int gaudi_sample(gaudi_handle* h, int B, int N, const float* node_mask, const float* edge_mask, uint64_t seed,
                 int64_t sample_offset, const float* noise, float std, const float* target_w ,
                 float scale, float* x_out , float* onehot_out ,
                 float* z0_out , gaudi_diag* diag );

int gaudi_sample_grid(gaudi_handle* h, int B, int N, const float* node_mask, const float* edge_mask, uint64_t seed,
                      int64_t sample_offset, const float* noise, float std, const float* target_w , float scale,
                      int n_grid, const int32_t* grid, const float* x0 , const float* onehot0 ,
                      float* x_out, float* onehot_out, float* z0_out , float* zt_out ,
                      gaudi_diag* diag );

typedef struct {
  int32_t K;
  const float* w;
  const float* q;
  const float* c;
  const int32_t* side;
  const float* scale;
  int32_t w_per_mol, q_per_mol, c_per_mol, side_per_mol, scale_per_mol;
  int32_t t_lo, t_hi;
} gaudi_target_spec;

int gaudi_sample_target(gaudi_handle* h, int B, int N, const float* node_mask, const float* edge_mask, uint64_t seed,
                        int64_t sample_offset, const float* noise, float std, const gaudi_target_spec* spec, int n_grid,
                        const int32_t* grid , const float* x0 , const float* onehot0 ,
                        float* x_out, float* onehot_out, float* z0_out , float* zt_out ,
                        float* trace_out , gaudi_diag* diag );
int gaudi_step_target(gaudi_handle* h, int B, int N, int s_idx, int t_idx, const float* z_t, const float* node_mask,
                      const float* edge_mask, const float* eps_raw, const gaudi_target_spec* spec, float* zs_out,
                      float* trace_out );
int gaudi_host_target_seed(const gaudi_target_spec* spec, int B, int K, const float* pred, float* out);

int gaudi_step_pair(gaudi_handle* h, int B, int N, int s_idx, int t_idx, const float* z_t, const float* node_mask,
                    const float* edge_mask, const float* eps_raw, const float* target_w , float scale,
                    float* zs_out);

int gaudi_host_grid_coefficients(int T, float noise_power , float noise_precision, int n_grid,
                                 const int32_t* grid, float* coef_out, int32_t* land_out);

typedef void (*gaudi_target_cb)(void* user, int B, int K, const float* pred, float t, float* dT_dpred_out);
int gaudi_sample_cb(gaudi_handle* h, int B, int N, const float* node_mask, const float* edge_mask, uint64_t seed,
                    int64_t sample_offset, const float* noise, float std, gaudi_target_cb target_grad, void* user,
                    float scale, float* x_out, float* onehot_out, float* z0_out, gaudi_diag* diag);

typedef void (*gaudi_target_cbz)(void* user, int B, int N, int D, int K, const float* z_s, const float* pred, float t,
                                 float* dT_dpred_out, float* dT_dz_out);
int gaudi_sample_cbz(gaudi_handle* h, int B, int N, const float* node_mask, const float* edge_mask, uint64_t seed,
                     int64_t sample_offset, const float* noise, float std, gaudi_target_cbz target_grad, void* user,
                     float scale, float* x_out, float* onehot_out, float* z0_out, gaudi_diag* diag);

int gaudi_sample_cb_grid(gaudi_handle* h, int B, int N, const float* node_mask, const float* edge_mask, uint64_t seed,
                         int64_t sample_offset, const float* noise, float std, gaudi_target_cb target_grad,
                         gaudi_target_cbz target_grad_z, void* user, float scale, int n_grid, const int32_t* grid,
                         const float* x0, const float* onehot0, float* x_out, float* onehot_out, float* z0_out, float* zt_out,
                         gaudi_diag* diag);

int gaudi_sample_chain(gaudi_handle* h, int B, int N, const float* node_mask, const float* edge_mask, uint64_t seed,
                       int64_t sample_offset, const float* noise, float std, int keep_frames, float* chain_out);

typedef struct {
  int32_t n_types;
  int32_t orientation;
  int32_t check_dihedrals;
  double tol;
  double min_dist;
  double dist_lo[16][16], dist_hi[16][16];
  int32_t a3_count[16];
  double a3_lo[16][4], a3_hi[16][4];
  double a4_0, a4_180;
} gaudi_ring_tables;

typedef struct {
  int32_t n_rings;
  int32_t n_edges;
  int32_t n_triplets;
  int32_t n_nan_angles;
  float a3_min, a3_max;
  float a4_min, a4_max;
} gaudi_stability_aux;

int gaudi_check_stability(gaudi_handle* h, const gaudi_ring_tables* tables, int B, int N, const float* x,
                          const int32_t* ring_type, const int32_t* n_nodes, uint8_t* flags_out,
                          float* dist_out , float* adj_out ,
                          gaudi_stability_aux* aux_out );
int gaudi_stability_profile_get(gaudi_handle* h, int32_t* n_launches, double* total_ms);

#define GAUDI_ATOMS_MAX_ATOMS 384
#define GAUDI_ATOMS_MAX_BONDS 384
typedef struct {
  int32_t n_types;
  int32_t ring_size[16];
  int32_t ring_elem[16][6];
  double templ[16][6][2];
  int32_t no_orientation[16];
  double extra_angle[16];
  int32_t n_template_h[16];
  int32_t template_h_parent[16][2];
  int32_t h_elem, c_elem;
  double h_bond;
} gaudi_atom_tables;

// ... 187 lines not shown
```

Measured before the change: 229.3.

## Dedicate the idle wave to prefetch edge-weight ring slots for single-tile graphs

When a graph occupies fewer node tiles than waves in the 8-wave single-tile path, the wave with no MFMA work becomes a loader that issues all buffer-to-LDS loads for the next ring slot, and the active waves skip their share of staging. The aim is to take global-to-LDS weight streaming off the compute waves so their MFMA chain is not interrupted. It adds a per-launch ktail flag bit, a loader role toggled per layer around side work, and compile-time knobs for sharing and priority. The risk is that one wave issuing every load may serialize the transfer and miss the next trip's deadline.

```diff
diff --git a/gaudi_amd/_lib.py b/gaudi_amd/_lib.py
--- a/gaudi_amd/_lib.py
+++ b/gaudi_amd/_lib.py
@@ -180,6 +180,7 @@
     "gaudi_last_warning": (C.c_char_p, [C.c_void_p]),
     "gaudi_last_kernel_key": (C.c_int, [C.c_void_p, C.c_char_p, C.c_int]),
     "gaudi_kernel_key_log": (C.c_int, [C.c_void_p, C.c_char_p, C.c_int]),
+    "gaudi_last_ring_loader": (C.c_int, [C.c_void_p]),
     "gaudi_host_kernel_keys": (C.c_int, [C.c_char_p, C.c_int]),
     "gaudi_abi_version": (C.c_int, []),
     "gaudi_last_family_split": (C.c_int, [C.c_void_p, C.POINTER(C.c_int32)]),
@@ -229,6 +230,7 @@
                "gaudi_fp_profile_get")
 _SUB_EXPORTS = ("gaudi_substructure_search", "gaudi_substructure_profile_get")
 _KEY_EXPORTS = ("gaudi_last_kernel_key", "gaudi_kernel_key_log", "gaudi_host_kernel_keys")
+_LOADER_EXPORTS = ("gaudi_last_ring_loader",)
 
 _lib = None
 
@@ -250,7 +252,7 @@
         raise GaudiError(f"{LIB_PATH} exports ABI version {abi}, this package expects {ABI_VERSION}: rebuild it "
                          "(`python -m gaudi_amd.build --force`)")
     for name, (res, args) in EXPORTS.items():
-        if lenient and not hasattr(lib, name) and (name.startswith("gaudi_host_") or name in _ROUND6_EXPORTS + _NLL_EXPORTS + _GRID_EXPORTS + _TARGET_EXPORTS + _ATOMS_EXPORTS + _RINGS_EXPORTS + _BONDS_EXPORTS + _CANON_EXPORTS + _FP_EXPORTS + _SUB_EXPORTS + _KEY_EXPORTS):
+        if lenient and not hasattr(lib, name) and (name.startswith("gaudi_host_") or name in _ROUND6_EXPORTS + _NLL_EXPORTS + _GRID_EXPORTS + _TARGET_EXPORTS + _ATOMS_EXPORTS + _RINGS_EXPORTS + _BONDS_EXPORTS + _CANON_EXPORTS + _FP_EXPORTS + _SUB_EXPORTS + _KEY_EXPORTS + _LOADER_EXPORTS):
             continue
         if lenient and abi != ABI_VERSION and name.startswith("gaudi_host_"):
             continue
diff --git a/gaudi_amd/csrc/gaudi_hip.hip b/gaudi_amd/csrc/gaudi_hip.hip
--- a/gaudi_amd/csrc/gaudi_hip.hip
+++ b/gaudi_amd/csrc/gaudi_hip.hip
@@ -76,6 +76,7 @@
   bool n1 = false;
   int ef = 2;
   int groups = 0;
+  int loader_groups = 0;
   int nslots = 0;
   int hk = 0;
   int pubx = 0, pub_ch = 0;
@@ -132,6 +133,8 @@
   bool no_fr = false;
   bool no_n1 = false;
   bool no_side = false;
+  bool no_ring_loader = false;
+  int last_ring_loader = 0;
   std::string last_key;
   std::vector<std::string> key_log;
   bool wide_full = true;
@@ -839,7 +842,9 @@
   return sizeof(float) * (lds_floats8_base(hpe, hpp, N, D, S, split, nodes) + (hpp ? pubx : 0));
 }
 
-static int launch(gaudi_handle* h, const KParams& P, int hpe, int hpp, long long steps) {
+static int launch(gaudi_handle* h, const KParams& P_, int hpe, int hpp, long long steps) {
+  KParams PR = P_;
+  const KParams& P = PR;
   const LaunchPlan& plan = h->plan;
   const bool v8 = plan.waves == 8;
   const bool se = hpe && plan.ef > 2;
@@ -863,6 +868,11 @@
       HIPCHECK(h, hipFuncSetAttribute((const void*)fn, hipFuncAttributeMaxDynamicSharedMemorySize, (int)lds));
       granted = (int)lds;
     }
+  }
+  const bool role = v8 && key.n1 && !h->no_ring_loader;
+  if (role) {
+    PR.edm.ktail |= 2;
+    PR.pred.ktail |= 2;
   }
   std::pair<hipEvent_t, hipEvent_t> ev{nullptr, nullptr};
   if (h->prof) HIPCHECK(h, h->prof_log.begin(h->stream, ev));
@@ -904,6 +914,7 @@
 #endif
   HIPCHECK(h, hipGetLastError());
   h->last_key = key_name(key);
+  h->last_ring_loader = role ? plan.loader_groups : 0;
   if (std::find(h->key_log.begin(), h->key_log.end(), h->last_key) == h->key_log.end()) h->key_log.push_back(h->last_key);
   if (const KernelEntry* e = find_entry(key); e && (e->side & 1) && P.side_off != 0) h->last_key += " SD=" + std::to_string(e->side);
   if (getenv("GAUDI_DEBUG_PLAN")) fprintf(stderr, "[launch] %s\n", h->last_key.c_str());
@@ -1244,6 +1255,7 @@
   plan.fr = !h->no_fr && gn8 == kResident && acc.mode == 1 && n_slots > 16;
   plan.n1 = n1_run;
   plan.groups = B;
+  plan.loader_groups = (int)std::count_if(M.ntiles.begin(), M.ntiles.begin() + B, [](int t) { return t <= w8::kWaves - 1; });
   plan.nslots = n_slots;
   plan.hk = hk;
   plan.pubx = acc.pubx;
@@ -1378,6 +1390,7 @@
   h->no_fr = getenv("GAUDI_NO_FR") != nullptr;
   h->no_n1 = getenv("GAUDI_NO_N1") != nullptr;
   h->no_side = getenv("GAUDI_NO_SIDE") != nullptr;
+  h->no_ring_loader = getenv("GAUDI_NO_RING_LOADER") != nullptr;
   h->plan.waves = h->variant;
   if (hipSetDevice(device) != hipSuccess || hipStreamCreateWithFlags(&h->stream, hipStreamNonBlocking) != hipSuccess) {
     delete h;
@@ -1425,6 +1438,7 @@
 
 const char* gaudi_last_error(const gaudi_handle* h) { return h ? h->err.c_str() : "null handle"; }
 const char* gaudi_last_warning(const gaudi_handle* h) { return h ? h->warn.c_str() : ""; }
+int gaudi_last_ring_loader(const gaudi_handle* h) { return h ? h->last_ring_loader : 0; }
 int gaudi_last_kernel_key(const gaudi_handle* h, char* buf, int n) {
   if (!h || !buf || n <= 0) return GAUDI_E_INVALID;
   snprintf(buf, (size_t)n, "%s", h->last_key.c_str());
diff --git a/gaudi_amd/csrc/w8_edm.h b/gaudi_amd/csrc/w8_edm.h
--- a/gaudi_amd/csrc/w8_edm.h
+++ b/gaudi_amd/csrc/w8_edm.h
@@ -129,7 +129,7 @@
   const float* __restrict__ w = W.w;
   const WBuf wb = make_wbuf(W.w, W.w_bytes);
   const WBuf wbe = SP ? make_wbuf(W.ws, W.ws_bytes) : wb;
-  const bool tw = W.ktail != 0;
+  const bool tw = (W.ktail & 1) != 0;
 
   for (int idx = tid; idx < N * 3; idx += kThreads) {
     const int n = idx / 3, d = idx % 3;
@@ -152,7 +152,8 @@
   __syncthreads();
   compute_geo(sm, mg, 0.f, tid, true);
   typename EdgeRing<HP, SP>::type ring;
-  er_init<HP>(ring, sm.ring, W.ktail != 0, W.ws, W.hinv);
+  er_init<HP>(ring, sm.ring, tw, W.ws, W.hinv);
+  if constexpr (node_one_tile(FL)) er_set_loader<HP>(ring, (W.ktail & 2) != 0 && mg.ntiles < kWaves);
   static_assert(SP == 0 || NodeMath<SP>::kF16, "the split edge GEMMs take their column scales from the fp16 node GEMMs' row maxima");
   constexpr bool NH = NodeMath<SP>::kF16;
   constexpr bool RI = node_ring_idle(HP, SP, GN);
diff --git a/gaudi_amd/csrc/w8_pred.h b/gaudi_amd/csrc/w8_pred.h
--- a/gaudi_amd/csrc/w8_pred.h
+++ b/gaudi_amd/csrc/w8_pred.h
@@ -77,7 +77,7 @@
   const float* __restrict__ w = W.w;
   const WBuf wb = make_wbuf(W.w, W.w_bytes);
   const WBuf wbe = SP ? make_wbuf(W.ws, W.ws_bytes) : wb;
-  const bool tw = W.ktail != 0;
+  const bool tw = (W.ktail & 1) != 0;
   float *h = sm.b0, *p = sm.b1, *q = sm.b2, *agg = sm.b3, *agg1 = sm.b4;
   float* estash = stash + pred_stash_node_floats(N, HP, W.L);
   float* astash = estash + (size_t)W.L * S * HP * 2;
@@ -104,7 +104,9 @@
   __syncthreads();
   compute_geo(sm, mg, 0.f, tid, true);
   typename EdgeRing<HP, SP>::type ring;
-  er_init<HP>(ring, sm.ring, W.ktail != 0, W.ws, W.hinv);
+  er_init<HP>(ring, sm.ring, tw, W.ws, W.hinv);
+  const bool role = node_one_tile(FL) && (W.ktail & 2) != 0 && mg.ntiles < kWaves;
+  er_set_loader<HP>(ring, role);
   constexpr bool NH = NodeMath<SP>::kF16;
   constexpr bool RI = node_ring_idle(HP, SP, GN);
   constexpr bool STG = GN && !NH;
@@ -132,6 +134,7 @@
     const bool last = l == W.L - 1;
     const PredLayerW Lw(w, lay.layer(l), HP, sm.vec);
     const bool side_l = kSideA && sm.side != nullptr && !last && (tw || !SplitGeo<HP, SP == 0 ? 1 : SP>::kTailOK);
+    if constexpr (kSideA) er_set_loader<HP>(ring, role && !side_l);
     vec_commit<NV, kThreads>(vpf, sm.vec, PredLayerW::vec_count(HP), tid);
     if constexpr (STG) stage_rows(xs0, h, N * LD, wave, lane);
     for (int idx = tid; idx < N * LD; idx += kThreads) {
@@ -309,7 +312,7 @@
   const float* __restrict__ w = W.w;
   const WBuf wb = make_wbuf(W.w, W.w_bytes);
   const WBuf wbe = SP ? make_wbuf(W.ws, W.ws_bytes) : wb;
-  const bool tw = W.ktail != 0;
+  const bool tw = (W.ktail & 1) != 0;
   float *B0 = sm.b0, *B1 = sm.b1, *B2 = sm.b2, *dh = sm.b3, *B4 = sm.b4;
   const int tid_ = tid;
   float* pub = sm.publish();
@@ -346,7 +349,8 @@
   __syncthreads();
 
   typename EdgeRing<HP, SP>::type ring;
-  er_init<HP>(ring, sm.ring, W.ktail != 0, W.ws, W.hinv);
+  er_init<HP>(ring, sm.ring, tw, W.ws, W.hinv);
+  if constexpr (node_one_tile(FL)) er_set_loader<HP>(ring, (W.ktail & 2) != 0 && mg.ntiles < kWaves);
   constexpr bool NH = NodeMath<SP>::kF16;
   constexpr bool RI = node_ring_idle(HP, SP, GN);
   constexpr bool STG = GN && !NH;
diff --git a/gaudi_amd/csrc/w8_split.h b/gaudi_amd/csrc/w8_split.h
--- a/gaudi_amd/csrc/w8_split.h
+++ b/gaudi_amd/csrc/w8_split.h
@@ -94,12 +94,21 @@
   __host__ __device__ static constexpr int tiles_of(int h) { return (h + 1) * CH <= T ? CH : T - h * CH; }
 };
 
+constexpr int kRingKTail = 1, kRingLoader = 2;
+#ifndef GAUDI_RING_LOADER_SHARE
+#define GAUDI_RING_LOADER_SHARE 0
+#endif
+#ifndef GAUDI_RING_LOADER_PRIO
+#define GAUDI_RING_LOADER_PRIO 0
+#endif
 template <int HP, int MODE>
 struct RingS {
   using G = SplitGeo<HP, MODE>;
   float* base;
   int par;
-  bool ktail;
+  int flags;
+  __device__ __forceinline__ bool ktail() const { return (flags & kRingKTail) != 0; }
+  __device__ __forceinline__ bool loader() const { return (flags & kRingLoader) != 0; }
   const float* gbase;
   float winv;
   __device__ __forceinline__ float* slot(int p) const { return base + p * G::kSlotFloats; }
@@ -108,7 +117,7 @@
 template <int HP, int MODE>
 __device__ __forceinline__ bool trip_group(const RingS<HP, MODE>& r, int W, int nextW, int tr, int& off, int& units) {
   using G = SplitGeo<HP, MODE>;
-  const bool tail = G::kTailOK && r.ktail;
+  const bool tail = G::kTailOK && r.ktail();
   const int n = tail ? G::kTripsTail : G::kTrips;
   const bool nxt = tr >= n;
   const int t2 = nxt ? tr - n : tr;
@@ -151,6 +160,78 @@
 template <int HP, int MODE>
 __device__ __forceinline__ void rings_stage(RingS<HP, MODE>& r, const WBuf& wb, int W, int nextW, int tr, int wave, int lane) {
   rings_dma(r, wb, r.slot(r.par ^ 1), W, nextW, tr + 1, wave, lane);
+}
+
+template <int HP, int MODE>
+__host__ __device__ constexpr bool ring_loader_ok() {
+  return SplitGeo<HP, MODE>::NH == 1 && SplitGeo<HP, MODE>::NC > 1 && (kWaves - 1) * (GAUDI_RING_LOADER_SHARE / 2) <= SplitGeo<HP, MODE>::T;
+}
+template <int HP, int MODE, int FIRST, int COUNT>
+struct LoaderUnits {
+__device__ __forceinline__ static void run(const WBuf& wb, int off_bytes, int lane, float* slot) {
+  using G = SplitGeo<HP, MODE>;
+  constexpr int kRun = 4, kB = G::kUnit * 4;
+  static_assert(kRun * kB <= 4096, "a run must lie within the immediate offset of its first unit");
+  const int vo = lane * 16;
+  int so = off_bytes + FIRST * kB;
+  float* l = slot + FIRST * G::kUnit;
+#pragma unroll 1
+  for (int i = 0; i < COUNT / kRun; ++i) {
+    static_for<kRun>([&](auto u_tag) {
+      constexpr int U = decltype(u_tag)::value;
+      __builtin_amdgcn_raw_ptr_buffer_load_lds(wb.r, (__attribute__((address_space(3))) void*)l, 16, vo, so, U * kB, 0);
+    });
+    so += kRun * kB;
+    l += kRun * G::kUnit;
+  }
+  static_for<COUNT % kRun>([&](auto u_tag) {
+    constexpr int U = decltype(u_tag)::value;
+    __builtin_amdgcn_raw_ptr_buffer_load_lds(wb.r, (__attribute__((address_space(3))) void*)l, 16, vo, so, U * kB, 0);
+  });
+}
+};
+template <int HP, int MODE, int UNITS, int KEEP>
+struct LoaderGroup {
+__device__ __forceinline__ static void run(const WBuf& wb, int off_bytes, int wave, int lane, float* slot, bool active) {
+  using G = SplitGeo<HP, MODE>;
+  if (!active) {
+    if (wave == kWaves - 1) {
+#if GAUDI_RING_LOADER_PRIO
+      __builtin_amdgcn_s_setprio(1);
+#endif
+      LoaderUnits<HP, MODE, (kWaves - 1) * KEEP, UNITS - (kWaves - 1) * KEEP>::run(wb, off_bytes, lane, slot);
+#if GAUDI_RING_LOADER_PRIO
+      __builtin_amdgcn_s_setprio(0);
+#endif
+    }
+  } else if constexpr (KEEP > 0) {
+    const int so = __builtin_amdgcn_readfirstlane(off_bytes + wave * KEEP * G::kUnit * 4);
+    float* const l = slot + wave * KEEP * G::kUnit;
+    static_for<KEEP>([&](auto u_tag) {
+      constexpr int U = decltype(u_tag)::value;
+      __builtin_amdgcn_raw_ptr_buffer_load_lds(wb.r, (__attribute__((address_space(3))) void*)l, 16, lane * 16, so, U * G::kUnit * 4, 0);
+    });
+  }
+}
+};
+template <int HP, int MODE, bool ACT>
+__device__ __forceinline__ void rings_stage_role(RingS<HP, MODE>& r, const WBuf& wb, int W, int nextW, int tr, int wave, int lane) {
+  using G = SplitGeo<HP, MODE>;
+  if constexpr (ring_loader_ok<HP, MODE>()) {
+    if (r.loader()) {
+      if constexpr (ACT && GAUDI_RING_LOADER_SHARE == 0) return;
+      const bool nxt = tr + 1 >= G::NC;
+      if (nxt && nextW < 0) return;
+      const int t2 = nxt ? tr + 1 - G::NC : tr + 1;
+      const int off = __builtin_amdgcn_readfirstlane(((nxt ? nextW : W) + t2 * G::kSlotFloats) * 4);
+      float* const slot = r.slot(r.par ^ 1);
+      constexpr int K2 = GAUDI_RING_LOADER_SHARE;
+      if (G::kTailOK && r.ktail() && t2 == G::NC - 1) LoaderGroup<HP, MODE, G::T, K2 / 2>::run(wb, off, wave, lane, slot, ACT);
+      else LoaderGroup<HP, MODE, G::T * kPieces, K2>::run(wb, off, wave, lane, slot, ACT);
+      return;
+    }
+  }
+  rings_stage(r, wb, W, nextW, tr, wave, lane);
 }
 
 template <int HP, int MODE>
@@ -205,7 +286,7 @@
 __device__ __forceinline__ void rings_mfma_act(f4* acc, const float* slot_lane, const B3& b, MID mid) {
   constexpr int U = SplitGeo<HP, MODE>::kUnit;
   if constexpr (!ACT) {
-    mid();
+    mid(std::bool_constant<false>{});
     return;
   }
   constexpr int kAhead = NT > 2 ? 2 : 1, kSets = kAhead + 1;
@@ -218,7 +299,7 @@
     constexpr int t = decltype(t_tag)::value;
     constexpr int cur = t % kSets;
     if (t == NT / 2) {
-      mid();
+      mid(std::bool_constant<true>{});
       __builtin_amdgcn_sched_barrier(0);
     }
     if (t == (NT - 2 > NT / 2 ? NT - 2 : NT - 1)) __builtin_amdgcn_sched_barrier(0);
@@ -254,7 +335,8 @@
 #pragma unroll
   for (int t = 0; t < T; ++t) {
     if (t == T / 2) {
-      mid();
+      if (active) mid(std::bool_constant<true>{});
+      else mid(std::bool_constant<false>{});
       __builtin_amdgcn_sched_barrier(0);
     }
     if (active) acc[t] = mfma1(a[t], b, acc[t]);
@@ -280,7 +362,7 @@
   };
   B3 bin = gen(0), nb = bin;
   static_assert(G::NH <= 3, "at most three trips per K chunk");
-  const bool tail = G::kTailOK && ring.ktail;
+  const bool tail = G::kTailOK && ring.ktail();
 #if GAUDI_EDGE_PRIO & 1
   if (wave >= kWaves / 2) __builtin_amdgcn_s_setprio(1);
 #endif
@@ -291,8 +373,8 @@
       constexpr int NT = G::tiles_of(h);
       const int tr = m * G::NH + h;
       trip_open(ring, lane);
-      rings_mfma<HP, MODE, NT>(acc + h * G::CH, ring.slot(ring.par) + lane * 4, bin, active, [&] {
-        rings_stage(ring, wb, W, nextW, tr, wave, lane);
+      rings_mfma<HP, MODE, NT>(acc + h * G::CH, ring.slot(ring.par) + lane * 4, bin, active, [&](auto act_tag) {
+        rings_stage_role<HP, MODE, decltype(act_tag)::value>(ring, wb, W, nextW, tr, wave, lane);
         if (h == G::NH - 1) nb = gen(mn);
       });
       trip_close(ring, lane);
@@ -314,7 +396,7 @@
       trip_open(ring, lane);
       const float bt = silu_f(edge_u_tail(pp, qq, sCr, sCd, g, T, r, d0)[0]) * se;
       rings_mfma_tail<HP, MODE>(acc, ring.slot(ring.par) + lane * 4, bt, active,
-                          [&] { rings_stage(ring, wb, W, nextW, G::kTripsTail - 1, wave, lane); });
+                          [&](auto act_tag) { rings_stage_role<HP, MODE, decltype(act_tag)::value>(ring, wb, W, nextW, G::kTripsTail - 1, wave, lane); });
       trip_close(ring, lane);
     }
   }
@@ -354,7 +436,7 @@
       constexpr int tr = m * G::NH + h;
       trip_open(ring, lane);
       rings_mfma<HP, MODE, G::tiles_of(h)>(out + h * G::CH, ring.slot(ring.par) + lane * 4, bin, active,
-                                           [&] { rings_stage(ring, wb, W, nextW, tr, wave, lane); });
+                                           [&](auto act_tag) { rings_stage_role<HP, MODE, decltype(act_tag)::value>(ring, wb, W, nextW, tr, wave, lane); });
       trip_close(ring, lane);
     };
     trip(std::integral_constant<int, 0>{});
@@ -375,10 +457,10 @@
   };
   static_for<G::NC - 1>([&](auto m_tag) { chunk(m_tag); });
   if constexpr (G::kTailOK) {
-    if (ring.ktail) {
+    if (ring.ktail()) {
       trip_open(ring, lane);
       rings_mfma_tail<HP, MODE>(out, ring.slot(ring.par) + lane * 4, tail_to_b(in[T - 1], c, g)[0] * se, active,
-                          [&] { rings_stage(ring, wb, W, nextW, G::kTripsTail - 1, wave, lane); });
+                          [&](auto act_tag) { rings_stage_role<HP, MODE, decltype(act_tag)::value>(ring, wb, W, nextW, G::kTripsTail - 1, wave, lane); });
       trip_close(ring, lane);
       finish();
       return;
@@ -418,9 +500,15 @@
 __device__ __forceinline__ void er_init(RingS<HP, MODE>& r, float* base, bool ktail, const float* ws, float winv) {
   r.base = base;
   r.par = 0;
-  r.ktail = ktail;
+  r.flags = ktail ? kRingKTail : 0;
   r.gbase = ws;
   r.winv = winv;
+}
+template <int HP>
+__device__ __forceinline__ void er_set_loader(Ring<HP>&, bool) {}
+template <int HP, int MODE>
+__device__ __forceinline__ void er_set_loader(RingS<HP, MODE>& r, bool on) {
+  if constexpr (ring_loader_ok<HP, MODE>()) r.flags = (r.flags & ~kRingLoader) | (on ? kRingLoader : 0);
 }
 template <int HP>
 __device__ __forceinline__ void er_start(Ring<HP>& r, const WBuf& wb, int W, int wave, int lane) {
diff --git a/gaudi_amd/engine.py b/gaudi_amd/engine.py
--- a/gaudi_amd/engine.py
+++ b/gaudi_amd/engine.py
@@ -164,6 +164,12 @@
         buf = C.create_string_buffer(256)
         self._check(fn(self.h, buf, len(buf)), "gaudi_last_kernel_key")
         return buf.value.decode()
+
+    def last_ring_loader(self) -> int:
+        fn = getattr(self.lib, "gaudi_last_ring_loader", None)
+        if fn is None or not fn.argtypes:
+            return 0
+        return int(fn(self.h))
 
     def kernel_keys_launched(self) -> list:
         fn = getattr(self.lib, "gaudi_kernel_key_log", None)
diff --git a/include/gaudi_hip.h b/include/gaudi_hip.h
--- a/include/gaudi_hip.h
+++ b/include/gaudi_hip.h
@@ -56,6 +56,7 @@
 const char* gaudi_last_error(const gaudi_handle* h);
 const char* gaudi_last_warning(const gaudi_handle* h);
 int gaudi_last_kernel_key(const gaudi_handle* h, char* buf, int n);
+int gaudi_last_ring_loader(const gaudi_handle* h);
 int gaudi_kernel_key_log(const gaudi_handle* h, char* buf, int n);
 int gaudi_host_kernel_keys(char* buf, int n);
 #define GAUDI_ABI_VERSION 7
```

After: 231.4, median of 6. Within noise of the previous version (+0.9%).
